# lukeduball/VoxelRaymarcher

Hardware: AMD Instinct MI355X
Metric: Mrays/sec at 1920x1080, 256^3 grid (VCS+original); achieved HBM GB/s (higher is better)
Workload: dtype f32; 1 GPU; C2: 256^3 synthetic, vcs+original, 1920x1080; grid=256, width=1920, height=1080, tiling=weak, store=VOXEL_CLUSTER_STORE, algorithm=ORIGINAL, scale=48, voxels=395883, parallelism=row-band tiles x1, layout=bands, frames_in_flight=2, hw_queues=4

## Files before the change

include/vr.h:

```cpp
#ifndef VR_H
#define VR_H

#include <stddef.h>
#include <stdint.h>

#ifdef __cplusplus
extern "C" {
#endif

#define VR_OK 0
#define VR_E_INVALID (-1)
#define VR_E_HIP (-2)
#define VR_E_NOMEM (-3)
#define VR_E_IO (-4)
#define VR_E_BUILD (-5)
#define VR_E_PARSE (-6)

typedef enum { VR_STORE_VCS = 0, VR_STORE_HASHTABLE = 1 } vr_store;

typedef enum { VR_ALGO_LONGESTAXIS = 0, VR_ALGO_ORIGINAL = 1 } vr_algo;

typedef struct {
    float origin[3];
    float lower_left[3];
    float horizontal[3];
    float vertical[3];
    float forward[3];
} vr_camera;

typedef struct {
    float light_dir[3];
    float light_color[3];
    float light_pos[3];
    int32_t use_point_light;
    int32_t use_shadows;
} vr_lighting;

typedef struct vr_scene vr_scene;

typedef struct {
    uint32_t diameter;
    int32_t min_coord;
    uint32_t region_count;
    uint32_t store;
    uint64_t voxel_count;
    uint64_t device_bytes;
    int32_t device;
} vr_scene_info;

typedef struct {
    uint32_t n;
    double p_region, p_cluster, p_voxel;
    uint64_t seed;
} vr_synth_params;

int vr_camera_make(const float eye[3], const float look_at[3], const float up[3],
                   float fov_deg, float aspect, vr_camera* out);

int vr_lighting_default(vr_lighting* out);

int vr_lighting_set_direction(vr_lighting* lit, const float dir[3]);

int vr_scene_create(int device, vr_store store, const int32_t* xyz, const uint32_t* rgb,
                    size_t n, vr_scene** out);

typedef enum { VR_BUILD_AUTO = 0, VR_BUILD_DEVICE = 1, VR_BUILD_HOST = 2 } vr_build;

int vr_scene_create_ex(int device, vr_store store, const int32_t* xyz, const uint32_t* rgb, size_t n,
                       int inputs_on_device, vr_build build, void* stream, vr_scene** out);

int vr_scene_digest(const vr_scene* s, uint64_t out[5]);

int vr_scene_load_vox(int device, vr_store store, const char* path, vr_scene** out);

int vr_scene_get_info(const vr_scene* s, vr_scene_info* out);
void vr_scene_destroy(vr_scene* s);

#define VR_VOXEL_REMOVE 0xFFFFFFFFu

int vr_scene_edit(vr_scene* s, const int32_t* xyz, const uint32_t* rgb, size_t n,
                  int inputs_on_device, void* stream);

int vr_scene_voxels(const vr_scene* s, int32_t* xyz, uint32_t* rgb, size_t capacity,
                    int outputs_on_device, void* stream, size_t* n_out);

#define VR_HIT_MISS    0u
#define VR_HIT_VOXEL   1u
#define VR_HIT_NEVER   2u
#define VR_HIT_OUTSIDE 3u

typedef struct {
    uint32_t status;
    uint32_t color;
    int32_t  voxel[3];
    int32_t  normal[3];
    int32_t  region[3];
    float    point[3];
    uint32_t reserved[2];
} vr_hit;

int vr_pick(const vr_scene* s, vr_algo algo, const vr_camera* cam,
            const float translation[3], uint32_t scale, uint32_t width, uint32_t height,
            const uint32_t* px, const uint32_t* py, size_t n, int inputs_on_device,
            vr_hit* hits, int outputs_on_device, void* stream);

typedef struct {
    float    origin[3];
    uint32_t reserved0;
    float    direction[3];
    uint32_t reserved1;
} vr_ray;

typedef enum {
    VR_TRACE_ORDER_AUTO = 0,
    VR_TRACE_ORDER_GIVEN = 1,
    VR_TRACE_ORDER_COHERENT = 2
} vr_trace_order;

int vr_trace(const vr_scene* s, vr_algo algo, const float translation[3], uint32_t scale,
             const vr_ray* rays, size_t n, int inputs_on_device,
             vr_hit* hits, int outputs_on_device, uint32_t order, void* stream);

int vr_camera_rays(int device, const vr_camera* cam, uint32_t width, uint32_t height,
                   const uint32_t* px, const uint32_t* py, size_t n, int inputs_on_device,
                   vr_ray* rays, int outputs_on_device, void* stream);

int vr_render(const vr_scene* s, vr_algo algo, const vr_camera* cam, const vr_lighting* lit,
              const float translation[3], uint32_t scale, uint32_t width, uint32_t height,
              uint32_t row_begin, uint32_t row_end, uint32_t* out_dev, void* stream);

int vr_render_bands(const vr_scene* s, vr_algo algo, const vr_camera* cam, const vr_lighting* lit,
                    const float translation[3], uint32_t scale, uint32_t width, uint32_t height,
                    uint32_t band_rows, uint32_t rank, uint32_t nranks, uint32_t* out_dev,
                    void* stream);
uint64_t vr_band_buffer_words(uint32_t width, uint32_t height, uint32_t band_rows, uint32_t nranks);

int vr_render_tiles(const vr_scene* s, vr_algo algo, const vr_camera* cam, const vr_lighting* lit,
                    const float translation[3], uint32_t scale, uint32_t width, uint32_t height,
                    uint32_t band_rows, uint32_t tile_cols, uint32_t rank, uint32_t nranks,
                    uint32_t* out_dev, void* stream);
uint64_t vr_tile_buffer_words(uint32_t width, uint32_t height, uint32_t band_rows, uint32_t tile_cols,
                              uint32_t nranks);
uint32_t vr_deal_stride_default(uint32_t nranks);
int vr_assemble_tiles(const void* parts_dev, void* frame_dev, uint32_t elem_bytes, uint32_t width,
                      uint32_t height, uint32_t band_rows, uint32_t tile_cols, uint32_t nranks,
                      uint32_t deal_stride, void* stream);

typedef enum {
    VR_KERNEL_AUTO = 0,
    VR_KERNEL_TILE = 1,
    VR_KERNEL_TILE_REWALK = 3
} vr_kernel;

typedef struct {
    uint32_t struct_size;
    uint32_t kernel;
    uint32_t row_begin, row_end;
    uint32_t band_rows;
    uint32_t rank, nranks;
    uint32_t defer_cap;
    uint64_t* bytes_dev;
    uint32_t schedule;
    uint32_t reserved;
    uint64_t* stats_dev;
    uint32_t occupancy;
    uint32_t tile_cols;
    uint32_t deal_stride;
    uint32_t reserved2;
} vr_render_opts;
#define VR_RENDER_OPTS_MIN_SIZE 48u

typedef enum {
    VR_OCCUPANCY_AUTO = 0,
    VR_OCCUPANCY_LONE = 1,
    VR_OCCUPANCY_IN_FLIGHT = 2
} vr_occupancy;

int vr_render_opts_init(vr_render_opts* opts);

typedef enum {
    VR_SCHEDULE_AUTO = 0,
    VR_SCHEDULE_GRID = 1,
    VR_SCHEDULE_HEAVIEST_FIRST = 2
} vr_schedule;
int vr_forget_orders(int device);
int vr_debug_skip_next_crawl(int device);
int vr_debug_capture_lane_order(int device);
int vr_debug_lane_order(int device, uint32_t info[8], uint32_t* pcost, uint64_t pcost_words, uint8_t* perm,
                        uint64_t perm_bytes);
int vr_debug_order_uses(int device, uint64_t out[8]);
int vr_render_ex(const vr_scene* s, vr_algo algo, const vr_camera* cam, const vr_lighting* lit,
                 const float translation[3], uint32_t scale, uint32_t width, uint32_t height,
                 const vr_render_opts* opts, uint32_t* out_dev, void* stream);

int vr_render_count(const vr_scene* s, vr_algo algo, const vr_camera* cam, const vr_lighting* lit,
                    const float translation[3], uint32_t scale, uint32_t width, uint32_t height,
                    uint32_t row_begin, uint32_t row_end, uint32_t* out_dev,
                    uint64_t* bytes_dev, void* stream);

int vr_pack_rgb8(const uint32_t* words_dev, uint8_t* rgb_dev, uint64_t n_pixels, void* stream);

int vr_png_write(const char* path, const uint8_t* image, uint32_t width, uint32_t height, int channels, int level);

int vr_png_encode(const uint8_t* image, uint32_t width, uint32_t height, int channels, int level, int threads,
                  uint8_t* out, size_t capacity, size_t* out_len);

int vr_synth_generate(const vr_synth_params* p, int32_t* xyz, uint32_t* rgb, size_t capacity,
                      size_t* n_out);

int vr_vox_read(const char* path, int32_t* xyz, uint32_t* rgb, size_t capacity, size_t* n_out);
int vr_vox_write(const char* path, const int32_t* xyz, const uint32_t* rgb, size_t n);

int vr_vxb_read(const char* path, int32_t* xyz, uint32_t* rgb, size_t capacity, size_t* n_out);
int vr_vxb_write(const char* path, const int32_t* xyz, const uint32_t* rgb, size_t n);
int vr_scene_file_read(const char* path, int32_t* xyz, uint32_t* rgb, size_t capacity, size_t* n_out);

const char* vr_last_error(void);
const char* vr_version(void);

#ifdef __cplusplus
}
#endif
#endif
```

voxelraymarcher_amd/__init__.py:

```python
from ._capi import LIB_PATH, VrError, lib
from .output import FrameWriter, ImageWriter, encode_png, write_png
from .renderer import (CONFIGS, HIT_DTYPE, VOXEL_REMOVE, Build, HitStatus, Camera, DeviceScene, Kernel, Occupancy, PreparedRender, RayMarchAlgorithm,
                       RenderConfig,
                       Schedule, StorageType, VoxelSceneCPU, VoxelSceneInfo, assemble_tiles_device, band_buffer_words,
                       create_scene, deal_stride_default, debug_capture_lane_order, debug_lane_order, debug_order_uses, debug_skip_next_crawl,
                       forget_orders, pack_rgb8, pick, parse_algorithm, parse_storage, RAY_DTYPE, TraceOrder, camera_rays, trace,
                       read_voxel_file, render_bands, render_count, render_ex, render_tiles, run_raymarching_kernel,
                       setup_constant_values, synth_scene, tile_buffer_words, write_binary_scene, write_voxel_file)

__all__ = ["LIB_PATH", "VrError", "lib", "FrameWriter", "ImageWriter", "encode_png", "write_png", "CONFIGS", "HIT_DTYPE", "HitStatus",
           "VOXEL_REMOVE", "Build", "pick", "RAY_DTYPE", "TraceOrder", "camera_rays", "trace",
           "Camera", "DeviceScene", "Kernel", "Occupancy", "PreparedRender", "RayMarchAlgorithm", "RenderConfig", "Schedule",
           "StorageType", "VoxelSceneCPU", "VoxelSceneInfo", "assemble_tiles_device", "band_buffer_words",
           "create_scene", "deal_stride_default", "debug_capture_lane_order", "debug_lane_order", "debug_order_uses",
           "debug_skip_next_crawl", "forget_orders", "pack_rgb8", "parse_algorithm", "parse_storage",
           "read_voxel_file", "render_bands", "render_count", "render_ex", "render_tiles", "run_raymarching_kernel",
           "setup_constant_values", "synth_scene", "tile_buffer_words", "write_binary_scene", "write_voxel_file"]
```

voxelraymarcher_amd/_capi.py:

```python
from __future__ import annotations

import ctypes
import os
from ctypes import (POINTER, c_char_p, c_double, c_float, c_int, c_int32, c_size_t, c_uint8, c_uint32,
                    c_uint64, c_void_p)

import torch

HERE = os.path.dirname(os.path.abspath(__file__))
LIB_PATH = os.environ.get("VR_LIBRARY") or os.path.join(HERE, "libvr.so")

VR_OK = 0
ERRORS = {-1: "VR_E_INVALID", -2: "VR_E_HIP", -3: "VR_E_NOMEM", -4: "VR_E_IO", -5: "VR_E_BUILD", -6: "VR_E_PARSE"}

VR_STORE_VCS, VR_STORE_HASHTABLE = 0, 1
VR_ALGO_LONGESTAXIS, VR_ALGO_ORIGINAL = 0, 1


class VrCamera(ctypes.Structure):
    _fields_ = [("origin", c_float * 3), ("lower_left", c_float * 3), ("horizontal", c_float * 3),
                ("vertical", c_float * 3), ("forward", c_float * 3)]


class VrLighting(ctypes.Structure):
    _fields_ = [("light_dir", c_float * 3), ("light_color", c_float * 3), ("light_pos", c_float * 3),
                ("use_point_light", c_int32), ("use_shadows", c_int32)]


class VrSceneInfo(ctypes.Structure):
    _fields_ = [("diameter", c_uint32), ("min_coord", c_int32), ("region_count", c_uint32), ("store", c_uint32),
                ("voxel_count", c_uint64), ("device_bytes", c_uint64), ("device", c_int32)]


class VrSynthParams(ctypes.Structure):
    _fields_ = [("n", c_uint32), ("p_region", c_double), ("p_cluster", c_double), ("p_voxel", c_double),
                ("seed", c_uint64)]


VR_KERNEL_AUTO, VR_KERNEL_TILE, VR_KERNEL_TILE_REWALK = 0, 1, 3
VR_SCHEDULE_AUTO, VR_SCHEDULE_GRID, VR_SCHEDULE_HEAVIEST_FIRST = 0, 1, 2
VR_OCCUPANCY_AUTO, VR_OCCUPANCY_LONE, VR_OCCUPANCY_IN_FLIGHT = 0, 1, 2


class VrRenderOpts(ctypes.Structure):
    _fields_ = [("struct_size", c_uint32), ("kernel", c_uint32), ("row_begin", c_uint32), ("row_end", c_uint32),
                ("band_rows", c_uint32), ("rank", c_uint32), ("nranks", c_uint32), ("defer_cap", c_uint32),
                ("bytes_dev", c_void_p), ("schedule", c_uint32), ("reserved", c_uint32), ("stats_dev", c_void_p),
                ("occupancy", c_uint32), ("tile_cols", c_uint32), ("deal_stride", c_uint32), ("reserved2", c_uint32)]


VR_RENDER_OPTS_MIN_SIZE = 48

VR_HIT_MISS, VR_HIT_VOXEL, VR_HIT_NEVER, VR_HIT_OUTSIDE = 0, 1, 2, 3


class VrHit(ctypes.Structure):
    _fields_ = [("status", c_uint32), ("color", c_uint32), ("voxel", c_int32 * 3), ("normal", c_int32 * 3),
                ("region", c_int32 * 3), ("point", c_float * 3), ("reserved", c_uint32 * 2)]


class VrRay(ctypes.Structure):
    _fields_ = [("origin", c_float * 3), ("reserved0", c_uint32), ("direction", c_float * 3), ("reserved1", c_uint32)]


VR_TRACE_ORDER_AUTO, VR_TRACE_ORDER_GIVEN, VR_TRACE_ORDER_COHERENT = 0, 1, 2


class VrError(RuntimeError):
    def __init__(self, code: int, where: str, msg: str):
        super().__init__(f"{where}: {ERRORS.get(code, code)}: {msg}")
        self.code = code


SIGNATURES = {
    "vr_camera_make": (c_int, [POINTER(c_float), POINTER(c_float), POINTER(c_float), c_float, c_float,
                               POINTER(VrCamera)]),
    "vr_lighting_default": (c_int, [POINTER(VrLighting)]),
    "vr_lighting_set_direction": (c_int, [POINTER(VrLighting), POINTER(c_float)]),
    "vr_png_write": (c_int, [c_char_p, c_void_p, c_uint32, c_uint32, c_int, c_int]),
    "vr_png_encode": (c_int, [c_void_p, c_uint32, c_uint32, c_int, c_int, c_int, c_void_p, c_size_t, POINTER(c_size_t)]),
    "vr_scene_create": (c_int, [c_int, c_int, POINTER(c_int32), POINTER(c_uint32), c_size_t, POINTER(c_void_p)]),
    "vr_scene_create_ex": (c_int, [c_int, c_int, c_void_p, c_void_p, c_size_t, c_int, c_int, c_void_p, POINTER(c_void_p)]),
    "vr_scene_digest": (c_int, [c_void_p, POINTER(c_uint64)]),
    "vr_scene_load_vox": (c_int, [c_int, c_int, c_char_p, POINTER(c_void_p)]),
    "vr_scene_get_info": (c_int, [c_void_p, POINTER(VrSceneInfo)]),
    "vr_scene_destroy": (None, [c_void_p]),
    "vr_scene_edit": (c_int, [c_void_p, c_void_p, c_void_p, c_size_t, c_int, c_void_p]),
    "vr_scene_voxels": (c_int, [c_void_p, c_void_p, c_void_p, c_size_t, c_int, c_void_p, POINTER(c_size_t)]),
    "vr_render": (c_int, [c_void_p, c_int, POINTER(VrCamera), POINTER(VrLighting), POINTER(c_float), c_uint32,
                          c_uint32, c_uint32, c_uint32, c_uint32, c_void_p, c_void_p]),
    "vr_render_bands": (c_int, [c_void_p, c_int, POINTER(VrCamera), POINTER(VrLighting), POINTER(c_float),
                                c_uint32, c_uint32, c_uint32, c_uint32, c_uint32, c_uint32, c_void_p, c_void_p]),
    "vr_band_buffer_words": (c_uint64, [c_uint32, c_uint32, c_uint32, c_uint32]),
    "vr_render_tiles": (c_int, [c_void_p, c_int, POINTER(VrCamera), POINTER(VrLighting), POINTER(c_float),
                                c_uint32, c_uint32, c_uint32, c_uint32, c_uint32, c_uint32, c_uint32, c_void_p,
                                c_void_p]),
    "vr_tile_buffer_words": (c_uint64, [c_uint32, c_uint32, c_uint32, c_uint32, c_uint32]),
    "vr_deal_stride_default": (c_uint32, [c_uint32]),
    "vr_forget_orders": (c_int, [c_int]),
    "vr_debug_skip_next_crawl": (c_int, [c_int]),
    "vr_debug_capture_lane_order": (c_int, [c_int]),
    "vr_debug_lane_order": (c_int, [c_int, POINTER(c_uint32), c_void_p, c_uint64, c_void_p, c_uint64]),
    "vr_debug_order_uses": (c_int, [c_int, POINTER(c_uint64)]),
    "vr_assemble_tiles": (c_int, [c_void_p, c_void_p, c_uint32, c_uint32, c_uint32, c_uint32, c_uint32, c_uint32,
                                  c_uint32, c_void_p]),
    "vr_render_ex": (c_int, [c_void_p, c_int, POINTER(VrCamera), POINTER(VrLighting), POINTER(c_float), c_uint32,
                             c_uint32, c_uint32, POINTER(VrRenderOpts), c_void_p, c_void_p]),
    "vr_render_opts_init": (c_int, [POINTER(VrRenderOpts)]),
    "vr_render_count": (c_int, [c_void_p, c_int, POINTER(VrCamera), POINTER(VrLighting), POINTER(c_float),
                                c_uint32, c_uint32, c_uint32, c_uint32, c_uint32, c_void_p, c_void_p, c_void_p]),
    "vr_pick": (c_int, [c_void_p, c_int, POINTER(VrCamera), POINTER(c_float), c_uint32, c_uint32, c_uint32, c_void_p,
                        c_void_p, c_size_t, c_int, c_void_p, c_int, c_void_p]),
    "vr_trace": (c_int, [c_void_p, c_int, POINTER(c_float), c_uint32, c_void_p, c_size_t, c_int, c_void_p, c_int,
                         c_uint32, c_void_p]),
    "vr_camera_rays": (c_int, [c_int, POINTER(VrCamera), c_uint32, c_uint32, c_void_p, c_void_p, c_size_t, c_int,
                               c_void_p, c_int, c_void_p]),
    "vr_pack_rgb8": (c_int, [c_void_p, c_void_p, c_uint64, c_void_p]),
    "vr_synth_generate": (c_int, [POINTER(VrSynthParams), POINTER(c_int32), POINTER(c_uint32), c_size_t,
                                  POINTER(c_size_t)]),
    "vr_vox_read": (c_int, [c_char_p, POINTER(c_int32), POINTER(c_uint32), c_size_t, POINTER(c_size_t)]),
    "vr_vox_write": (c_int, [c_char_p, POINTER(c_int32), POINTER(c_uint32), c_size_t]),
    "vr_vxb_read": (c_int, [c_char_p, POINTER(c_int32), POINTER(c_uint32), c_size_t, POINTER(c_size_t)]),
    "vr_vxb_write": (c_int, [c_char_p, POINTER(c_int32), POINTER(c_uint32), c_size_t]),
    "vr_scene_file_read": (c_int, [c_char_p, POINTER(c_int32), POINTER(c_uint32), c_size_t, POINTER(c_size_t)]),
    "vr_last_error": (c_char_p, []),
    "vr_version": (c_char_p, []),
}

_lib = None


def lib() -> ctypes.CDLL:
    global _lib
    if _lib is None:
        if not os.path.exists(LIB_PATH):
            raise ImportError(f"{LIB_PATH} not built: run __graft_entry__.build() "
                              "(make -C voxelraymarcher_amd/csrc)")
        handle = ctypes.CDLL(LIB_PATH, mode=ctypes.RTLD_GLOBAL)
        for name, (res, args) in SIGNATURES.items():
            fn = getattr(handle, name)
            fn.restype = res
            fn.argtypes = args
        _lib = handle
    return _lib


def check(rc: int, where: str) -> None:
    if rc != VR_OK:
        raise VrError(rc, where, lib().vr_last_error().decode(errors="replace"))


def f3(v) -> ctypes.Array:
    return (c_float * 3)(*[float(x) for x in v])


__all__ = ["lib", "check", "VrCamera", "VrLighting", "VrRenderOpts", "VR_RENDER_OPTS_MIN_SIZE", "VR_KERNEL_AUTO",
           "VR_KERNEL_TILE", "VR_KERNEL_TILE_REWALK", "VR_SCHEDULE_AUTO", "VR_SCHEDULE_GRID",
           "VR_SCHEDULE_HEAVIEST_FIRST", "VR_OCCUPANCY_AUTO", "VR_OCCUPANCY_LONE", "VR_OCCUPANCY_IN_FLIGHT",
           "VrSceneInfo", "VrSynthParams", "VrHit", "VR_HIT_MISS",
           "VR_HIT_VOXEL", "VR_HIT_NEVER", "VR_HIT_OUTSIDE", "VrRay", "VR_TRACE_ORDER_AUTO",
           "VR_TRACE_ORDER_GIVEN", "VR_TRACE_ORDER_COHERENT", "VrError", "SIGNATURES",
           "VR_STORE_VCS", "VR_STORE_HASHTABLE", "VR_ALGO_LONGESTAXIS", "VR_ALGO_ORIGINAL", "f3", "LIB_PATH",
           "c_uint8"]
```

voxelraymarcher_amd/csrc/vr_internal.h:

```cpp
#pragma once

#include <hip/hip_runtime.h>
#include <stddef.h>
#include <stdint.h>

#include <string>

namespace vr {

int set_error(int code, const std::string& msg);

constexpr uint32_t kEmpty = 1u << 30;
constexpr uint32_t kNone = 0xFFFFFFFFu;
constexpr int32_t kBlock = 64;
constexpr uint32_t kTileBudget = 4096u;
constexpr uint32_t kCrawlBudget = 1u << 30;
constexpr uint32_t kDeferMarker = 0xFFFFFFFFu;
constexpr uint32_t kVcsMaxRegions = 65536u;
constexpr uint32_t kHashFilterWords = 8192u;

struct KScene {
    const uint32_t* region_slot;
    const uint2* vcs_mask;
    const uint32_t* vcs_vals;
    const uint32_t* vcs_cbits;
    const uint4* ht_meta;
    const uint2* ht_slots;
    const uint32_t* ht_filter;
    uint32_t D;
    int32_t min_coord;
    uint32_t n_regions;
};

struct KView {
    float llc[3], hor[3], ver[3], org[3];
    float L[3], LC[3], LP[3];
    float Lr[3];
    uint32_t L_fast;
    float Lw[3];
    uint32_t L_order, L_cls, L_unit, L_eq;
    float translation[3];
    float scale_f;
    int32_t use_point_light, use_shadows;
    uint32_t W, H;
    uint32_t row0, band_rows, rank, nranks, local_rows, row_limit;
    uint32_t band_minv;
    uint32_t LW;
    uint32_t tile_cols;
    uint32_t tile_minv;
    uint32_t col_R, col_rank, col_stride;
    uint32_t* out;
    unsigned long long* bytes;
    unsigned long long* stats;
    uint32_t* defer;
    uint32_t defer_cap;
    uint32_t crawl_rewalk;
    uint32_t crawl_rpw;
    uint32_t* defer_stat;
    const uint32_t* order;
    uint32_t* cost;
    const uint8_t* perm;
    uint32_t* pcost;
    uint32_t* slot_stat;
    uint32_t launch_id;
};
static_assert(sizeof(KView) - offsetof(KView, out) == 104,
              "a KView field was added after `out`: review whether it belongs to the view identity");

constexpr uint32_t kDeferCap = 16384;
constexpr uint32_t kDeferRecWords = 20;
constexpr uint32_t kDeferWords = 4 + kDeferCap * kDeferRecWords;

hipError_t launch_march(int store, int algo, bool count, const KScene& s, const KView& v,
                        hipStream_t stream, uint32_t crawl_wgs, bool in_flight, bool crawl = true);
uint32_t crawl_grid(uint32_t records, uint32_t rpw);
constexpr uint32_t kPickMiss = 0, kPickVoxel = 1, kPickNever = 2, kPickOutside = 3;
hipError_t launch_pick(int store, int algo, const KScene& s, const KView& v, const uint32_t* px, const uint32_t* py,
                       uint32_t n, void* hits, hipStream_t stream);
hipError_t launch_trace(int store, int algo, const KScene& s, const KView& v, const void* rays, const uint32_t* idx,
                        uint32_t n, void* hits, hipStream_t stream);
hipError_t launch_camera_rays(const KView& v, const uint32_t* px, const uint32_t* py, uint32_t n, void* rays,
                              hipStream_t stream);
hipError_t trace_order(const KScene& s, const KView& v, const void* rays, uint32_t n, hipStream_t stream,
                       void** scratch, const uint32_t** idx);
hipError_t launch_cluster_bits(const uint2* vcs_mask, uint32_t n_regions, uint32_t* cbits, hipStream_t stream);
hipError_t launch_hash_filter(const uint4* ht_meta, const uint2* ht_slots, uint32_t n_regions, uint32_t* filter,
                              hipStream_t stream);
hipError_t launch_pack_rgb8(const uint32_t* words, uint8_t* rgb, uint64_t n, hipStream_t stream);
struct TileLayout {
    uint32_t W, H, band_rows, tile_cols, R, stride, LW;
    uint64_t rank_words;
};
hipError_t launch_assemble_tiles(const void* parts, void* frame, uint32_t elem_bytes, const TileLayout& t,
                                 hipStream_t stream);
void march_grid(const KView& v, uint32_t& columns, uint32_t& rows);
constexpr uint32_t kWavesPerTileGroup = 2;
hipError_t launch_order(const uint32_t* cost, uint32_t n, uint32_t columns, uint32_t* order, hipStream_t stream);
size_t perm_bytes(uint32_t gx, uint32_t gy);
struct LaneShape {
    uint32_t block_x, block_y, entry_bytes, seat;
};
LaneShape lane_shape();
hipError_t launch_perm(const uint32_t* pcost, uint32_t LW, uint32_t rows, uint32_t gx, uint32_t gy, uint8_t* perm,
                       uint32_t* cost, hipStream_t stream);

}
```

voxelraymarcher_amd/csrc/vr_launch.cpp:

```cpp
#include <algorithm>
#include <chrono>
#include <climits>
#include <cmath>
#include <cstddef>
#include <cstdio>
#include <cstdlib>
#include <cstring>
#include <initializer_list>
#include <mutex>
#include <string>
#include <vector>

#include "vr_host.h"
#pragma GCC visibility push(hidden)
#include "vr_launch_plan.h"
#pragma GCC visibility pop

namespace {

using vr::DeviceGuard;
using vr::fail;
using vr::hip_fail;

int make_view(const vr_scene* s, const vr_camera* cam, const vr_lighting* lit, const float translation[3],
              uint32_t scale, uint32_t width, uint32_t height, vr::KView& v) {
    if (!s) return fail(VR_E_INVALID, "scene is NULL");
    if (!cam || !lit) return fail(VR_E_INVALID, "camera/lighting NULL");
    if (width == 0 || height == 0 || width > 65536 || height > 65536) return fail(VR_E_INVALID, "bad image size");
    memset(&v, 0, sizeof v);
    for (int i = 0; i < 3; ++i) {
        v.llc[i] = cam->lower_left[i]; v.hor[i] = cam->horizontal[i]; v.ver[i] = cam->vertical[i];
        v.org[i] = cam->origin[i];
        v.L[i] = lit->light_dir[i]; v.LC[i] = lit->light_color[i]; v.LP[i] = lit->light_pos[i];
        v.translation[i] = translation ? translation[i] : 0.0f;
    }
    v.L_fast = 1u;
    for (int i = 0; i < 3; ++i) {
        const float a = std::fabs(v.L[i]);
        v.Lr[i] = 1.0f / v.L[i];
        if (!(a >= 0x1p-64f && a <= 0x1p+20f)) v.L_fast = 0u;
    }
    {
        const float ax = std::fabs(v.L[0]), ay = std::fabs(v.L[1]), az = std::fabs(v.L[2]);
        const uint32_t order =
            (ax > ay && ax > az) ? (ay > az ? 0u : 1u) : (ay > az ? (ax > az ? 2u : 3u) : (ax > ay ? 4u : 5u));
        const float k = 1.0f / (order < 2u ? ax : (order < 4u ? ay : az));
        uint32_t cls = 0;
        bool unit = order == 5u && ax == ay && ay == az;
        for (int i = 0; i < 3; ++i) {
            v.Lw[i] = k * v.L[i];
            cls |= (uint32_t)(v.Lw[i] > 0.0f) << (2 * i) | (uint32_t)(v.Lw[i] < 0.0f) << (2 * i + 1);
            unit = unit && std::fabs(v.Lw[i]) == 1.0f;
        }
        v.L_order = order;
        v.L_cls = cls;
        v.L_unit = unit ? 1u : 0u;
        v.L_eq = (v.L[0] == v.L[1] && v.L[1] == v.L[2]) ? 1u : 0u;
    }
    v.scale_f = (float)scale;
    v.use_point_light = lit->use_point_light ? 1 : 0;
    v.use_shadows = lit->use_shadows ? 1 : 0;
    v.W = width;
    v.H = height;
    v.LW = width;
    return VR_OK;
}

bool env_flag(const char* name, bool dflt) {
    const char* e = std::getenv(name);
    return e ? (dflt ? e[0] != '0' : e[0] == '1') : dflt;
}
uint32_t env_uint(const char* name, long lo, long hi, uint32_t dflt) {
    const char* e = std::getenv(name);
    const long v = e ? std::strtol(e, nullptr, 10) : lo - 1;
    return v >= lo && v <= hi ? (uint32_t)v : dflt;
}
uint32_t order_refresh() { static const uint32_t r = env_uint("VR_ORDER_REFRESH", 1, LONG_MAX, 0); return r; }
bool order_enabled() { static const bool on = env_flag("VR_ORDER", true); return on; }
bool lane_order_enabled() { static const bool on = env_flag("VR_LANE_ORDER", true); return on; }
bool crawl_skip_enabled() { static const bool on = env_flag("VR_CRAWL_SKIP", true); return on; }
const vr::PolicyKnobs& policy_knobs() {
    static const vr::PolicyKnobs k = {env_flag("VR_INFLIGHT_HEAVY", false), env_flag("VR_INFLIGHT_WAVES", true),
                                      env_uint("VR_CRAWL_RPW", 1, 64, 0), env_uint("VR_CRAWL_RPW_IN_FLIGHT", 1, 64, 32)};
    return k;
}

struct SlotRing {
    const size_t words = vr::kDeferWords;
    const uint32_t nslots = 16;
    struct Slot {
        vr::WorkOrder work;
        vr::LaneOrder lane;
        vr::CrawlSkip skip;
    };
    struct Dev {
        std::mutex mu;
        uint32_t* base = nullptr;
        std::vector<hipEvent_t> ev;
        std::vector<bool> used;
        uint32_t next = 0;
        uint32_t* stat_host = nullptr;
        uint32_t* stat_dev = nullptr;
        uint32_t launch_serial = 0;
        std::vector<Slot> slot;
        bool any = false;
        hipStream_t last_stream = nullptr;
        uint32_t last_idx = 0;
        uint64_t last_key = 0;
        bool force_skip = false;
        uint64_t uses[6] = {0, 0, 0, 0, 0, 0};
        bool capture_lane = false;
        struct LaneCapture {
            uint32_t LW = 0, rows = 0, gx = 0, gy = 0;
            std::vector<uint32_t> pcost;
            std::vector<uint8_t> perm;
        } lane_capture;
        bool alone(hipStream_t st) const {
            return !any || last_stream == st || hipEventQuery(ev[last_idx]) == hipSuccess;
        }
        bool follow(hipStream_t st, uint32_t idx, uint64_t key) {
            const bool repeat = last_key == key;
            any = true;
            last_stream = st;
            last_idx = idx;
            last_key = key;
            return repeat;
        }
    } dev[64];
} g_defer_ring;

int ring_init(SlotRing& r, SlotRing::Dev& D) {
    void* q = nullptr;
    const size_t bytes = (size_t)r.nslots * r.words * sizeof(uint32_t);
    std::vector<hipEvent_t> made;
    auto undo = [&](hipError_t e, const char* what) {
        for (hipEvent_t x : made) (void)hipEventDestroy(x);
        if (q) (void)hipFree(q);
        return hip_fail(e, what);
    };
    hipError_t e = hipMalloc(&q, bytes);
    if (e != hipSuccess) { q = nullptr; return undo(e, "hipMalloc(slot ring)"); }
    e = hipMemset(q, 0, bytes);
    if (e == hipSuccess) e = hipDeviceSynchronize();
    if (e != hipSuccess) return undo(e, "hipMemset(slot ring)");
    std::vector<hipEvent_t> ev(r.nslots);
    for (uint32_t i = 0; i < r.nslots; ++i) {
        e = hipEventCreateWithFlags(&ev[i], hipEventDisableTiming);
        if (e != hipSuccess) return undo(e, "hipEventCreate(slot ring)");
        made.push_back(ev[i]);
    }
    void* h = nullptr;
    void* hd = nullptr;
    const size_t stat_words = 2u + 2u * (size_t)r.nslots;
    e = hipHostMalloc(&h, sizeof(uint32_t) * stat_words, hipHostMallocMapped | hipHostMallocCoherent);
    if (e == hipSuccess) {
        for (size_t i = 0; i < stat_words; ++i) ((volatile uint32_t*)h)[i] = 0u;
        e = hipHostGetDevicePointer(&hd, h, 0);
        if (e != hipSuccess) (void)hipHostFree(h);
    }
    if (e != hipSuccess) return undo(e, "hipHostMalloc(crawl statistics)");
    D.ev = std::move(ev);
    D.used.assign(r.nslots, false);
    D.slot.assign(r.nslots, SlotRing::Slot{});
    D.stat_host = (uint32_t*)h;
    D.stat_dev = (uint32_t*)hd;
    D.base = (uint32_t*)q;
    return VR_OK;
}

struct SlotLease {
    SlotRing* ring = nullptr;
    std::unique_lock<std::mutex> lk;
    int dev = -1;
    uint32_t idx = 0;
    uint32_t* p = nullptr;
    int acquire(SlotRing& r, int d, hipStream_t stream) {
        if (d < 0 || d >= 64) return fail(VR_E_INVALID, "device index too large");
        SlotRing::Dev& D = r.dev[d];
        lk = std::unique_lock<std::mutex>(D.mu);
        if (!D.base) {
            int rc = ring_init(r, D);
            if (rc) return rc;
        }
        ring = &r;
        dev = d;
        idx = D.next;
        D.next = (D.next + 1u) % r.nslots;
        if (D.used[idx]) {
            hipError_t e = hipStreamWaitEvent(stream, D.ev[idx], 0);
            if (e != hipSuccess) return hip_fail(e, "hipStreamWaitEvent(slot ring)");
        }
        p = D.base + r.words * idx;
        return VR_OK;
    }
    SlotRing::Dev& D() const { return ring->dev[dev]; }
    int release(hipStream_t stream) {
        hipError_t e = hipEventRecord(D().ev[idx], stream);
        if (e != hipSuccess) return hip_fail(e, "hipEventRecord(slot ring)");
        D().used[idx] = true;
        lk.unlock();
        return VR_OK;
    }
};

uint64_t view_key(const vr_scene* s, vr_algo algo, const vr::KView& v) {
    const uint32_t a = (uint32_t)algo;
    uint64_t h = vr::fnv1a(vr::kFnvBasis, &s->serial, sizeof s->serial);
    h = vr::fnv1a(h, &s->revision, sizeof s->revision);
    h = vr::fnv1a(h, &a, sizeof a);
    return vr::fnv1a(h, &v, offsetof(vr::KView, out));
}

uint64_t crawl_key(uint64_t key, const vr::KView& v) {
    const uint32_t knobs[2] = {v.defer_cap, v.crawl_rewalk};
    return vr::fnv1a(key, knobs, sizeof knobs);
}

struct Regrow {
    void** p;
    size_t bytes;
};
hipError_t regrow(std::initializer_list<Regrow> bufs, hipStream_t st) {
    hipError_t e = hipSuccess;
    for (const Regrow& b : bufs) {
        const hipError_t e2 = *b.p ? hipFreeAsync(*b.p, st) : hipSuccess;
        if (e == hipSuccess) e = e2;
        *b.p = nullptr;
    }
    for (const Regrow& b : bufs)
        if (e == hipSuccess) e = hipMallocAsync(b.p, b.bytes, st);
    if (e != hipSuccess)
        for (const Regrow& b : bufs) {
            if (*b.p) (void)hipFreeAsync(*b.p, st);
            *b.p = nullptr;
        }
    return e;
}

hipError_t bind_work_order(vr::WorkOrder& W, uint32_t gx, uint32_t gy, uint64_t key, bool repeat, hipStream_t st,
                           vr::KView& v, bool& remake) {
    const uint32_t n = gx * gy;
    if (n > W.cap) {
        W.cap = 0;
        W.valid = false;
        const hipError_t e = regrow({{(void**)&W.cost, sizeof(uint32_t) * vr::kWavesPerTileGroup * (size_t)n},
                                     {(void**)&W.order, sizeof(uint32_t) * (size_t)n}}, st);
        if (e != hipSuccess) return e;
        W.cap = n;
    }
    const bool match = W.matches(gx, gy, key);
    v.order = match ? W.order : nullptr;
    remake = vr::remake_due(match, W.relaned, repeat, W.age, order_refresh());
    v.cost = remake ? W.cost : nullptr;
    return hipSuccess;
}

hipError_t bind_lane_order(vr::LaneOrder& L, uint32_t gx, uint32_t gy, uint64_t key, bool repeat, hipStream_t st,
                           vr::KView& v, bool& relane, const char*& what) {
    const size_t nperm = vr::perm_bytes(gx, gy);
    if (nperm > L.bcap) {
        L.bcap = 0;
        L.valid = false;
        what = "lane order buffer";
        const hipError_t e = regrow({{(void**)&L.perm, nperm}}, st);
        if (e != hipSuccess) return e;
        L.bcap = nperm;
    }
    const bool match = L.matches(gx, gy, key);
    v.perm = match ? L.perm : nullptr;
    relane = vr::remake_due(match, false, repeat, L.age, order_refresh());
    if (!relane) return hipSuccess;
    what = "lane order walk lengths";
    return hipMallocAsync((void**)&v.pcost, sizeof(uint32_t) * (size_t)v.LW * v.local_rows, st);
}

int refuse_capture(hipStream_t st) {
    hipStreamCaptureStatus cap = hipStreamCaptureStatusNone;
    const hipError_t e = hipStreamIsCapturing(st, &cap);
    if (e != hipSuccess) return hip_fail(e, "hipStreamIsCapturing");
    if (cap != hipStreamCaptureStatusNone)
        return fail(VR_E_INVALID, "vr_render* cannot be captured into a HIP graph (stream is capturing)");
    return VR_OK;
}

void order_check(const vr::WorkOrder& W, uint32_t slot, uint32_t gx, uint32_t gy) {
    if (!std::getenv("VR_ORDER_CHECK")) return;
    const uint32_t n = gx * gy;
    std::vector<uint32_t> h(n), c(2 * (size_t)n);
    (void)hipDeviceSynchronize();
    (void)hipMemcpy(h.data(), W.order, 4 * (size_t)n, hipMemcpyDeviceToHost);
    (void)hipMemcpy(c.data(), W.cost, 8 * (size_t)n, hipMemcpyDeviceToHost);
    std::vector<int> seen(n, 0);
    int bad = 0;
    for (uint32_t i = 0; i < n; ++i) {
        const uint32_t t = (h[i] >> 16) * gx + (h[i] & 0xFFFFu);
        if ((h[i] & 0xFFFFu) >= gx || t >= n || seen[t]++) ++bad;
    }
    fprintf(stderr, "[order] slot %u grid %ux%u n %u bad %d first %08x %08x cost0 %u %u\n", slot, gx, gy, n, bad, h[0],
            n > 1 ? h[1] : 0u, c[0], c[1]);
}

#ifdef VR_HOST_PROF
}
static uint64_t g_hp[4096][8];
static uint32_t g_hp_n = 0;
static inline uint64_t hp_now() { return (uint64_t)std::chrono::steady_clock::now().time_since_epoch().count(); }
extern "C" int vr_host_prof_fetch(uint64_t* out, int n) {
    const uint32_t k = g_hp_n < 4096u ? g_hp_n : 4096u;
    const uint32_t m = (uint32_t)n < k ? (uint32_t)n : k;
    for (uint32_t i = 0; i < m; ++i)
        for (int j = 0; j < 8; ++j) out[8 * i + j] = g_hp[(g_hp_n - m + i) % 4096u][j];
    return (int)m;
}
namespace {
#define VR_HP(i) hp_row[i] = hp_now()
#else
#define VR_HP(i) do { } while (0)
#endif

int launch(const vr_scene* s, vr_algo algo, uint32_t kernel, uint32_t schedule, uint32_t occupancy, vr::KView& v,
           void* stream) {
#ifdef VR_HOST_PROF
    uint64_t* hp_row = g_hp[g_hp_n++ % 4096u];
    for (int j = 0; j < 8; ++j) hp_row[j] = 0;
#endif
    VR_HP(0);
    if (algo != VR_ALGO_ORIGINAL && algo != VR_ALGO_LONGESTAXIS) return fail(VR_E_INVALID, "unknown algorithm");
    if (kernel != VR_KERNEL_AUTO && kernel != VR_KERNEL_TILE && kernel != VR_KERNEL_TILE_REWALK)
        return fail(VR_E_INVALID, "unknown kernel (2, the persistent kernel, was retired)");
    if (occupancy > VR_OCCUPANCY_IN_FLIGHT) return fail(VR_E_INVALID, "unknown occupancy");
    if (v.local_rows == 0 || v.LW == 0) return VR_OK;
    DeviceGuard dg(s->device);
    const hipStream_t st = (hipStream_t)stream;
    int rc = refuse_capture(st);
    if (rc) return rc;
    SlotLease lease;
    rc = lease.acquire(g_defer_ring, s->device, st);
    if (rc) return rc;
    VR_HP(1);
    auto bail = [&](hipError_t err, const char* what) {
        (void)lease.release(st);
        return hip_fail(err, what);
    };
    SlotRing::Dev& D = lease.D();
    SlotRing::Slot& S = D.slot[lease.idx];
    v.crawl_rewalk = kernel == VR_KERNEL_TILE_REWALK ? 1u : 0u;
    v.defer = lease.p;
    v.defer_cap = (v.defer_cap && v.defer_cap < vr::kDeferCap) ? v.defer_cap : vr::kDeferCap;
    v.defer_stat = D.stat_dev;
    v.slot_stat = D.stat_dev + 2 + 2 * (size_t)lease.idx;
    const uint32_t expect = *(volatile uint32_t*)D.stat_host;
    uint32_t gx = 0, gy = 0;
    vr::march_grid(v, gx, gy);
    const uint32_t n = gx * gy;
    const bool alone = D.alone(st);
    VR_HP(2);
    const vr::LaunchPolicy pol = vr::launch_policy(schedule, occupancy, alone, policy_knobs());
    v.crawl_rpw = pol.crawl_rpw;
    const uint64_t key = view_key(s, algo, v);
    const bool repeat = D.follow(st, lease.idx, key);
    VR_HP(3);
    bool remake = false, relane = false;
    hipError_t e = hipSuccess;
    if (pol.heavy && order_enabled() && n != 0) {
        e = bind_work_order(S.work, gx, gy, key, repeat, st, v, remake);
        if (e != hipSuccess) return bail(e, "work order buffers");
    }
    if (lane_order_enabled() && n != 0) {
        const char* what = "";
        e = bind_lane_order(S.lane, gx, gy, key, repeat, st, v, relane, what);
        if (e != hipSuccess) return bail(e, what);
    }
    VR_HP(4);
    v.launch_id = vr::next_launch_id(D.launch_serial);
    const uint64_t report = *reinterpret_cast<volatile uint64_t*>(D.stat_host + 2 + 2 * (size_t)lease.idx);
    const bool crawl = S.skip.step(crawl_key(key, v), report, v.launch_id, D.force_skip, crawl_skip_enabled());
    VR_HP(5);
    const vr::KScene ks = vr::kscene(s);
    const uint32_t cwgs = vr::crawl_grid(expect, v.crawl_rpw);
    D.uses[0] += 1u;
    D.uses[2] += v.perm != nullptr;
    D.uses[4] += v.order != nullptr;
    D.uses[5] += !crawl;
    VR_HP(6);
    e = vr::launch_march((int)s->store, (int)algo, v.bytes != nullptr, ks, v, st, cwgs, pol.hi, crawl);
    VR_HP(7);
    bool with_costs = false;
    if (e == hipSuccess && relane) {
        with_costs = order_enabled() && S.work.cost && S.work.cap >= n;
        e = vr::launch_perm(v.pcost, v.LW, v.local_rows, gx, gy, S.lane.perm, with_costs ? S.work.cost : nullptr, st);
        S.lane.learned(gx, gy, key, e == hipSuccess);
        D.uses[1] += e == hipSuccess;
        S.work.relaned = !with_costs;
        if (e == hipSuccess && D.capture_lane) {
            D.capture_lane = false;
            SlotRing::Dev::LaneCapture& C = D.lane_capture;
            C.LW = v.LW, C.rows = v.local_rows, C.gx = gx, C.gy = gy;
            C.pcost.resize((size_t)v.LW * v.local_rows);
            C.perm.resize(vr::perm_bytes(gx, gy));
            e = hipStreamSynchronize(st);
            if (e == hipSuccess) e = hipMemcpy(C.pcost.data(), v.pcost, sizeof(uint32_t) * C.pcost.size(), hipMemcpyDeviceToHost);
            if (e == hipSuccess) e = hipMemcpy(C.perm.data(), S.lane.perm, C.perm.size(), hipMemcpyDeviceToHost);
        }
    }
    if (e == hipSuccess && (remake || with_costs)) {
        e = vr::launch_order(S.work.cost, n, gx, S.work.order, st);
        order_check(S.work, lease.idx, gx, gy);
        S.work.learned(gx, gy, key, e == hipSuccess);
        D.uses[3] += e == hipSuccess;
    }
    if (v.pcost) {
        const hipError_t ef = hipFreeAsync(v.pcost, st);
        if (e == hipSuccess) e = ef;
    }
    rc = lease.release(st);
    if (e != hipSuccess) return hip_fail(e, "ray-march launch");
    return rc;
}

}

extern "C" {

int vr_render_ex(const vr_scene* s, vr_algo algo, const vr_camera* cam, const vr_lighting* lit,
                 const float translation[3], uint32_t scale, uint32_t width, uint32_t height,
                 const vr_render_opts* opts, uint32_t* out_dev, void* stream) {
    if (!opts) return fail(VR_E_INVALID, "opts is NULL");
    if (opts->struct_size < VR_RENDER_OPTS_MIN_SIZE)
        return fail(VR_E_INVALID, "vr_render_opts.struct_size is " + std::to_string(opts->struct_size) +
                                      ": set it to sizeof(vr_render_opts) (vr_render_opts_init); a struct built "
                                      "against the layout without struct_size is not accepted");
    vr_render_opts o{};
    std::memcpy(&o, opts, std::min<size_t>(opts->struct_size, sizeof o));
    if (o.reserved != 0u) return fail(VR_E_INVALID, "vr_render_opts.reserved must be 0");
    vr::KView v;
    int rc = make_view(s, cam, lit, translation, scale, width, height, v);
    if (rc) return rc;
    if (!out_dev) return fail(VR_E_INVALID, "out_dev is NULL");
    const uint32_t row_end = o.row_end == 0xFFFFFFFFu ? height : o.row_end;
    if (o.row_begin > row_end || row_end > height) return fail(VR_E_INVALID, "bad row range");
    if (!o.nranks || o.rank >= o.nranks) return fail(VR_E_INVALID, "bad band partition");
    if (o.reserved2 != 0u) return fail(VR_E_INVALID, "vr_render_opts.reserved2 must be 0");
    const uint32_t rows = row_end - o.row_begin;
    const uint32_t band = o.band_rows ? o.band_rows : std::max(1u, rows);
    v.row0 = o.row_begin;
    v.row_limit = row_end;
    v.band_rows = band;
    v.band_minv = band == 1u ? 0xFFFFFFFFu : (uint32_t)((1ull << 32) / band);
    if (o.tile_cols == 0u) {
        v.rank = o.rank;
        v.nranks = o.nranks;
        v.local_rows = (uint32_t)(vr_band_buffer_words(width, rows, band, o.nranks) / width);
    } else {
        if (o.tile_cols > width) return fail(VR_E_INVALID, "tile_cols larger than the frame width");
        v.rank = 0;
        v.nranks = 1;
        v.local_rows = (uint32_t)(((uint64_t)rows + band - 1) / band * band);
        const uint32_t nblk = (width + o.tile_cols - 1) / o.tile_cols;
        v.LW = (nblk + o.nranks - 1) / o.nranks * o.tile_cols;
        v.tile_cols = o.tile_cols;
        v.tile_minv = o.tile_cols == 1u ? 0xFFFFFFFFu : (uint32_t)((1ull << 32) / o.tile_cols);
        v.col_R = o.nranks;
        v.col_rank = o.rank;
        v.col_stride = (o.deal_stride ? o.deal_stride : vr_deal_stride_default(o.nranks)) % o.nranks;
        if (v.local_rows > 65535u || v.LW > 65535u) return fail(VR_E_INVALID, "tile buffer too large");
    }
    v.out = out_dev;
    v.bytes = (unsigned long long*)o.bytes_dev;
    v.stats = o.bytes_dev ? (unsigned long long*)o.stats_dev : nullptr;
    v.defer_cap = o.defer_cap;
    if (o.schedule > VR_SCHEDULE_HEAVIEST_FIRST) return fail(VR_E_INVALID, "unknown schedule");
    return launch(s, algo, o.kernel, o.schedule, o.occupancy, v, stream);
}

int vr_pick(const vr_scene* s, vr_algo algo, const vr_camera* cam, const float translation[3], uint32_t scale,
            uint32_t width, uint32_t height, const uint32_t* px, const uint32_t* py, size_t n, int inputs_on_device,
            vr_hit* hits, int outputs_on_device, void* stream) {
    static_assert(sizeof(vr_hit) == 64 && offsetof(vr_hit, voxel) == 8 && offsetof(vr_hit, normal) == 20 &&
                      offsetof(vr_hit, region) == 32 && offsetof(vr_hit, point) == 44 && offsetof(vr_hit, reserved) == 56,
                  "vr_hit: the record pick_kernel writes");
    static_assert(vr::kPickMiss == VR_HIT_MISS && vr::kPickVoxel == VR_HIT_VOXEL && vr::kPickNever == VR_HIT_NEVER &&
                      vr::kPickOutside == VR_HIT_OUTSIDE, "VR_HIT_*");
    if (!s) return fail(VR_E_INVALID, "vr_pick: scene is NULL");
    if (!cam || !translation) return fail(VR_E_INVALID, "vr_pick: camera/translation NULL");
    if (n && (!px || !py || !hits)) return fail(VR_E_INVALID, "vr_pick: px/py/hits NULL");
    if (width == 0 || height == 0 || width > 65536 || height > 65536) return fail(VR_E_INVALID, "vr_pick: bad image size");
    if (n >= (1ull << 31)) return fail(VR_E_INVALID, "vr_pick: too many queries");
    if (algo != VR_ALGO_ORIGINAL && algo != VR_ALGO_LONGESTAXIS) return fail(VR_E_INVALID, "vr_pick: unknown algorithm");
    if (n == 0) return VR_OK;
    vr_lighting lit;
    vr_lighting_default(&lit);
    vr::KView v;
    int rc = make_view(s, cam, &lit, translation, scale, width, height, v);
    if (rc) return rc;
    v.row_limit = height;
    v.band_rows = height;
    v.band_minv = height == 1u ? 0xFFFFFFFFu : (uint32_t)((1ull << 32) / height);
    v.nranks = 1;
    v.local_rows = height;
    DeviceGuard dg(s->device);
    const hipStream_t st = (hipStream_t)stream;
    hipStreamCaptureStatus cap = hipStreamCaptureStatusNone;
    hipError_t e = hipStreamIsCapturing(st, &cap);
    if (e != hipSuccess) return hip_fail(e, "hipStreamIsCapturing");
    if (cap != hipStreamCaptureStatusNone)
        return fail(VR_E_INVALID, "vr_pick cannot be captured into a HIP graph (stream is capturing)");
    const uint32_t *dpx = px, *dpy = py;
    void *tq = nullptr, *th = nullptr;
    auto release = [&]() {
        if (tq) (void)hipFree(tq);
        if (th) (void)hipFree(th);
    };
    if (!inputs_on_device) {
        e = hipMalloc(&tq, 2 * n * sizeof(uint32_t));
        if (e == hipSuccess) e = hipMemcpyAsync(tq, px, n * sizeof(uint32_t), hipMemcpyHostToDevice, st);
        if (e == hipSuccess)
            e = hipMemcpyAsync((uint32_t*)tq + n, py, n * sizeof(uint32_t), hipMemcpyHostToDevice, st);
        if (e != hipSuccess) { release(); return hip_fail(e, "vr_pick: query upload"); }
        dpx = (const uint32_t*)tq;
        dpy = dpx + n;
    }
    void* dh = hits;
    if (!outputs_on_device) {
        e = hipMalloc(&th, n * sizeof(vr_hit));
        if (e != hipSuccess) { release(); return hip_fail(e, "vr_pick: hit buffer"); }
        dh = th;
    } else if (((uintptr_t)hits & 15u) != 0u) {
        release();
        return fail(VR_E_INVALID, "vr_pick: device hits must be 16-byte aligned");
    }
    e = vr::launch_pick((int)s->store, (int)algo, vr::kscene(s), v, dpx, dpy, (uint32_t)n, dh, st);
    if (e == hipSuccess && !outputs_on_device)
        e = hipMemcpyAsync(hits, th, n * sizeof(vr_hit), hipMemcpyDeviceToHost, st);
    const hipError_t es = hipStreamSynchronize(st);
    if (e == hipSuccess) e = es;
    release();
    if (e != hipSuccess) return hip_fail(e, "vr_pick");
    return VR_OK;
}

int vr_trace(const vr_scene* s, vr_algo algo, const float translation[3], uint32_t scale, const vr_ray* rays, size_t n,
             int inputs_on_device, vr_hit* hits, int outputs_on_device, uint32_t order, void* stream) {
    static_assert(sizeof(vr_ray) == 32 && offsetof(vr_ray, reserved0) == 12 && offsetof(vr_ray, direction) == 16 &&
                      offsetof(vr_ray, reserved1) == 28, "vr_ray: the record trace_kernel loads");
    if (!s) return fail(VR_E_INVALID, "vr_trace: scene is NULL");
    if (!translation) return fail(VR_E_INVALID, "vr_trace: translation NULL");
    if (n && (!rays || !hits)) return fail(VR_E_INVALID, "vr_trace: rays/hits NULL");
    if (n >= (1ull << 31)) return fail(VR_E_INVALID, "vr_trace: too many rays");
    if (algo != VR_ALGO_ORIGINAL && algo != VR_ALGO_LONGESTAXIS) return fail(VR_E_INVALID, "vr_trace: unknown algorithm");
    if (order != VR_TRACE_ORDER_AUTO && order != VR_TRACE_ORDER_GIVEN && order != VR_TRACE_ORDER_COHERENT)
        return fail(VR_E_INVALID, "vr_trace: unknown order");
    if (n == 0) return VR_OK;
    if (inputs_on_device && ((uintptr_t)rays & 15u) != 0u)
        return fail(VR_E_INVALID, "vr_trace: device rays must be 16-byte aligned");
    if (outputs_on_device && ((uintptr_t)hits & 15u) != 0u)
        return fail(VR_E_INVALID, "vr_trace: device hits must be 16-byte aligned");
    vr::KView v;
    memset(&v, 0, sizeof v);
    for (int i = 0; i < 3; ++i) v.translation[i] = translation[i];
    v.scale_f = (float)scale;
    const bool coherent = order == VR_TRACE_ORDER_COHERENT;
    DeviceGuard dg(s->device);
    const hipStream_t st = (hipStream_t)stream;
    hipStreamCaptureStatus cap = hipStreamCaptureStatusNone;
    hipError_t e = hipStreamIsCapturing(st, &cap);
    if (e != hipSuccess) return hip_fail(e, "hipStreamIsCapturing");
    if (cap != hipStreamCaptureStatusNone)
        return fail(VR_E_INVALID, "vr_trace cannot be captured into a HIP graph (stream is capturing)");
    void *tr = nullptr, *th = nullptr, *to = nullptr;
    auto release = [&]() {
        if (tr) (void)hipFree(tr);
        if (th) (void)hipFree(th);
        if (to) (void)hipFree(to);
    };
    const void* dr = rays;
    if (!inputs_on_device) {
        e = hipMalloc(&tr, n * sizeof(vr_ray));
        if (e == hipSuccess) e = hipMemcpyAsync(tr, rays, n * sizeof(vr_ray), hipMemcpyHostToDevice, st);
        if (e != hipSuccess) { (void)hipStreamSynchronize(st); release(); return hip_fail(e, "vr_trace: ray upload"); }
        dr = tr;
    }
    void* dh = hits;
    if (!outputs_on_device) {
        e = hipMalloc(&th, n * sizeof(vr_hit));
        if (e != hipSuccess) { (void)hipStreamSynchronize(st); release(); return hip_fail(e, "vr_trace: hit buffer"); }
        dh = th;
    }
    const uint32_t* idx = nullptr;
    if (coherent) e = vr::trace_order(vr::kscene(s), v, dr, (uint32_t)n, st, &to, &idx);
    if (e == hipSuccess) e = vr::launch_trace((int)s->store, (int)algo, vr::kscene(s), v, dr, idx, (uint32_t)n, dh, st);
    if (e == hipSuccess && !outputs_on_device)
        e = hipMemcpyAsync(hits, th, n * sizeof(vr_hit), hipMemcpyDeviceToHost, st);
    const hipError_t es = hipStreamSynchronize(st);
    if (e == hipSuccess) e = es;
    release();
    if (e != hipSuccess) return hip_fail(e, "vr_trace");
    return VR_OK;
}

int vr_camera_rays(int device, const vr_camera* cam, uint32_t width, uint32_t height, const uint32_t* px,
                   const uint32_t* py, size_t n, int inputs_on_device, vr_ray* rays, int outputs_on_device, void* stream) {
    if (!cam) return fail(VR_E_INVALID, "vr_camera_rays: camera NULL");
    if (n && (!px || !py || !rays)) return fail(VR_E_INVALID, "vr_camera_rays: px/py/rays NULL");
    if (width == 0 || height == 0 || width > 65536 || height > 65536)
        return fail(VR_E_INVALID, "vr_camera_rays: bad image size");
    if (n >= (1ull << 31)) return fail(VR_E_INVALID, "vr_camera_rays: too many pixels");
    if (device < 0 || device > 63) return fail(VR_E_INVALID, "vr_camera_rays: bad device");
    if (n == 0) return VR_OK;
    if (outputs_on_device && ((uintptr_t)rays & 15u) != 0u)
        return fail(VR_E_INVALID, "vr_camera_rays: device rays must be 16-byte aligned");
    vr::KView v;
    memset(&v, 0, sizeof v);
    for (int i = 0; i < 3; ++i) {
        v.llc[i] = cam->lower_left[i]; v.hor[i] = cam->horizontal[i]; v.ver[i] = cam->vertical[i];
        v.org[i] = cam->origin[i];
    }
    v.W = width;
    v.H = height;
    v.LW = width;
    v.row_limit = height;
    v.band_rows = height;
    v.band_minv = height == 1u ? 0xFFFFFFFFu : (uint32_t)((1ull << 32) / height);
    v.nranks = 1;
    v.local_rows = height;
    int ndev = 0;
    if (hipGetDeviceCount(&ndev) != hipSuccess || device >= ndev) return fail(VR_E_INVALID, "vr_camera_rays: no such device");
    DeviceGuard dg(device);
    const hipStream_t st = (hipStream_t)stream;
    hipStreamCaptureStatus cap = hipStreamCaptureStatusNone;
    hipError_t e = hipStreamIsCapturing(st, &cap);
    if (e != hipSuccess) return hip_fail(e, "hipStreamIsCapturing");
    if (cap != hipStreamCaptureStatusNone)
        return fail(VR_E_INVALID, "vr_camera_rays cannot be captured into a HIP graph (stream is capturing)");
    const uint32_t *dpx = px, *dpy = py;
    void *tq = nullptr, *tr = nullptr;
    auto release = [&]() {
        if (tq) (void)hipFree(tq);
        if (tr) (void)hipFree(tr);
    };
    if (!inputs_on_device) {
        e = hipMalloc(&tq, 2 * n * sizeof(uint32_t));
        if (e == hipSuccess) e = hipMemcpyAsync(tq, px, n * sizeof(uint32_t), hipMemcpyHostToDevice, st);
        if (e == hipSuccess)
            e = hipMemcpyAsync((uint32_t*)tq + n, py, n * sizeof(uint32_t), hipMemcpyHostToDevice, st);
        if (e != hipSuccess) { (void)hipStreamSynchronize(st); release(); return hip_fail(e, "vr_camera_rays: pixel upload"); }
        dpx = (const uint32_t*)tq;
        dpy = dpx + n;
    }
    void* dr = rays;
    if (!outputs_on_device) {
        e = hipMalloc(&tr, n * sizeof(vr_ray));
        if (e != hipSuccess) { (void)hipStreamSynchronize(st); release(); return hip_fail(e, "vr_camera_rays: ray buffer"); }
        dr = tr;
    }
    e = vr::launch_camera_rays(v, dpx, dpy, (uint32_t)n, dr, st);
    if (e == hipSuccess && !outputs_on_device)
        e = hipMemcpyAsync(rays, tr, n * sizeof(vr_ray), hipMemcpyDeviceToHost, st);
    const hipError_t es = hipStreamSynchronize(st);
    if (e == hipSuccess) e = es;
    release();
    if (e != hipSuccess) return hip_fail(e, "vr_camera_rays");
    return VR_OK;
}

int vr_render_opts_init(vr_render_opts* opts) {
    if (!opts) return fail(VR_E_INVALID, "NULL argument");
    *opts = vr_render_opts{};
    opts->struct_size = (uint32_t)sizeof(vr_render_opts);
    opts->kernel = VR_KERNEL_AUTO;
    opts->row_begin = 0;
    opts->row_end = 0xFFFFFFFFu;
    opts->band_rows = 0;
    opts->rank = 0;
    opts->nranks = 1;
    opts->schedule = VR_SCHEDULE_AUTO;
    return VR_OK;
}

namespace {
vr_render_opts opts_rows(uint32_t row_begin, uint32_t row_end) {
    vr_render_opts o;
    vr_render_opts_init(&o);
    o.row_begin = row_begin;
    o.row_end = row_end;
    return o;
}
}

int vr_render(const vr_scene* s, vr_algo algo, const vr_camera* cam, const vr_lighting* lit, const float translation[3],
              uint32_t scale, uint32_t width, uint32_t height, uint32_t row_begin, uint32_t row_end, uint32_t* out_dev,
              void* stream) {
    const vr_render_opts o = opts_rows(row_begin, row_end);
    return vr_render_ex(s, algo, cam, lit, translation, scale, width, height, &o, out_dev, stream);
}

uint64_t vr_band_buffer_words(uint32_t width, uint32_t height, uint32_t band_rows, uint32_t nranks) {
    if (!band_rows || !nranks) return 0;
    uint64_t nb = (height + (uint64_t)band_rows - 1) / band_rows;
    uint64_t per = (nb + nranks - 1) / nranks;
    return per * band_rows * (uint64_t)width;
}

uint32_t vr_deal_stride_default(uint32_t nranks) {
    return (nranks % 3u == 0u) ? 1u : 3u;
}

int vr_forget_orders(int device) {
    if (device < 0 || device >= 64) return fail(VR_E_INVALID, "device index out of range");
    SlotRing::Dev& D = g_defer_ring.dev[device];
    std::lock_guard<std::mutex> lk(D.mu);
    for (SlotRing::Slot& S : D.slot) {
        S.work.forget();
        S.lane.forget();
        S.skip.forget();
    }
    D.last_key = 0;
    return VR_OK;
}

int vr_debug_skip_next_crawl(int device) {
    if (device < 0 || device >= 64) return fail(VR_E_INVALID, "device index out of range");
    SlotRing::Dev& D = g_defer_ring.dev[device];
    std::lock_guard<std::mutex> lk(D.mu);
    D.force_skip = true;
    return VR_OK;
}

int vr_debug_order_uses(int device, uint64_t out[8]) {
    if (device < 0 || device >= 64) return fail(VR_E_INVALID, "device index out of range");
    if (!out) return fail(VR_E_INVALID, "out is NULL");
    SlotRing::Dev& D = g_defer_ring.dev[device];
    const vr::LaneShape sh = vr::lane_shape();
    std::lock_guard<std::mutex> lk(D.mu);
    for (int i = 0; i < 6; ++i) out[i] = D.uses[i];
    out[6] = g_defer_ring.nslots;
    out[7] = (uint64_t)sh.block_x << 16 | sh.block_y;
    return VR_OK;
}

int vr_debug_capture_lane_order(int device) {
    if (device < 0 || device >= 64) return fail(VR_E_INVALID, "device index out of range");
    SlotRing::Dev& D = g_defer_ring.dev[device];
    std::lock_guard<std::mutex> lk(D.mu);
    D.capture_lane = true;
    D.lane_capture = {};
    return VR_OK;
}

int vr_debug_lane_order(int device, uint32_t info[8], uint32_t* pcost, uint64_t pcost_words, uint8_t* perm,
                        uint64_t perm_bytes) {
    if (device < 0 || device >= 64) return fail(VR_E_INVALID, "device index out of range");
    if (!info) return fail(VR_E_INVALID, "info is NULL");
    SlotRing::Dev& D = g_defer_ring.dev[device];
    std::lock_guard<std::mutex> lk(D.mu);
    const SlotRing::Dev::LaneCapture& C = D.lane_capture;
    if (C.perm.empty()) return fail(VR_E_INVALID, "no lane order captured (vr_debug_capture_lane_order, then a repeated view)");
    const vr::LaneShape sh = vr::lane_shape();
    const uint32_t words[8] = {C.LW, C.rows, C.gx, C.gy, sh.block_x, sh.block_y, sh.entry_bytes, sh.seat};
    std::memcpy(info, words, sizeof words);
    if (pcost) {
        if (pcost_words != C.pcost.size()) return fail(VR_E_INVALID, "pcost_words is not info[0] * info[1]");
        std::memcpy(pcost, C.pcost.data(), sizeof(uint32_t) * C.pcost.size());
    }
    if (perm) {
        if (perm_bytes != C.perm.size()) return fail(VR_E_INVALID, "perm_bytes is not the captured order's size");
        std::memcpy(perm, C.perm.data(), C.perm.size());
    }
    return VR_OK;
}

uint64_t vr_tile_buffer_words(uint32_t width, uint32_t height, uint32_t band_rows, uint32_t tile_cols, uint32_t nranks) {
    if (!nranks || !tile_cols || !width || !height) return 0;
    const uint64_t band = band_rows ? band_rows : height;
    const uint64_t rows = (height + band - 1) / band * band;
    const uint64_t nblk = ((uint64_t)width + tile_cols - 1) / tile_cols;
    return rows * ((nblk + nranks - 1) / nranks * tile_cols);
}

int vr_render_tiles(const vr_scene* s, vr_algo algo, const vr_camera* cam, const vr_lighting* lit,
                    const float translation[3], uint32_t scale, uint32_t width, uint32_t height, uint32_t band_rows,
                    uint32_t tile_cols, uint32_t rank, uint32_t nranks, uint32_t* out_dev, void* stream) {
    if (!band_rows || !tile_cols) return fail(VR_E_INVALID, "band_rows and tile_cols must be > 0");
    vr_render_opts o = opts_rows(0, height);
    o.band_rows = band_rows;
    o.tile_cols = tile_cols;
    o.rank = rank;
    o.nranks = nranks;
    return vr_render_ex(s, algo, cam, lit, translation, scale, width, height, &o, out_dev, stream);
}

int vr_assemble_tiles(const void* parts_dev, void* frame_dev, uint32_t elem_bytes, uint32_t width, uint32_t height,
                      uint32_t band_rows, uint32_t tile_cols, uint32_t nranks, uint32_t deal_stride, void* stream) {
    if (!parts_dev || !frame_dev) return fail(VR_E_INVALID, "NULL device buffer");
    if (elem_bytes < 1u || elem_bytes > 4u) return fail(VR_E_INVALID, "elem_bytes must be 1..4");
    if (!width || !height || !band_rows || !tile_cols || !nranks || tile_cols > width)
        return fail(VR_E_INVALID, "bad tile layout");
    vr::TileLayout t{};
    t.W = width;
    t.H = height;
    t.band_rows = band_rows;
    t.tile_cols = tile_cols;
    t.R = nranks;
    t.stride = (deal_stride ? deal_stride : vr_deal_stride_default(nranks)) % nranks;
    t.LW = (uint32_t)(vr_tile_buffer_words(width, band_rows, band_rows, tile_cols, nranks) / band_rows);
    t.rank_words = vr_tile_buffer_words(width, height, band_rows, tile_cols, nranks);
    hipError_t e = vr::launch_assemble_tiles(parts_dev, frame_dev, elem_bytes, t, (hipStream_t)stream);
    if (e != hipSuccess) return hip_fail(e, "assemble_tiles launch");
    return VR_OK;
}

int vr_render_bands(const vr_scene* s, vr_algo algo, const vr_camera* cam, const vr_lighting* lit,
                    const float translation[3], uint32_t scale, uint32_t width, uint32_t height, uint32_t band_rows,
                    uint32_t rank, uint32_t nranks, uint32_t* out_dev, void* stream) {
    if (!band_rows) return fail(VR_E_INVALID, "band_rows must be > 0");
    vr_render_opts o = opts_rows(0, height);
    o.band_rows = band_rows;
    o.rank = rank;
    o.nranks = nranks;
    return vr_render_ex(s, algo, cam, lit, translation, scale, width, height, &o, out_dev, stream);
}

int vr_render_count(const vr_scene* s, vr_algo algo, const vr_camera* cam, const vr_lighting* lit,
                    const float translation[3], uint32_t scale, uint32_t width, uint32_t height, uint32_t row_begin,
                    uint32_t row_end, uint32_t* out_dev, uint64_t* bytes_dev, void* stream) {
    if (!bytes_dev) return fail(VR_E_INVALID, "bytes_dev is NULL");
    vr_render_opts o = opts_rows(row_begin, row_end);
    o.bytes_dev = bytes_dev;
    return vr_render_ex(s, algo, cam, lit, translation, scale, width, height, &o, out_dev, stream);
}

int vr_pack_rgb8(const uint32_t* words_dev, uint8_t* rgb_dev, uint64_t n_pixels, void* stream) {
    if (n_pixels && (!words_dev || !rgb_dev)) return fail(VR_E_INVALID, "NULL device buffer");
    hipError_t e = vr::launch_pack_rgb8(words_dev, rgb_dev, n_pixels, (hipStream_t)stream);
    if (e != hipSuccess) return hip_fail(e, "pack_rgb8 launch");
    return VR_OK;
}

}
```

voxelraymarcher_amd/csrc/vr_launch_plan.h:

```cpp
#pragma once

#include <stddef.h>
#include <stdint.h>

#include "vr.h"

namespace vr {

struct PolicyKnobs {
    bool inflight_heavy;
    bool in_flight_occupancy;
    uint32_t rpw_override;
    uint32_t rpw_in_flight;
};
struct LaunchPolicy {
    bool heavy;
    bool hi;
    uint32_t crawl_rpw;
};
inline LaunchPolicy launch_policy(uint32_t schedule, uint32_t occupancy, bool alone, const PolicyKnobs& k) {
    LaunchPolicy p;
    p.heavy = schedule == VR_SCHEDULE_HEAVIEST_FIRST || (schedule == VR_SCHEDULE_AUTO && (alone || k.inflight_heavy));
    p.hi = occupancy == VR_OCCUPANCY_IN_FLIGHT || (occupancy == VR_OCCUPANCY_AUTO && !alone && k.in_flight_occupancy);
    p.crawl_rpw = k.rpw_override ? k.rpw_override : (alone ? 2u : k.rpw_in_flight);
    return p;
}

inline bool refresh_due(uint32_t& age, uint32_t refresh) { return refresh != 0 && ++age >= refresh; }
inline bool remake_due(bool match, bool stale, bool repeat, uint32_t& age, uint32_t refresh) {
    return match ? (stale || refresh_due(age, refresh)) : repeat;
}

struct Learned {
    uint32_t gx = 0, gy = 0, age = 0;
    uint64_t key = 0;
    bool valid = false;
    bool matches(uint32_t x, uint32_t y, uint64_t k) const { return valid && gx == x && gy == y && key == k; }
    void learned(uint32_t x, uint32_t y, uint64_t k, bool ok) { valid = ok; gx = x; gy = y; key = k; age = 0; }
    void forget() { valid = false; }
};
struct WorkOrder : Learned {
    uint32_t* cost = nullptr;
    uint32_t* order = nullptr;
    uint32_t cap = 0;
    bool relaned = false;
    void learned(uint32_t x, uint32_t y, uint64_t k, bool ok) { Learned::learned(x, y, k, ok); relaned = false; }
    void forget() { valid = relaned = false; }
};
struct LaneOrder : Learned {
    uint8_t* perm = nullptr;
    size_t bcap = 0;
};

inline uint32_t next_launch_id(uint32_t& serial) { return ++serial ? serial : ++serial; }

struct CrawlSkip {
    uint32_t cid = 0;
    uint64_t ckey = 0;
    bool czero = false;
    bool step(uint64_t key, uint64_t report, uint32_t lid, bool& force, bool enabled) {
        const uint32_t rid = (uint32_t)report, count = (uint32_t)(report >> 32);
        if (ckey != key) {
            czero = false;
        } else if (czero) {
            if (count != 0u) czero = false;
        } else if (cid != 0u) {
            czero = rid == cid && count == 0u;
        }
        if (force) {
            force = false;
            czero = true;
            ckey = key;
        }
        const bool crawl = !(czero && enabled);
        if (crawl) {
            cid = lid;
            ckey = key;
        }
        return crawl;
    }
    void forget() { cid = 0; czero = false; }
};

}
```

voxelraymarcher_amd/csrc/vr_march.hip:

```cpp
#include "vr_device.h"
#include "vr_crawl.h"

#include <algorithm>
#include <type_traits>

#ifdef VR_CRAWL_PROF
__device__ unsigned int g_vr_crawl_prof[16384 * 8];
#endif
#ifdef VR_DIAG
__device__ unsigned long long g_vr_diag[64];
#define VR_DIAG_COUNT(k)                                                              \
    do {                                                                             \
        if (__lane_id() == (uint32_t)__builtin_ctzll(__builtin_amdgcn_read_exec())) \
            atomicAdd(&g_vr_diag[(k)], 1ull);                                        \
    } while (0)
#define VR_DIAG_COUNT_IF(c, k)                                  \
    do {                                                       \
        if (__builtin_amdgcn_ballot_w64(c) != 0) VR_DIAG_COUNT(k); \
    } while (0)
#define VR_DIAG_PAT(shadow, p) VR_DIAG_COUNT(((shadow) ? 51 : 43) + (p))
#else
#define VR_DIAG_COUNT(k) do { } while (0)
#define VR_DIAG_COUNT_IF(c, k) do { } while (0)
#define VR_DIAG_PAT(shadow, p) do { } while (0)
#endif

namespace vr {
namespace {

template <int S> struct Sgn { static constexpr int value = S; };
template <int S>
__device__ __forceinline__ float plane_v(float o, float g, float ge) {
    if constexpr (S > 0) return ceilf(o) + kEps;
    else if constexpr (S < 0) return floorf(o) - kEps;
    else return next_plane_fma(o, g, ge);
}
template <int S>
__device__ __forceinline__ int32_t plane_c8(int32_t c8) {
    if constexpr (S > 0) return 8;
    else if constexpr (S < 0) return 0;
    else return c8;
}

#ifndef VR_TILES_X
#define VR_TILES_X 2
#endif
#ifndef VR_TILES_Y
#define VR_TILES_Y 1
#endif
constexpr uint32_t kTilesX = VR_TILES_X, kTilesY = VR_TILES_Y;
#ifndef VR_UNIFORM_SKIP
#define VR_UNIFORM_SKIP 1
#endif
#ifndef VR_LONG_TAIL_GENERIC
#define VR_LONG_TAIL_GENERIC false
#endif
#ifndef VR_LONG_TAIL_EQ
#define VR_LONG_TAIL_EQ 0
#endif

constexpr uint32_t kDeferredIters = 0xFFFFFFFFu;

__device__ __forceinline__ void deferral_report(const KView& v) {
    if (v.slot_stat) *reinterpret_cast<uint2*>(v.slot_stat) = uint2{v.launch_id, 1u};
}

__device__ __forceinline__ void tile_group(const KView& v, uint32_t& bx, uint32_t& by) {
    bx = blockIdx.x;
    by = blockIdx.y;
    if (v.order) {
        const uint32_t t = v.order[blockIdx.y * gridDim.x + blockIdx.x];
        bx = t & 0xFFFFu;
        by = t >> 16;
    }
}

#ifdef VR_LANE_BLOCK
#define VR_LANE_BLOCK_DEFAULT_X VR_LANE_BLOCK
#define VR_LANE_BLOCK_DEFAULT_Y VR_LANE_BLOCK
#else
#define VR_LANE_BLOCK_DEFAULT_X 16
#define VR_LANE_BLOCK_DEFAULT_Y 32
#endif
#ifndef VR_LANE_BLOCK_X
#define VR_LANE_BLOCK_X VR_LANE_BLOCK_DEFAULT_X
#endif
#ifndef VR_LANE_BLOCK_Y
#define VR_LANE_BLOCK_Y VR_LANE_BLOCK_DEFAULT_Y
#endif
constexpr uint32_t kLaneBlockX = VR_LANE_BLOCK_X, kLaneBlockY = VR_LANE_BLOCK_Y;
static_assert((kLaneBlockX == 16 || kLaneBlockX == 32) && (kLaneBlockY == 16 || kLaneBlockY == 32),
              "lane block: 16 or 32 pixels a side");
constexpr uint32_t kLanePixels = kLaneBlockX * kLaneBlockY;
constexpr uint32_t kLbX = kLaneBlockX / (8u * kTilesX), kLbY = kLaneBlockY / (8u * kTilesY);
using PermT = std::conditional<kLanePixels == 256, uint8_t, uint16_t>::type;
#ifndef VR_LANE_SEAT
#define VR_LANE_SEAT 0
#endif
constexpr uint32_t kLaneSeat = VR_LANE_SEAT;
static_assert(kLaneSeat <= 1u, "lane seat: 0 (cost order) or 1 (Morton order)");
constexpr bool kLaneOrder = kTilesX == 2 && kTilesY == 1;
__device__ __forceinline__ void lane_pixel(const KView& v, uint32_t& x, uint32_t& l) {
    const uint32_t lane = threadIdx.x & 63u, wave = threadIdx.x >> 6;
    uint32_t bx, by;
    tile_group(v, bx, by);
    const uint32_t BX = bx / kLbX, BY = by / kLbY;
    if (kLaneOrder && v.perm && (BX + 1u) * kLbX <= gridDim.x && (BY + 1u) * kLbY <= gridDim.y) {
        const uint32_t q = ((by % kLbY) * kLbX + bx % kLbX) * kTilesX + wave;
        const uint32_t blk = BY * ((gridDim.x + kLbX - 1u) / kLbX) + BX;
        const uint32_t p = reinterpret_cast<const PermT*>(v.perm)[(size_t)blk * kLanePixels + q * 64u + lane];
        x = BX * kLaneBlockX + p % kLaneBlockX;
        l = BY * kLaneBlockY + p / kLaneBlockX;
    } else {
        x = (bx * kTilesX + wave % kTilesX) * 8u + (lane & 7u);
        l = (by * kTilesY + wave / kTilesX) * 8u + (lane >> 3);
    }
}

__device__ __forceinline__ uint32_t* tile_pixels() {
    __shared__ uint32_t p[64u * kTilesX * kTilesY];
    return p;
}

__device__ __forceinline__ uint32_t* tile_prim() {
    __shared__ uint32_t p[64u * kTilesX * kTilesY];
    return p;
}

template <int STORE, bool CRAWL>
struct ExactWalk { static constexpr bool value = CRAWL; };
template <bool PICK> struct PickCell {};
template <> struct PickCell<true> { i3 pv{0, 0, 0}; };
template <int STORE, bool COUNT, bool CRAWL, bool PICK = false>
struct Walker : Ctx<STORE, COUNT, ExactWalk<STORE, CRAWL>::value ? kCrawlBudget : kTileBudget>, PickCell<PICK> {
    using C = Ctx<STORE, COUNT, ExactWalk<STORE, CRAWL>::value ? kCrawlBudget : kTileBudget>;
    static constexpr bool kExact = ExactWalk<STORE, CRAWL>::value;
    static constexpr uint32_t kBudget = C::kBudget;
    using C::s; using C::v; using C::aborted; using C::tick; using C::exists; using C::lookup;
    using C::lighting; using C::normal_from_t; using C::in_region; using C::grid_in_region;
    using C::advance_region; using C::in_scene; using C::region_at; using C::skip_null; using C::bytes;
    __device__ Walker(const KScene& s_, const KView& v_) : C(s_, v_) {}
    static constexpr bool kFastSetup = STORE == STORE_HASH;
#ifndef VR_LONG_REMAT
#define VR_LONG_REMAT 1
#endif
    static constexpr bool kRematDir = VR_LONG_REMAT && STORE == STORE_VCS && !CRAWL;
    uint32_t ctx = 0, lit_saved = 0;
    uint32_t* lbm = nullptr;
    uint32_t bm_reg = kNone;

    template <bool SHADOW, bool EQ = false>
    __device__ __forceinline__ bool grid_original(f3& o, f3 d, uint32_t reg, i3 cr, Hit& h,
                                                  const uint32_t* rs = nullptr, const Rcp* rc = nullptr) {
        return grid_original_rt(o, d, reg, cr, h, SHADOW, SHADOW && EQ, rs, rc);
    }
    __device__ __forceinline__ bool grid_original_rt(f3& o, f3 d, uint32_t reg, i3 cr, Hit& h, const bool SHADOW,
                                                     const bool EQ, const uint32_t* rs = nullptr,
                                                     const Rcp* rc = nullptr, const bool generic = false) {
        const bool resume = CRAWL && rs != nullptr;
        VR_DIAG_COUNT(SHADOW ? 9 : 8);
        const bool px = d.x > 0.0f, py = d.y > 0.0f, pz = d.z > 0.0f;
        const bool zx = SHADOW && d.x == 0.0f, zy = SHADOW && d.y == 0.0f, zz = SHADOW && d.z == 0.0f;
        float tX, tY, tZ;
        if (resume) {
            tX = __uint_as_float(rs[11]); tY = __uint_as_float(rs[12]); tZ = __uint_as_float(rs[13]);
        } else if (!CRAWL) {
            const bool use_rc = rc && (kFastSetup || SHADOW);
            const Rcp r0x = use_rc ? rc[0] : rcp_setup(d.x), r0y = use_rc ? rc[1] : rcp_setup(d.y),
                      r0z = use_rc ? rc[2] : rcp_setup(d.z);
            const float sx = px ? 1.0f : -1.0f, sy = py ? 1.0f : -1.0f, sz = pz ? 1.0f : -1.0f;
            const float ax = next_plane_fma(o.x, sx, sx * kEps) - o.x, ay = next_plane_fma(o.y, sy, sy * kEps) - o.y,
                        az = next_plane_fma(o.z, sz, sz * kEps) - o.z;
            const bool fast = r0x.ok && r0y.ok && r0z.ok && !zx && !zy && !zz &&
                              fminf(fabsf(ax), fminf(fabsf(ay), fabsf(az))) >= 0x1p-90f;
            tX = div_fast(ax, r0x); tY = div_fast(ay, r0y); tZ = div_fast(az, r0z);
            if (__builtin_expect(__builtin_amdgcn_ballot_w64(!fast) != 0, 0)) {
                VR_DIAG_COUNT(32);
                tX = fast ? tX : (zx ? kInf : ax / d.x);
                tY = fast ? tY : (zy ? kInf : ay / d.y);
                tZ = fast ? tZ : (zz ? kInf : az / d.z);
            }
            o = add(o, scl(fminf(tX, fminf(tY, tZ)) + kEps, d));
        } else {
            const float nX = px ? ceilf(o.x) + kEps : floorf(o.x) - kEps;
            const float nY = py ? ceilf(o.y) + kEps : floorf(o.y) - kEps;
            const float nZ = pz ? ceilf(o.z) + kEps : floorf(o.z) - kEps;
            tX = zx ? kInf : (nX - o.x) / d.x;
            tY = zy ? kInf : (nY - o.y) / d.y;
            tZ = zz ? kInf : (nZ - o.z) / d.z;
            o = add(o, scl(fminf(tX, fminf(tY, tZ)) + kEps, d));
        }
        uint32_t col = kEmpty;
        if constexpr (STORE == STORE_VCS) {
            const uint2* mreg = s.vcs_mask + (size_t)reg * 8192u;
            const uint32_t moff = reg << 16;
            const uint32_t* bits = nullptr;
            if constexpr (CRAWL) {
                if (lbm) {
                    if (reg != bm_reg) {
                        const uint4* src = reinterpret_cast<const uint4*>(s.vcs_cbits + (size_t)reg * 16u);
                        const uint4 b0 = src[0], b1 = src[1], b2 = src[2], b3 = src[3];
                        uint4* dst = reinterpret_cast<uint4*>(lbm);
                        dst[0] = b0; dst[1] = b1; dst[2] = b2; dst[3] = b3;
                        bm_reg = reg;
                    }
                    bits = lbm;
                }
            }
            o = add(o, f3{0.0f, 0.0f, 0.0f});
            if (!this->in_region_bits_nz(o)) return false;
            if (aborted || this->iters >= kBudget) { aborted = true; return false; }
            bool found = false, inside = true, crawl = false;
            uint32_t crawl_after = 0;
            bool crawl_off = false;
            uint32_t vi = 0;
            int32_t qx = 0, qy = 0, qz = 0;
            Blk blk{0u, kNone};
            uint32_t bit = 0;
            bool resume_now = resume;
            for (;;) {
                f3 dl = d;
                if (CRAWL) asm("" : "+v"(dl.x), "+v"(dl.y), "+v"(dl.z));
                Rcp rx, ry, rz;
                if (rc && !CRAWL && (kFastSetup || SHADOW)) {
                    rx = EQ ? Rcp{fabsf(dl.x), fabsf(rc[0].r), rc[0].ok} : rc[0];
                    ry = rc[1];
                    rz = rc[2];
                } else {
                    rx = rcp_setup(EQ ? fabsf(dl.x) : dl.x); ry = rcp_setup(dl.y); rz = rcp_setup(dl.z);
                }
                const float gx = px ? 1.0f : -1.0f, gy = py ? 1.0f : -1.0f, gz = pz ? 1.0f : -1.0f;
                const float ex = gx * kEps, ey = gy * kEps, ez = gz * kEps;
                const int32_t cx8 = px ? 8 : 0, cy8 = py ? 8 : 0, cz8 = pz ? 8 : 0;
                const bool walk_ok = rx.ok && ry.ok && rz.ok && !zx && !zy && !zz;
                const float nlim = walk_ok ? 0x1p-90f : kInf;
                if (resume_now) {
                    resume_now = false;
                    blk = Blk{0u, kNone};
                    bit = 0;
                    qx = (int32_t)rs[15]; qy = (int32_t)rs[16]; qz = (int32_t)rs[17];
                } else {
                    auto walk = [&](auto SXc, auto SYc, auto SZc) {
                        constexpr int SX = decltype(SXc)::value, SY = decltype(SYc)::value, SZ = decltype(SZc)::value;
                        constexpr bool kPos = SX == 2 && SY == 2 && SZ == 2;
                        uint32_t ic = this->iters + (0x42800000u - kBudget);
                        const bool okw = __builtin_amdgcn_ballot_w64(!walk_ok) == 0;
                        VR_DIAG_COUNT((SHADOW ? 4 : 0) + (SX == 0 ? 1 : 0));
                        for (;;) {
                            VR_DIAG_COUNT((SHADOW ? 6 : 2) + (SX == 0 ? 1 : 0));
                            const int32_t vx = f2i(o.x), vy = f2i(o.y), vz = f2i(o.z);
                            this->count(4);
                            const uint32_t wi = this->word_index((uint32_t)vx, (uint32_t)vy, (uint32_t)vz);
                            if constexpr (CRAWL) {
                                const bool pres = !bits || ((bits[wi >> 9] >> ((wi >> 4) & 31u)) & 1u);
                                if (COUNT && !pres) ++this->nl;
                                blk = Blk{0u, kNone};
                                if (pres)
                                    blk = *reinterpret_cast<const uint2*>(reinterpret_cast<const char*>(s.vcs_mask) +
                                                                          (moff | (wi << 3)));
                            } else {
                                blk = *reinterpret_cast<const uint2*>(reinterpret_cast<const char*>(s.vcs_mask) +
                                                                      (moff | (wi << 3)));
                            }
                            __builtin_amdgcn_sched_barrier(0);
#if VR_UNIFORM_SKIP
                            float vX = plane_v<SX>(o.x, gx, ex), vY = plane_v<SY>(o.y, gy, ey), vZ = plane_v<SZ>(o.z, gz, ez);
                            asm("" : "+v"(vX), "+v"(vY), "+v"(vZ), "+v"(blk.x), "+v"(blk.y));
                            const bool skip = absent(blk);
                            float nX = vX, nY = vY, nZ = vZ;
                            const bool any_skip = __builtin_amdgcn_ballot_w64(skip) != 0;
                            if (any_skip) {
                                float cX = (float)((vx & 0x38) + plane_c8<SX>(cx8)), cY = (float)((vy & 0x38) + plane_c8<SY>(cy8)),
                                      cZ = (float)((vz & 0x38) + plane_c8<SZ>(cz8));
                                nX = skip ? cX : vX; nY = skip ? cY : vY; nZ = skip ? cZ : vZ;
                                asm volatile("" : "+v"(nX), "+v"(nY), "+v"(nZ));
                            }
#else
                            float vX = plane_v<SX>(o.x, gx, ex), vY = plane_v<SY>(o.y, gy, ey), vZ = plane_v<SZ>(o.z, gz, ez);
                            float cX = (float)((vx & 0x38) + plane_c8<SX>(cx8)), cY = (float)((vy & 0x38) + plane_c8<SY>(cy8)),
                                  cZ = (float)((vz & 0x38) + plane_c8<SZ>(cz8));
                            asm("" : "+v"(vX), "+v"(vY), "+v"(vZ), "+v"(cX), "+v"(cY), "+v"(cZ), "+v"(blk.x), "+v"(blk.y));
                            const bool skip = absent(blk);
                            const bool any_skip = __builtin_amdgcn_ballot_w64(skip) != 0;
#endif
                            const bool chk = !kPos && (!okw || any_skip);
#ifdef VR_DIAG
                            {
                                const uint64_t bs = __builtin_amdgcn_ballot_w64(skip);
                                if (bs == 0) VR_DIAG_COUNT(SHADOW ? 24 : 22);
                                else if (bs == __builtin_amdgcn_read_exec()) VR_DIAG_COUNT(SHADOW ? 25 : 23);
                            }
#endif
                            bit = this->word_bit5((uint32_t)vy, (uint32_t)vz);
                            const uint32_t fm = (uint32_t)__builtin_amdgcn_sbfe((int32_t)blk.x, bit, 1u);
                            found = fm != 0u;
                            vi = blk.y + __popc(blk.x & ((1u << (bit & 31u)) - 1u));
                            if (COUNT && !skip) this->count_bsearch(mreg + (wi & ~15u), vi, found);
#if !VR_UNIFORM_SKIP
                            const float nX = skip ? cX : vX;
                            const float nY = skip ? cY : vY;
                            const float nZ = skip ? cZ : vZ;
#endif
                            const float ax = nX - o.x, ay = nY - o.y, az = nZ - o.z;
                            float sMin;
                            crawl = false;
                            if (EQ) {
                                const float am = fminf(fabsf(ax), fminf(fabsf(ay), fabsf(az)));
                                sMin = div_fast(am, rx);
                                if (chk) {
                                    const bool bad = !(am >= nlim);
                                    if (__builtin_expect(__builtin_amdgcn_ballot_w64(bad) != 0, 0)) {
                                        VR_DIAG_COUNT(33);
                                        sMin = bad ? am / fabsf(d.x) : sMin;
                                        crawl = bad & walk_ok & skip & (sMin == 0.0f) &
                                                (CRAWL ? ic + 1u - (0x42800000u - kBudget) >= crawl_after : !crawl_off);
                                        if (CRAWL && crawl) { qx = vx; qy = vy; qz = vz; }
                                    }
                                }
                            } else {
                                float sX = div_fast(ax, rx), sY = div_fast(ay, ry), sZ = div_fast(az, rz);
                                if (chk) {
                                    const bool bad = !(fminf(fabsf(ax), fminf(fabsf(ay), fabsf(az))) >= nlim);
                                    if (__builtin_expect(__builtin_amdgcn_ballot_w64(bad) != 0, 0)) {
                                        VR_DIAG_COUNT(34);
                                        sX = bad ? (zx ? kInf : ax / d.x) : sX;
                                        sY = bad ? (zy ? kInf : ay / d.y) : sY;
                                        sZ = bad ? (zz ? kInf : az / d.z) : sZ;
                                        crawl = bad & walk_ok & skip & (fminf(sX, fminf(sY, sZ)) == 0.0f) &
                                                (CRAWL ? ic + 1u - (0x42800000u - kBudget) >= crawl_after : !crawl_off);
                                        if (CRAWL && crawl) { qx = vx; qy = vy; qz = vz; }
                                    }
                                }
                                sMin = fminf(sX, fminf(sY, sZ));
                                const bool vox = !skip && !found;
                                tX = vox ? sX : tX; tY = vox ? sY : tY; tZ = vox ? sZ : tZ;
                            }
                            const float ts = bit_select(fm, -kEps, sMin) + kEps;
                            o = EQ ? add(o, f3{ts * d.x, ts * d.x, ts * d.x}) : add(o, scl(ts, d));
                            asm("v_add_u32 %0, 1, %0" : "+v"(ic));
                            const uint32_t ev = max(max(max(max(__float_as_uint(o.x), __float_as_uint(o.y)), __float_as_uint(o.z)),
                                                        ic), fm);
                            if (ev >= 0x42800000u || crawl) break;
                        }
                        this->iters = ic - (0x42800000u - kBudget);
                    };
                    const uint32_t sg = (px ? 1u : 0u) | (py ? 2u : 0u) | (pz ? 4u : 0u);
                    using N = Sgn<-1>;
                    using P = Sgn<1>;
                    if (CRAWL || generic) {
                        walk(Sgn<0>{}, Sgn<0>{}, Sgn<0>{});
                    } else {
                        bool todo = true;
#ifdef VR_DIAG
                        uint32_t pass = 0;
#endif
                        while (todo) {
                            const uint32_t pat = __builtin_amdgcn_readfirstlane(sg);
#ifdef VR_DIAG
                            if (++pass == 2u) VR_DIAG_COUNT(41);
#endif
                            if (sg == pat) {
                                todo = false;
                                switch (pat) {
                                case 0: VR_DIAG_PAT(SHADOW, 0); walk(N{}, N{}, N{}); break;
                                case 7:
                                    VR_DIAG_PAT(SHADOW, 7);
                                    if (__builtin_amdgcn_ballot_w64(!walk_ok) == 0) {
                                        walk(Sgn<2>{}, Sgn<2>{}, Sgn<2>{});
                                    } else {
                                        VR_DIAG_COUNT(42);
                                        walk(P{}, P{}, P{});
                                    }
                                    break;
                                case 1: VR_DIAG_PAT(SHADOW, 1); if (!EQ) walk(P{}, N{}, N{}); break;
                                case 2: VR_DIAG_PAT(SHADOW, 2); if (!EQ) walk(N{}, P{}, N{}); break;
                                case 3: VR_DIAG_PAT(SHADOW, 3); if (!EQ) walk(P{}, P{}, N{}); break;
                                case 4: VR_DIAG_PAT(SHADOW, 4); if (!EQ) walk(N{}, N{}, P{}); break;
                                case 5: VR_DIAG_PAT(SHADOW, 5); if (!EQ) walk(P{}, N{}, P{}); break;
                                default: VR_DIAG_PAT(SHADOW, 6); if (!EQ) walk(N{}, P{}, P{}); break;
                                }
                            }
                        }
                    }
                }
                asm("" : "+v"(blk.x), "+v"(blk.y), "+v"(bit), "+v"(o.x), "+v"(o.y), "+v"(o.z), "+v"(this->iters));
                found = !absent(blk) & (__builtin_amdgcn_ubfe(blk.x, bit, 1u) != 0u);
                inside = found || this->in_region_bits_nz(o);
                crawl = !found && inside && this->iters < kBudget;
                if (!crawl || !inside || this->iters >= kBudget) break;
                if constexpr (!CRAWL) {
                    const bool kx = !px && truncf(o.x * 0.125f) == o.x * 0.125f && o.x + kEps * d.x == o.x;
                    const bool ky = !py && truncf(o.y * 0.125f) == o.y * 0.125f && o.y + kEps * d.y == o.y;
                    const bool kz = !pz && truncf(o.z * 0.125f) == o.z * 0.125f && o.z + kEps * d.z == o.z;
                    if ((kx || ky || kz) && v.defer) {
                        const uint32_t idx = atomicAdd(v.defer, 1u);
                        deferral_report(v);
                        if (idx < v.defer_cap) {
                            uint32_t* r = v.defer + 4 + (size_t)idx * kDeferRecWords;
                            r[0] = tile_pixels()[threadIdx.x];
                            r[1] = (SHADOW ? 1u : 0u) | this->ctx;
                            r[2] = __float_as_uint(o.x); r[3] = __float_as_uint(o.y); r[4] = __float_as_uint(o.z);
                            r[5] = (uint32_t)cr.x; r[6] = (uint32_t)cr.y; r[7] = (uint32_t)cr.z;
                            r[8] = v.launch_id;
                            r[9] = this->iters;
                            r[10] = this->bytes;
                            r[11] = SHADOW ? 0u : __float_as_uint(tX); r[12] = SHADOW ? 0u : __float_as_uint(tY);
                            r[13] = SHADOW ? 0u : __float_as_uint(tZ); r[14] = 0u;
                            r[1] |= v.crawl_rewalk ? 4u : 0u;
                            r[18] = this->lit_saved;
                            this->iters = kDeferredIters;
                            aborted = true;
                            return false;
                        }
                    }
                    if (kx || ky || kz) crawl_off = true;
// ... 557 lines not shown
            if (__builtin_expect(__builtin_amdgcn_ballot_w64(!fast) != 0, 0)) {
                VR_DIAG_COUNT(39);
                tX = fast ? tX : ax / d.x;
                tY = fast ? tY : ay / d.y;
                tZ = fast ? tZ : az / d.z;
            }
            if (tX <= 0.0f) tX = kInf;
            if (tY <= 0.0f) tY = kInf;
            if (tZ <= 0.0f) tZ = kInf;
            float tMin = fminf(tX, fminf(tY, tZ));
            if (tMin == kInf) return false;
            so = add(so, scl(tMin + kEps, d));
            cr = i3{f2i(floorf(so.x / 64.0f)), f2i(floorf(so.y / 64.0f)), f2i(floorf(so.z / 64.0f))};
            if (kExact && this->cycle_step(cyc, cr, so)) { aborted = true; return false; }
        }
        f3 o = sub(so, mk((float)(cr.x * kBlock), (float)(cr.y * kBlock), (float)(cr.z * kBlock)));
        return primary_regions<ALGO>(o, d, cr, h, nullptr, rc);
    }
    template <int ALGO>
    __device__ __forceinline__ bool primary_regions(f3 o, f3 d, i3 cr, Hit& h, const uint32_t* rs,
                                                    const Rcp* rc = nullptr) {
        if (CRAWL && rs != nullptr) {
            const bool hit = grid_original_rt(o, d, this->region_at_nocount(cr), cr, h, false, false, rs);
            if (aborted) return false;
            if (hit) return true;
            advance_region(cr, o);
        }
        auto cyc = this->cycle_start(cr, o);
        while (in_scene(cr)) {
            if (kRematDir && ALGO == ALGO_LONGEST) asm volatile("" : "+v"(d.x), "+v"(d.y), "+v"(d.z));
            if (!tick()) return false;
            VR_DIAG_COUNT(10);
            uint32_t reg = region_at(cr);
            auto cyc1 = this->cycle_start(cr, o);
            while (reg == kNone) {
                if (!tick()) return false;
                VR_DIAG_COUNT(11);
                if (!this->template skip_null<false>(cr, o, d, reg)) return false;
                if (kExact && this->cycle_step(cyc1, cr, o)) { aborted = true; return false; }
            }
            bool hit = ALGO == ALGO_ORIGINAL ? grid_original<false>(o, d, reg, cr, h, nullptr, rc)
                                             : (STORE == STORE_VCS ? grid_longest_vcs<false>(o, d, reg, cr, h)
                                                                   : grid_longest<false>(o, d, reg, cr, h));
            if (aborted) return false;
            if (hit) return true;
            advance_region(cr, o);
            if (kExact && this->cycle_step(cyc, cr, o)) { aborted = true; return false; }
        }
        return false;
    }

    template <bool LONGEST, bool EQ = false>
    __device__ __forceinline__ bool shadow(f3 o, i3 cr, const uint32_t* rs = nullptr) {
        f3 d = ld3(v.L);
        const bool lf = v.L_fast != 0u;
        const Rcp rc[3] = {Rcp{d.x, v.Lr[0], lf}, Rcp{d.y, v.Lr[1], lf}, Rcp{d.z, v.Lr[2], lf}};
        Hit dummy;
        if (CRAWL && rs != nullptr) {
            const bool hit = grid_original_rt(o, d, this->region_at_nocount(cr), cr, dummy, true, EQ, rs);
            if (aborted) return false;
            if (hit) return true;
            advance_region(cr, o);
        }
        auto cyc = this->cycle_start(cr, o);
        while (in_scene(cr)) {
            if (kRematDir && LONGEST) asm volatile("" : "+s"(d.x), "+s"(d.y), "+s"(d.z));
            if (!tick()) return false;
            VR_DIAG_COUNT(12);
            uint32_t reg = region_at(cr);
            auto cyc1 = this->cycle_start(cr, o);
            while (reg == kNone) {
                if (!tick()) return false;
                VR_DIAG_COUNT(13);
                if (!this->template skip_null<!LONGEST>(cr, o, d, reg)) return false;
                if (kExact && this->cycle_step(cyc1, cr, o)) { aborted = true; return false; }
            }
            bool hit = LONGEST ? (STORE == STORE_VCS ? grid_longest_vcs<true>(o, d, reg, cr, dummy)
                                                     : grid_longest<true>(o, d, reg, cr, dummy))
                               : grid_original<true, EQ>(o, d, reg, cr, dummy, nullptr, rc);
            if (aborted) return false;
            if (hit) return true;
            advance_region(cr, o);
            if (kExact && this->cycle_step(cyc, cr, o)) { aborted = true; return false; }
        }
        return false;
    }
};

template <bool FAST>
__device__ __forceinline__ bool pixel_ray(const KView& v, uint32_t x, uint32_t l, f3& ro, f3& rd) {
    const uint32_t q0 = __umulhi(l, v.band_minv), r0 = l - q0 * v.band_rows;
    const bool up = r0 >= v.band_rows;
    const uint32_t band = q0 + (up ? 1u : 0u), in_band = up ? r0 - v.band_rows : r0;
    const uint32_t y = v.row0 + (band * v.nranks + v.rank) * v.band_rows + in_band;
    if (y >= v.row_limit) return false;
    if (v.tile_cols) {
        const uint32_t j0 = __umulhi(x, v.tile_minv), r1 = x - j0 * v.tile_cols;
        const bool up1 = r1 >= v.tile_cols;
        const uint32_t j = j0 + (up1 ? 1u : 0u), in_blk = up1 ? r1 - v.tile_cols : r1;
        const uint32_t off = (v.col_rank + v.col_R - (v.col_stride * (band % v.col_R)) % v.col_R) % v.col_R;
        x = (j * v.col_R + off) * v.tile_cols + in_blk;
        if (x >= v.W) return false;
    }
    if (!FAST) {
        float u = ((float)x + 0.5f) / (float)v.W;
        float vv = ((float)(v.H - y) + 0.5f) / (float)v.H;
        ro = add(add(ld3(v.llc), scl(u, ld3(v.hor))), scl(vv, ld3(v.ver)));
        rd = unit(sub(ro, ld3(v.org)));
        return true;
    }
    const Rcp rW = rcp_setup((float)v.W), rH = rcp_setup((float)v.H);
    float u = div_fast((float)x + 0.5f, rW);
    float vv = div_fast((float)(v.H - y) + 0.5f, rH);
    ro = add(add(ld3(v.llc), scl(u, ld3(v.hor))), scl(vv, ld3(v.ver)));
    const f3 c = sub(ro, ld3(v.org));
    const float len = sqrtf(c.x * c.x + c.y * c.y + c.z * c.z);
    const Rcp rl = rcp_setup(len);
    auto okn = [&](float n) { return __float_as_uint(n) == 0u || div_fast_ok(n, rl); };
    rd = f3{div_fast(c.x, rl), div_fast(c.y, rl), div_fast(c.z, rl)};
    VR_DIAG_COUNT_IF(!(okn(c.x) && okn(c.y) && okn(c.z)), 40);
    if (!(okn(c.x) && okn(c.y) && okn(c.z))) rd = f3{c.x / len, c.y / len, c.z / len};
    return true;
}

template <int STORE, bool COUNT, bool CRAWL>
__device__ __forceinline__ uint32_t light_and_shadow(Walker<STORE, COUNT, CRAWL>& w, const KView& v, const Hit& h) {
    bool sh = false;
    const f3 rwp = add(ld3(v.translation), mk((float)(h.region.x * kBlock), (float)(h.region.y * kBlock),
                                              (float)(h.region.z * kBlock)));
    const uint32_t lit = w.lighting(h.col, h.nc, rwp, h.so);
    if (v.use_shadows) {
        VR_DIAG_COUNT(16);
        w.lit_saved = lit;
        const bool eq = v.L[0] == v.L[1] && v.L[1] == v.L[2];
        if (h.longest) {
            w.ctx = 2u;
            sh = w.template shadow<true>(h.so, h.region);
        } else {
            sh = eq ? w.template shadow<false, true>(h.so, h.region) : w.template shadow<false>(h.so, h.region);
        }
    }
    return lit * (uint32_t)!sh;
}

__device__ __forceinline__ uint32_t defer_rewalk(const KView& v) {
    const uint32_t idx = atomicAdd(v.defer, 1u);
    deferral_report(v);
    if (idx < v.defer_cap) {
        uint32_t* r = v.defer + 4 + (size_t)idx * kDeferRecWords;
        r[0] = tile_pixels()[threadIdx.x];
        r[1] = 4u;
        r[8] = v.launch_id;
        return 0u;
    }
    atomicAdd(v.defer + 2, 1u);
    return kDeferMarker;
}

struct CrawlLds {
    uint32_t* lbm = nullptr;
};
template <class W>
__device__ __forceinline__ void attach(W& w, const CrawlLds* cl) {
    if (!cl) return;
    w.lbm = cl->lbm;
}

template <int STORE, int ALGO, bool COUNT, bool CRAWL>
__device__ __forceinline__ uint32_t shade(const KScene& s, const KView& v, uint32_t x, uint32_t l,
                                          uint32_t& bytes, uint32_t* iters = nullptr, uint2* ff = nullptr,
                                          uint32_t* dg = nullptr, const CrawlLds* cl = nullptr) {
    uint32_t col = 0;
    bytes = 0;
    if (ff) *ff = uint2{0u, 0u};
    f3 ro, rd;
    if (pixel_ray<true>(v, x, l, ro, rd)) {
        Walker<STORE, COUNT, CRAWL> w(s, v);
        attach(w, cl);
        Hit h;
        const bool hit = w.template primary<ALGO>(ro, rd, h);
        if (!CRAWL && v.pcost) tile_prim()[threadIdx.x] = w.iters;
        if (hit) col = light_and_shadow(w, v, h);
        if (iters) *iters = w.iters;
        bytes = w.bytes + 4u;
        if (ff) *ff = uint2{w.ff, w.nl};
#ifdef VR_CRAWL_PROF
        if (dg) { dg[0] = w.iters - w.ff; dg[1] = w.d_runs; dg[2] = w.d_trips; }
#endif
        if (w.aborted) {
            col = 0;
            if (ff) *ff = uint2{0u, 0u};
            if (Walker<STORE, COUNT, CRAWL>::kExact) {
                bytes = 4u;
            } else {
                bytes = 0u;
                if (w.iters != kDeferredIters) col = defer_rewalk(v);
            }
        }
    }
    return col;
}

template <int STORE, int ALGO, bool COUNT>
__device__ __forceinline__ uint32_t shade_resume(const KScene& s, const KView& v,
                                                 const uint32_t* r, uint32_t& bytes, uint2& ff,
                                                 uint32_t* dg = nullptr, const CrawlLds* cl = nullptr) {
    const uint32_t x = r[0] & 0xFFFFu, l = r[0] >> 16;
    Walker<STORE, COUNT, true> w(s, v);
    attach(w, cl);
    w.iters = r[9];
    w.bytes = r[10];
    const f3 o{__uint_as_float(r[2]), __uint_as_float(r[3]), __uint_as_float(r[4])};
    const i3 cr{(int32_t)r[5], (int32_t)r[6], (int32_t)r[7]};
    uint32_t col = 0;
    if (!(r[1] & 1u)) {
        f3 ro, rd;
        pixel_ray<true>(v, x, l, ro, rd);
        Hit h;
        if (w.template primary_regions<ALGO>(o, rd, cr, h, r)) col = light_and_shadow(w, v, h);
    } else {
        const bool eq = v.L[0] == v.L[1] && v.L[1] == v.L[2];
        bool sh;
        if (r[1] & 2u) sh = eq ? w.template shadow<true, true>(o, cr, r) : w.template shadow<true>(o, cr, r);
        else sh = eq ? w.template shadow<false, true>(o, cr, r) : w.template shadow<false>(o, cr, r);
        col = r[18] * (uint32_t)!sh;
    }
    bytes = w.bytes + 4u;
    ff = uint2{w.ff, w.nl};
#ifdef VR_CRAWL_PROF
    if (dg) { dg[0] = w.iters - r[9] - w.ff; dg[1] = w.d_runs; dg[2] = w.d_trips; }
#endif
    if (w.aborted) {
        col = 0;
        bytes = 4u;
        ff = uint2{0u, 0u};
    }
    return col;
}

__device__ __forceinline__ void add_bytes(const KView& v, uint32_t lane, unsigned long long b) {
    for (int off = 32; off > 0; off >>= 1) b += __shfl_down(b, off, 64);
    if (lane == 0 && b) atomicAdd(v.bytes, b);
}
__device__ __forceinline__ void add_ff(const KView& v, uint32_t lane, unsigned long long n, unsigned long long m) {
    for (int off = 32; off > 0; off >>= 1) {
        n += __shfl_down(n, off, 64);
        m += __shfl_down(m, off, 64);
    }
    if (lane == 0 && (n | m) && v.stats) {
        atomicAdd(v.stats, n);
        atomicAdd(v.stats + 1, 4ull * (n + m));
    }
}

#ifndef VR_ORIG_WAVES
#define VR_ORIG_WAVES 7
#endif
#ifndef VR_LONG_WAVES
#define VR_LONG_WAVES 6
#endif
#ifndef VR_ORIG_WAVES_HI
#define VR_ORIG_WAVES_HI 7
#endif
#ifndef VR_LONG_WAVES_HI
#define VR_LONG_WAVES_HI 6
#endif
constexpr bool kLongHiVariant = VR_LONG_WAVES_HI != VR_LONG_WAVES;
constexpr bool kOrigHiVariant = VR_ORIG_WAVES_HI != VR_ORIG_WAVES;
template <int ALGO, bool HI> struct TileWaves {
    static constexpr int value = ALGO == ALGO_ORIGINAL ? (HI ? VR_ORIG_WAVES_HI : VR_ORIG_WAVES)
                                                       : (HI ? VR_LONG_WAVES_HI : VR_LONG_WAVES);
};
static_assert(kTilesX * kTilesY == kWavesPerTileGroup, "cost layout (vr_internal.h)");
template <int STORE, int ALGO, bool COUNT, bool HI = false>
__global__ __launch_bounds__(64 * kTilesX * kTilesY, (TileWaves<ALGO, HI>::value)) void march_kernel(KScene s, KView v) {
    const uint32_t lane = threadIdx.x & 63u, wave = threadIdx.x >> 6;
    uint32_t x, l;
    lane_pixel(v, x, l);
    tile_pixels()[threadIdx.x] = (l << 16) | x;
    if (v.pcost) tile_prim()[threadIdx.x] = 0u;
    uint32_t bytes = 0, iters = 0;
    if (x < v.LW && l < v.local_rows) {
        const uint32_t c = shade<STORE, ALGO, COUNT, false>(s, v, x, l, bytes, &iters);
        asm volatile("" ::: "memory");
        const uint32_t p = tile_pixels()[threadIdx.x];
        const size_t at = (size_t)(p >> 16) * v.LW + (p & 0xFFFFu);
        v.out[at] = c;
        if (v.pcost) {
            const uint32_t p0 = tile_prim()[threadIdx.x];
            v.pcost[at] = min(p0, 0xFFFFu) << 16 | min(iters - p0, 0xFFFFu);
        }
    }
    if (COUNT) add_bytes(v, lane, bytes);
    if (v.cost) {
        for (int off = 32; off > 0; off >>= 1) iters = max(iters, (uint32_t)__shfl_xor((int)iters, off, 64));
        if (lane == 0) {
            uint32_t bx, by;
            tile_group(v, bx, by);
            v.cost[(by * gridDim.x + bx) * kWavesPerTileGroup + wave] = iters;
        }
    }
}

constexpr uint32_t kLaneShift = kLanePixels == 256 ? 8u : kLanePixels == 512 ? 9u : 10u;
template <bool DESCENDING>
__device__ __forceinline__ uint32_t wave_sort(uint32_t key, uint32_t lane) {
    for (uint32_t size = 2; size <= 64u; size <<= 1) {
        for (uint32_t stride = size >> 1; stride > 0; stride >>= 1) {
            const uint32_t other = (uint32_t)__shfl_xor((int)key, (int)stride, 64);
            const bool keep_max = (((lane & stride) == 0u) == ((lane & size) == 0u)) == DESCENDING;
            key = keep_max ? max(key, other) : min(key, other);
        }
    }
    return key;
}
__device__ __forceinline__ uint32_t lane_morton(uint32_t px, uint32_t py) {
    auto spread4 = [](uint32_t v) {
        v = (v | v << 2) & 0x33u;
        return (v | v << 1) & 0x55u;
    };
    return spread4(px & 15u) | spread4(py & 15u) << 1 | (px >> 4) << 8 | (py >> 4) << 9;
}
__global__ __launch_bounds__(kLanePixels) void perm_kernel(const uint32_t* __restrict__ pcost, uint32_t LW,
                                                           uint32_t rows, uint32_t gx, uint32_t gy,
                                                           uint8_t* __restrict__ perm, uint32_t* __restrict__ cost) {
    constexpr uint32_t kWaves = kLanePixels / 64u, kTiles = (kLaneBlockX / 8u) * (kLaneBlockY / 8u);
    __shared__ uint32_t sorted[kLanePixels];
    __shared__ __attribute__((aligned(16))) PermT slots[kLanePixels];
    __shared__ uint32_t wmax[2u * kWaves];
    __shared__ uint32_t ps[kLanePixels];
    static_assert(kTiles == kWaves, "one 8x8 tile per wave slot");
    const uint32_t t = threadIdx.x, lane = t & 63u, wave = t >> 6;
    const uint32_t nbx = (gx + kLbX - 1u) / kLbX, BX = blockIdx.x % nbx, BY = blockIdx.x / nbx;
    const uint32_t px = t % kLaneBlockX, py = t / kLaneBlockX;
    const uint32_t x = BX * kLaneBlockX + px, l = BY * kLaneBlockY + py;
    uint32_t p = 0, s = 0;
    if (x < LW && l < rows) {
        const uint32_t w = pcost[(size_t)l * LW + x];
        p = w >> 16;
        s = w & 0xFFFFu;
    }
    const uint32_t c = min(max(p, s) + ((p + s) >> 3), (1u << (32u - kLaneShift)) - 1u);
    if (cost) {
        if (t < 2u * kWaves) wmax[t] = 0u;
        ps[t] = p << 16 | s;
    }
    if ((BX + 1u) * kLbX > gx || (BY + 1u) * kLbY > gy) {
        if (cost) {
            __syncthreads();
            const uint32_t ti = (py >> 3) * (kLaneBlockX / 8u) + (px >> 3);
            atomicMax(&wmax[ti], p);
            atomicMax(&wmax[kWaves + ti], s);
            __syncthreads();
            if (t < kTiles) {
                const uint32_t tx = t % (kLaneBlockX / 8u), ty = t / (kLaneBlockX / 8u);
                const uint32_t col = BX * kLbX + tx / kTilesX, row = BY * kLbY + ty;
                if (col < gx && row < gy)
                    cost[(row * gx + col) * kWavesPerTileGroup + tx % kTilesX] = wmax[t] + wmax[kWaves + t];
            }
        }
        return;
    }
    const uint32_t key = wave_sort<true>((c << kLaneShift) | t, lane);
    sorted[t] = key;
    __syncthreads();
    uint32_t rank = lane;
#pragma unroll
    for (uint32_t o = 1; o < kWaves; ++o) {
        const uint32_t* sw = sorted + (((wave + o) % kWaves) << 6);
        uint32_t lo = 0;
#pragma unroll
        for (uint32_t step = 32; step > 0; step >>= 1)
            if (sw[lo + step - 1u] > key) lo += step;
        rank += lo + (sw[63] > key ? 1u : 0u);
    }
    const uint32_t pix = key & (kLanePixels - 1u);
    slots[rank] = (PermT)pix;
    if (cost) {
        const uint32_t w = ps[pix];
        atomicMax(&wmax[rank >> 6], w >> 16);
        atomicMax(&wmax[kWaves + (rank >> 6)], w & 0xFFFFu);
    }
    __syncthreads();
    if (cost && t < kWaves) {
        const uint32_t g = t / kTilesX;
        const uint32_t col = BX * kLbX + g % kLbX, row = BY * kLbY + g / kLbX;
        cost[(row * gx + col) * kWavesPerTileGroup + t % kTilesX] = wmax[t] + wmax[kWaves + t];
    }
    if (kLaneSeat == 1u) {
        const uint32_t q = slots[t];
        const uint32_t k = wave_sort<false>(lane_morton(q % kLaneBlockX, q / kLaneBlockX) << kLaneShift | q, lane);
        slots[t] = (PermT)(k & (kLanePixels - 1u));
        __syncthreads();
    }
    constexpr uint32_t kWords = kLanePixels * sizeof(PermT) / 4u;
    uint32_t* out = reinterpret_cast<uint32_t*>(perm + (size_t)blockIdx.x * kLanePixels * sizeof(PermT));
    if (t < kWords) out[t] = reinterpret_cast<const uint32_t*>(slots)[t];
}

constexpr uint32_t kOrderClasses = 128;
__global__ __launch_bounds__(1024) void order_kernel(const uint32_t* __restrict__ cost, uint32_t n, uint32_t columns,
                                                     uint32_t* __restrict__ order) {
    __shared__ uint32_t cnt[kOrderClasses];
    if (threadIdx.x < kOrderClasses) cnt[threadIdx.x] = 0u;
    __syncthreads();
    auto cls = [&](uint32_t i) {
        uint32_t c = 0;
#pragma unroll
        for (uint32_t w = 0; w < kWavesPerTileGroup; ++w) c = max(c, cost[i * kWavesPerTileGroup + w]);
        return kOrderClasses - 1u - min(kOrderClasses - 1u, c >> 2);
    };
    for (uint32_t i = threadIdx.x; i < n; i += blockDim.x) atomicAdd(&cnt[cls(i)], 1u);
    __syncthreads();
    if (threadIdx.x == 0) {
        uint32_t run = 0;
        for (uint32_t k = 0; k < kOrderClasses; ++k) {
            const uint32_t c = cnt[k];
            cnt[k] = run;
            run += c;
        }
    }
    __syncthreads();
    for (uint32_t i = threadIdx.x; i < n; i += blockDim.x) order[atomicAdd(&cnt[cls(i)], 1u)] = (i / columns) << 16 | (i % columns);
}

#ifndef VR_CRAWL_RPW
#define VR_CRAWL_RPW 4
#endif
constexpr uint32_t kCrawlRpw = VR_CRAWL_RPW;
#ifndef VR_CRAWL_MAX_RPW
#define VR_CRAWL_MAX_RPW 32
#endif
constexpr uint32_t kCrawlMaxRpw = VR_CRAWL_MAX_RPW;
constexpr uint32_t kCrawlWaves = 2;
constexpr uint32_t kCrawlLdsWords = 4u + kCrawlWaves * kCrawlMaxRpw * 16u;
template <int STORE, int ALGO, bool COUNT>
__global__ __launch_bounds__(64 * kCrawlWaves) void crawl_kernel(KScene s, KView v) {
    __shared__ __attribute__((aligned(16))) uint32_t dyn[kCrawlLdsWords];
    if (threadIdx.x == 0) {
        dyn[0] = v.defer[0];
        dyn[1] = v.defer[2];
    }
    __syncthreads();
    const uint32_t total = dyn[0], overflow = dyn[1];
    if (blockIdx.x == 0 && threadIdx.x == 0) {
        if (v.defer_stat) *v.defer_stat = total + overflow;
        if (v.slot_stat) *reinterpret_cast<uint2*>(v.slot_stat) = uint2{v.launch_id, total + overflow};
    }
    if (total == 0u && overflow == 0u) return;
    const uint32_t n = min(total, v.defer_cap);
    CrawlLds cl;
    unsigned long long bytes = 0, ffs = 0, nls = 0;
    const uint32_t rpw = v.crawl_rpw ? v.crawl_rpw : kCrawlRpw;
    const uint32_t wave = (blockIdx.x * blockDim.x + threadIdx.x) >> 6, wlane = threadIdx.x & 63u;
    const uint32_t nwaves = (gridDim.x * blockDim.x) >> 6;
    if (STORE == STORE_VCS && s.vcs_cbits && rpw <= kCrawlMaxRpw && wlane < rpw)
        cl.lbm = dyn + 4 + ((threadIdx.x >> 6) * kCrawlMaxRpw + wlane) * 16u;
    for (uint32_t i = wave * rpw + wlane; wlane < rpw && i < n; i += nwaves * rpw) {
        uint32_t* r = v.defer + 4 + (size_t)i * kDeferRecWords;
        if (r[8] != v.launch_id) continue;
        uint32_t b;
        const uint32_t x = r[0] & 0xFFFFu, l = r[0] >> 16;
        bool amb = (r[1] & 4u) != 0u;
        if (!amb) {
            f3 d = ld3(v.L);
            if (!(r[1] & 1u)) {
                f3 ro;
                pixel_ray<true>(v, x, l, ro, d);
            }
            const f3 o{__uint_as_float(r[2]), __uint_as_float(r[3]), __uint_as_float(r[4])};
#pragma unroll 1
            for (uint32_t a = 0; a < 3u; ++a) {
                int32_t qa;
                amb |= !crawl_voxel(comp(o, a), kEps * comp(d, a), qa);
                r[15 + a] = (uint32_t)qa;
            }
        }
        uint2 f{0u, 0u};
#ifdef VR_CRAWL_PROF
        uint32_t dg[3] = {0, 0, 0};
        const long long c0 = clock64(), t0 = wall_clock64();
        v.out[(size_t)l * v.LW + x] = amb ? shade<STORE, ALGO, COUNT, true>(s, v, x, l, b, nullptr, &f, dg, &cl)
                                         : shade_resume<STORE, ALGO, COUNT>(s, v, r, b, f, dg, &cl);
        const long long c1 = clock64(), t1 = wall_clock64();
        if (i < 16384u) {
            g_vr_crawl_prof[8 * i + 0] = (uint32_t)min(c1 - c0, 0xFFFFFFFFll);
            g_vr_crawl_prof[8 * i + 1] = dg[0] | (amb ? 0x80000000u : 0u);
            g_vr_crawl_prof[8 * i + 2] = dg[1];
            g_vr_crawl_prof[8 * i + 3] = dg[2];
            g_vr_crawl_prof[8 * i + 4] = (uint32_t)t0;
            g_vr_crawl_prof[8 * i + 5] = (uint32_t)t1;
        }
#else
        v.out[(size_t)l * v.LW + x] = amb ? shade<STORE, ALGO, COUNT, true>(s, v, x, l, b, nullptr, &f, nullptr, &cl)
                                         : shade_resume<STORE, ALGO, COUNT>(s, v, r, b, f, nullptr, &cl);
#endif
        bytes += b;
        ffs += f.x;
        nls += f.y;
    }
    if (overflow != 0u) {
        const size_t npx = (size_t)v.local_rows * v.LW;
        for (size_t i = (size_t)blockIdx.x * blockDim.x + threadIdx.x; i < npx; i += (size_t)gridDim.x * blockDim.x) {
            if (v.out[i] != kDeferMarker) continue;
            uint32_t b;
            uint2 f{0u, 0u};
            const CrawlLds clo;
            v.out[i] = shade<STORE, ALGO, COUNT, true>(s, v, (uint32_t)(i % v.LW), (uint32_t)(i / v.LW), b, nullptr, &f,
                                                       nullptr, &clo);
            bytes += b;
            ffs += f.x;
            nls += f.y;
        }
    }
    if (COUNT) {
        add_bytes(v, threadIdx.x & 63u, bytes);
        add_ff(v, threadIdx.x & 63u, ffs, nls);
    }
    __syncthreads();
    if (threadIdx.x == 0 && atomicAdd(&v.defer[1], 1u) == gridDim.x - 1u) {
        v.defer[0] = 0;
        v.defer[1] = 0;
        v.defer[2] = 0;
    }
}

constexpr uint32_t kPickThreads = 256;
template <int STORE, int ALGO>
__global__ __launch_bounds__(kPickThreads) void pick_kernel(KScene s, KView v, const uint32_t* __restrict__ px,
                                                           const uint32_t* __restrict__ py, uint32_t n,
                                                           uint4* __restrict__ hits) {
    const uint32_t i = blockIdx.x * kPickThreads + threadIdx.x;
    if (i >= n) return;
    const uint32_t x = px[i], y = py[i];
    uint4 r0{kPickOutside, 0u, 0u, 0u}, r1{0u, 0u, 0u, 0u}, r2{0u, 0u, 0u, 0u}, r3{0u, 0u, 0u, 0u};
    f3 ro, rd;
    if (x < v.W && y < v.H && pixel_ray<true>(v, x, y, ro, rd)) {
        Walker<STORE, false, true, true> w(s, v);
        Hit h;
        const bool hit = w.template primary<ALGO>(ro, rd, h);
        r0.x = w.aborted ? kPickNever : (hit ? kPickVoxel : kPickMiss);
        if (hit && !w.aborted) {
            const uint32_t key = ((uint32_t)w.pv.x << 20) | ((uint32_t)w.pv.y << 10) | (uint32_t)w.pv.z;
            const f3 nrm = w.normal_of(h.nc);
            r0.y = h.col;
            r0.z = (uint32_t)(h.region.x * kBlock) + (key >> 20);
            r0.w = (uint32_t)(h.region.y * kBlock) + ((key >> 10) & 1023u);
            r1.x = (uint32_t)(h.region.z * kBlock) + (key & 1023u);
            r1.y = (uint32_t)(int32_t)nrm.x;
            r1.z = (uint32_t)(int32_t)nrm.y;
            r1.w = (uint32_t)(int32_t)nrm.z;
            r2 = uint4{(uint32_t)h.region.x, (uint32_t)h.region.y, (uint32_t)h.region.z, __float_as_uint(h.so.x)};
            r3 = uint4{__float_as_uint(h.so.y), __float_as_uint(h.so.z), 0u, 0u};
        }
    }
    uint4* rec = hits + (size_t)i * 4u;
    rec[0] = r0;
    rec[1] = r1;
    rec[2] = r2;
    rec[3] = r3;
}

template <int STORE, int ALGO>
__global__ __launch_bounds__(kPickThreads) void trace_kernel(KScene s, KView v, const float4* __restrict__ rays,
                                                            const uint32_t* __restrict__ idx, uint32_t n,
                                                            uint4* __restrict__ hits) {
    const uint32_t i = blockIdx.x * kPickThreads + threadIdx.x;
    if (i >= n) return;
    const uint32_t r = idx ? idx[i] : i;
    const float4 a = rays[(size_t)r * 2u], b = rays[(size_t)r * 2u + 1u];
    uint4 r0{kPickMiss, 0u, 0u, 0u}, r1{0u, 0u, 0u, 0u}, r2{0u, 0u, 0u, 0u}, r3{0u, 0u, 0u, 0u};
    {
        Walker<STORE, false, true, true> w(s, v);
        Hit h;
        const bool hit = w.template primary<ALGO>(f3{a.x, a.y, a.z}, unit(f3{b.x, b.y, b.z}), h);
        r0.x = w.aborted ? kPickNever : (hit ? kPickVoxel : kPickMiss);
        if (hit && !w.aborted) {
            const uint32_t key = ((uint32_t)w.pv.x << 20) | ((uint32_t)w.pv.y << 10) | (uint32_t)w.pv.z;
            const f3 nrm = w.normal_of(h.nc);
            r0.y = h.col;
            r0.z = (uint32_t)(h.region.x * kBlock) + (key >> 20);
            r0.w = (uint32_t)(h.region.y * kBlock) + ((key >> 10) & 1023u);
            r1.x = (uint32_t)(h.region.z * kBlock) + (key & 1023u);
            r1.y = (uint32_t)(int32_t)nrm.x;
            r1.z = (uint32_t)(int32_t)nrm.y;
            r1.w = (uint32_t)(int32_t)nrm.z;
            r2 = uint4{(uint32_t)h.region.x, (uint32_t)h.region.y, (uint32_t)h.region.z, __float_as_uint(h.so.x)};
            r3 = uint4{__float_as_uint(h.so.y), __float_as_uint(h.so.z), 0u, 0u};
        }
    }
    uint4* rec = hits + (size_t)r * 4u;
    rec[0] = r0;
    rec[1] = r1;
    rec[2] = r2;
    rec[3] = r3;
}

__global__ __launch_bounds__(kPickThreads) void camera_rays_kernel(KView v, const uint32_t* __restrict__ px,
                                                                  const uint32_t* __restrict__ py, uint32_t n,
                                                                  uint4* __restrict__ rays) {
    const uint32_t i = blockIdx.x * kPickThreads + threadIdx.x;
    if (i >= n) return;
    const uint32_t x = px[i], y = py[i];
    constexpr uint32_t kNaN = 0x7FC00000u;
    uint4 o{kNaN, kNaN, kNaN, 0u}, d{kNaN, kNaN, kNaN, 0u};
    f3 ro, rd;
    if (x < v.W && y < v.H && pixel_ray<true>(v, x, y, ro, rd)) {
        const f3 c = sub(ro, ld3(v.org));
        o = uint4{__float_as_uint(ro.x), __float_as_uint(ro.y), __float_as_uint(ro.z), 0u};
        d = uint4{__float_as_uint(c.x), __float_as_uint(c.y), __float_as_uint(c.z), 0u};
    }
    rays[(size_t)i * 2u] = o;
    rays[(size_t)i * 2u + 1u] = d;
}

__global__ void cluster_bits_kernel(const uint2* __restrict__ mask, uint32_t n_regions, uint32_t* __restrict__ cbits) {
    const uint32_t t = blockIdx.x * blockDim.x + threadIdx.x;
    if (t >= n_regions * 16u) return;
    const uint2* m = mask + (size_t)(t >> 4) * 8192u + (size_t)(t & 15u) * 32u * 16u;
    uint32_t b = 0;
    for (uint32_t k = 0; k < 32u; ++k) b |= (m[k * 16u].y != kNone ? 1u : 0u) << k;
    cbits[t] = b;
}

__global__ void hash_filter_kernel(const uint4* __restrict__ meta, const uint2* __restrict__ slots,
                                   uint32_t* __restrict__ filter) {
    using F = Ctx<STORE_VCS, false, kTileBudget>;
    const uint4 m = meta[blockIdx.x];
    uint32_t* f = filter + (size_t)blockIdx.x * kHashFilterWords;
    for (uint32_t i = threadIdx.x; i < 2u * m.y; i += blockDim.x) {
        const uint32_t k = slots[m.x + i].x;
        if (k == kEmpty) continue;
        const uint32_t x = (k >> 20) & 63u, y = (k >> 10) & 63u, z = k & 63u;
        atomicOr(&f[F::word_index(x, y, z)], 1u << (F::word_bit5(y, z) & 31u));
    }
}

__global__ void pack_rgb8_kernel(const uint32_t* __restrict__ w, uint8_t* __restrict__ rgb, uint64_t n) {
    uint64_t i = (uint64_t)blockIdx.x * blockDim.x + threadIdx.x;
    if (i >= n) return;
    uint32_t c = w[i];
    rgb[3 * i + 0] = (uint8_t)(c >> 16);
    rgb[3 * i + 1] = (uint8_t)((c >> 8) & 0xFFu);
    rgb[3 * i + 2] = (uint8_t)(c & 0xFFu);
}

template <int E>
__global__ void assemble_tiles_kernel(const uint8_t* __restrict__ parts, uint8_t* __restrict__ frame, TileLayout t) {
    const uint64_t i = (uint64_t)blockIdx.x * blockDim.x + threadIdx.x;
    if (i >= (uint64_t)t.W * t.H) return;
    const uint32_t y = (uint32_t)(i / t.W), x = (uint32_t)(i - (uint64_t)y * t.W);
    const uint32_t b = y / t.band_rows, j = x / t.tile_cols, in_blk = x - j * t.tile_cols;
    const uint32_t rank = (j + t.stride * (b % t.R)) % t.R;
    const uint64_t lx = (uint64_t)(j / t.R) * t.tile_cols + in_blk;
    const uint64_t src = (uint64_t)rank * t.rank_words + (uint64_t)y * t.LW + lx;
#pragma unroll
    for (int k = 0; k < E; ++k) frame[i * E + k] = parts[src * E + k];
}

}

uint32_t crawl_grid(uint32_t records, uint32_t rpw) {
    const uint32_t waves_per_wg = kCrawlWaves;
    rpw = rpw ? rpw : kCrawlRpw;
    const uint64_t waves = ((uint64_t)records * 5u / 4u + rpw - 1u) / rpw;
    const uint64_t wgs = (waves + waves_per_wg - 1u) / waves_per_wg;
    return (uint32_t)std::min<uint64_t>(std::max<uint64_t>(wgs, 64u), 4096u);
}

#ifdef VR_NO_CRAWL_PASS
constexpr bool kNoCrawlPass = true;
#else
constexpr bool kNoCrawlPass = false;
#endif

void march_grid(const KView& v, uint32_t& columns, uint32_t& rows) {
    columns = (v.LW + 8u * kTilesX - 1u) / (8u * kTilesX);
    rows = (v.local_rows + 8u * kTilesY - 1u) / (8u * kTilesY);
}

size_t perm_bytes(uint32_t gx, uint32_t gy) {
    return (size_t)((gx + kLbX - 1u) / kLbX) * ((gy + kLbY - 1u) / kLbY) * kLanePixels * sizeof(PermT);
}

LaneShape lane_shape() {
    return {kLaneBlockX, kLaneBlockY, (uint32_t)sizeof(PermT), kLaneSeat};
}

hipError_t launch_perm(const uint32_t* pcost, uint32_t LW, uint32_t rows, uint32_t gx, uint32_t gy, uint8_t* perm,
                       uint32_t* cost, hipStream_t stream) {
    const uint32_t nb = ((gx + kLbX - 1u) / kLbX) * ((gy + kLbY - 1u) / kLbY);
    if (nb == 0) return hipSuccess;
    hipLaunchKernelGGL(perm_kernel, dim3(nb), dim3(kLanePixels), 0, stream, pcost, LW, rows, gx, gy, perm, cost);
    return hipGetLastError();
}

hipError_t launch_order(const uint32_t* cost, uint32_t n, uint32_t columns, uint32_t* order, hipStream_t stream) {
    if (n == 0) return hipSuccess;
    hipLaunchKernelGGL(order_kernel, dim3(1), dim3(1024), 0, stream, cost, n, columns, order);
    return hipGetLastError();
}

hipError_t launch_march(int store, int algo, bool count, const KScene& s, const KView& v, hipStream_t stream,
                        uint32_t crawl_wgs, bool in_flight, bool crawl) {
    uint32_t gx, gy;
    march_grid(v, gx, gy);
    dim3 grid(gx, gy);
    dim3 block(64u * kTilesX * kTilesY);
    if (grid.x == 0 || grid.y == 0) return hipSuccess;
    const dim3 cgrid(crawl_wgs ? crawl_wgs : 64u);
    const dim3 cblock(64u * kCrawlWaves);
#define VR_LAUNCH(ST, AL, CT) VR_LAUNCH_HI(ST, AL, CT, false)
#define VR_LAUNCH_HI(ST, AL, CT, HI)                                                              \
    do {                                                                                           \
        hipLaunchKernelGGL((march_kernel<ST, AL, CT, HI>), grid, block, 0, stream, s, v);          \
        if (v.defer && crawl && !kNoCrawlPass)                                                     \
            hipLaunchKernelGGL((crawl_kernel<ST, AL, CT>), cgrid, cblock, 0, stream, s, v);        \
    } while (0)
#ifdef VR_ISA_ONLY
#ifndef VR_ISA_STORE
#define VR_ISA_STORE STORE_VCS
#endif
    (void)algo; (void)count; (void)store;
    if (in_flight) VR_LAUNCH_HI(VR_ISA_STORE, VR_ISA_ONLY, false, true);
    else VR_LAUNCH(VR_ISA_STORE, VR_ISA_ONLY, false);
#else
    const bool hi = in_flight && !count;
    if (store == STORE_VCS) {
        if (algo == ALGO_ORIGINAL) { if (count) VR_LAUNCH(STORE_VCS, ALGO_ORIGINAL, true); else VR_LAUNCH(STORE_VCS, ALGO_ORIGINAL, false); }
        else if (hi && kLongHiVariant) VR_LAUNCH_HI(STORE_VCS, ALGO_LONGEST, false, true);
        else { if (count) VR_LAUNCH(STORE_VCS, ALGO_LONGEST, true); else VR_LAUNCH(STORE_VCS, ALGO_LONGEST, false); }
    } else {
        if (algo == ALGO_ORIGINAL) {
            if (hi && kOrigHiVariant) VR_LAUNCH_HI(STORE_HASH, ALGO_ORIGINAL, false, true);
            else if (count) VR_LAUNCH(STORE_HASH, ALGO_ORIGINAL, true);
            else VR_LAUNCH(STORE_HASH, ALGO_ORIGINAL, false);
        }
        else { if (count) VR_LAUNCH(STORE_HASH, ALGO_LONGEST, true); else VR_LAUNCH(STORE_HASH, ALGO_LONGEST, false); }
    }
#endif
#undef VR_LAUNCH
#undef VR_LAUNCH_HI
    return hipGetLastError();
}

hipError_t launch_pick(int store, int algo, const KScene& s, const KView& v, const uint32_t* px, const uint32_t* py,
                       uint32_t n, void* hits, hipStream_t stream) {
    if (n == 0) return hipSuccess;
    const dim3 grid((n + kPickThreads - 1u) / kPickThreads), block(kPickThreads);
    uint4* out = static_cast<uint4*>(hits);
#define VR_PICK(ST, AL) hipLaunchKernelGGL((pick_kernel<ST, AL>), grid, block, 0, stream, s, v, px, py, n, out)
    if (store == STORE_VCS) {
        if (algo == ALGO_ORIGINAL) VR_PICK(STORE_VCS, ALGO_ORIGINAL); else VR_PICK(STORE_VCS, ALGO_LONGEST);
    } else {
        if (algo == ALGO_ORIGINAL) VR_PICK(STORE_HASH, ALGO_ORIGINAL); else VR_PICK(STORE_HASH, ALGO_LONGEST);
    }
#undef VR_PICK
    return hipGetLastError();
}

hipError_t launch_trace(int store, int algo, const KScene& s, const KView& v, const void* rays, const uint32_t* idx,
                        uint32_t n, void* hits, hipStream_t stream) {
    if (n == 0) return hipSuccess;
    const dim3 grid((n + kPickThreads - 1u) / kPickThreads), block(kPickThreads);
    const float4* in = static_cast<const float4*>(rays);
    uint4* out = static_cast<uint4*>(hits);
#define VR_TRACE(ST, AL) hipLaunchKernelGGL((trace_kernel<ST, AL>), grid, block, 0, stream, s, v, in, idx, n, out)
    if (store == STORE_VCS) {
        if (algo == ALGO_ORIGINAL) VR_TRACE(STORE_VCS, ALGO_ORIGINAL); else VR_TRACE(STORE_VCS, ALGO_LONGEST);
    } else {
        if (algo == ALGO_ORIGINAL) VR_TRACE(STORE_HASH, ALGO_ORIGINAL); else VR_TRACE(STORE_HASH, ALGO_LONGEST);
    }
#undef VR_TRACE
    return hipGetLastError();
}

hipError_t launch_camera_rays(const KView& v, const uint32_t* px, const uint32_t* py, uint32_t n, void* rays,
                              hipStream_t stream) {
    if (n == 0) return hipSuccess;
    hipLaunchKernelGGL(camera_rays_kernel, dim3((n + kPickThreads - 1u) / kPickThreads), dim3(kPickThreads), 0, stream, v,
                       px, py, n, static_cast<uint4*>(rays));
    return hipGetLastError();
}

hipError_t launch_cluster_bits(const uint2* vcs_mask, uint32_t n_regions, uint32_t* cbits, hipStream_t stream) {
    if (n_regions == 0) return hipSuccess;
    const uint32_t threads = n_regions * 16u;
    hipLaunchKernelGGL(cluster_bits_kernel, dim3((threads + 255u) / 256u), dim3(256), 0, stream, vcs_mask, n_regions,
                       cbits);
    return hipGetLastError();
}

hipError_t launch_assemble_tiles(const void* parts, void* frame, uint32_t elem_bytes, const TileLayout& t,
                                 hipStream_t stream) {
    const uint64_t n = (uint64_t)t.W * t.H;
    if (n == 0) return hipSuccess;
    const dim3 grid((unsigned)((n + 255) / 256)), block(256);
    const uint8_t* p = static_cast<const uint8_t*>(parts);
    uint8_t* f = static_cast<uint8_t*>(frame);
    switch (elem_bytes) {
    case 1: hipLaunchKernelGGL(assemble_tiles_kernel<1>, grid, block, 0, stream, p, f, t); break;
    case 2: hipLaunchKernelGGL(assemble_tiles_kernel<2>, grid, block, 0, stream, p, f, t); break;
    case 3: hipLaunchKernelGGL(assemble_tiles_kernel<3>, grid, block, 0, stream, p, f, t); break;
    default: hipLaunchKernelGGL(assemble_tiles_kernel<4>, grid, block, 0, stream, p, f, t); break;
    }
    return hipGetLastError();
}

hipError_t launch_hash_filter(const uint4* ht_meta, const uint2* ht_slots, uint32_t n_regions, uint32_t* filter,
                              hipStream_t stream) {
    if (n_regions == 0) return hipSuccess;
    hipLaunchKernelGGL(hash_filter_kernel, dim3(n_regions), dim3(256), 0, stream, ht_meta, ht_slots, filter);
    return hipGetLastError();
}

hipError_t launch_pack_rgb8(const uint32_t* words, uint8_t* rgb, uint64_t n, hipStream_t stream) {
    if (n == 0) return hipSuccess;
    hipLaunchKernelGGL(pack_rgb8_kernel, dim3((unsigned)((n + 255) / 256)), dim3(256), 0, stream, words, rgb, n);
    return hipGetLastError();
}

}

#ifdef VR_CRAWL_PROF
extern "C" int vr_crawl_prof_fetch(unsigned int* out, unsigned int n) {
    if (hipDeviceSynchronize() != hipSuccess) return -1;
    if (hipMemcpyFromSymbol(out, HIP_SYMBOL(g_vr_crawl_prof), sizeof(unsigned int) * 8 * (n < 16384u ? n : 16384u)) !=
        hipSuccess)
        return -1;
    return 0;
}
#endif
#ifdef VR_DIAG
extern "C" int vr_diag_fetch(uint64_t* out, int reset) {
    static_assert(sizeof(uint64_t) == sizeof(unsigned long long), "counter width");
    if (hipDeviceSynchronize() != hipSuccess) return -1;
    if (hipMemcpyFromSymbol(out, HIP_SYMBOL(g_vr_diag), sizeof(unsigned long long) * 64) != hipSuccess) return -1;
    if (reset) {
        unsigned long long z[64] = {0};
        if (hipMemcpyToSymbol(HIP_SYMBOL(g_vr_diag), z, sizeof z) != hipSuccess) return -1;
    }
    return 0;
}
#endif
```

voxelraymarcher_amd/renderer.py:

```python
from __future__ import annotations

import ctypes
import enum
from ctypes import c_int32, c_size_t, c_uint32, c_void_p
from dataclasses import dataclass, field

import numpy as np
import torch

from . import _capi
from ._capi import check, f3, lib


class StorageType(enum.IntEnum):
    VOXEL_CLUSTER_STORE = _capi.VR_STORE_VCS
    HASH_TABLE = _capi.VR_STORE_HASHTABLE


class RayMarchAlgorithm(enum.IntEnum):
    LONGEST_AXIS = _capi.VR_ALGO_LONGESTAXIS
    ORIGINAL = _capi.VR_ALGO_ORIGINAL


def parse_storage(name: str) -> StorageType:
# ... 245 lines not shown

class Kernel(enum.IntEnum):
    AUTO = _capi.VR_KERNEL_AUTO
    TILE = _capi.VR_KERNEL_TILE
    TILE_REWALK = _capi.VR_KERNEL_TILE_REWALK


class Schedule(enum.IntEnum):
    AUTO = _capi.VR_SCHEDULE_AUTO
    GRID = _capi.VR_SCHEDULE_GRID
    HEAVIEST_FIRST = _capi.VR_SCHEDULE_HEAVIEST_FIRST


class Occupancy(enum.IntEnum):
    AUTO = _capi.VR_OCCUPANCY_AUTO
    LONE = _capi.VR_OCCUPANCY_LONE
    IN_FLIGHT = _capi.VR_OCCUPANCY_IN_FLIGHT


def render_ex(scene: DeviceScene, algorithm: RayMarchAlgorithm, camera: Camera, lighting: _capi.VrLighting,
              info: VoxelSceneInfo, width: int, height: int, out: torch.Tensor, row_begin: int = 0,
              row_end: int | None = None, band_rows: int = 0, rank: int = 0, nranks: int = 1,
              counter: torch.Tensor | None = None, kernel: Kernel = Kernel.AUTO, stream=None,
              defer_cap: int = 0, schedule: Schedule = Schedule.AUTO,
              stats: torch.Tensor | None = None, occupancy: Occupancy = Occupancy.AUTO,
              tile_cols: int = 0, deal_stride: int = 0) -> torch.Tensor:
    row_end = height if row_end is None else row_end
    rows = row_end - row_begin
    if tile_cols:
        words = tile_buffer_words(width, rows, band_rows or max(1, rows), tile_cols, nranks)
    else:
        words = band_buffer_words(width, rows, band_rows or max(1, rows), nranks)
    _require_u32(out, words)
    for name, t in (("counter", counter), ("stats", stats)):
        if t is not None and (not t.is_cuda or t.dtype != torch.int64):
            raise TypeError(f"{name} must be a CUDA int64 tensor")
    if stats is not None and (counter is None or stats.numel() < 2 or not stats.is_contiguous()):
        raise ValueError("stats needs a counter and 2 contiguous int64 elements")
    opts = _capi.VrRenderOpts()
    check(lib().vr_render_opts_init(ctypes.byref(opts)), "vr_render_opts_init")
    opts.kernel, opts.row_begin, opts.row_end = int(kernel), int(row_begin), int(row_end)
    opts.band_rows, opts.rank, opts.nranks = int(band_rows), int(rank), int(nranks)
    opts.bytes_dev = c_void_p(counter.data_ptr()) if counter is not None else None
    opts.defer_cap, opts.schedule = int(defer_cap), int(schedule)
    opts.stats_dev = c_void_p(stats.data_ptr()) if stats is not None else None
    opts.occupancy, opts.tile_cols, opts.deal_stride = int(occupancy), int(tile_cols), int(deal_stride)
    check(lib().vr_render_ex(scene.handle, int(algorithm), ctypes.byref(camera.raw), ctypes.byref(lighting),
                             f3(info.translation), int(info.scale), int(width), int(height), ctypes.byref(opts),
                             c_void_p(out.data_ptr()), _stream_ptr(stream)), "vr_render_ex")
    return out


class PreparedRender:
    vr_stream_arg = True

    def __init__(self, scene: DeviceScene, algorithm: RayMarchAlgorithm, camera: Camera,
                 lighting: _capi.VrLighting, info: VoxelSceneInfo, width: int, height: int, row_begin: int = 0,
                 row_end: int | None = None, band_rows: int = 0, rank: int = 0, nranks: int = 1,
                 kernel: Kernel = Kernel.AUTO, schedule: Schedule = Schedule.AUTO,
                 occupancy: Occupancy = Occupancy.AUTO, tile_cols: int = 0, deal_stride: int = 0):
        row_end = height if row_end is None else row_end
        rows = row_end - row_begin
        if tile_cols:
            self.words = tile_buffer_words(width, rows, band_rows or max(1, rows), tile_cols, nranks)
        else:
            self.words = band_buffer_words(width, rows, band_rows or max(1, rows), nranks)
        opts = _capi.VrRenderOpts()
        check(lib().vr_render_opts_init(ctypes.byref(opts)), "vr_render_opts_init")
        opts.kernel, opts.row_begin, opts.row_end = int(kernel), int(row_begin), int(row_end)
        opts.band_rows, opts.rank, opts.nranks = int(band_rows), int(rank), int(nranks)
        opts.schedule, opts.occupancy = int(schedule), int(occupancy)
        opts.tile_cols, opts.deal_stride = int(tile_cols), int(deal_stride)
        self._keep = (scene, camera, lighting, opts, f3(info.translation))
        self._fn = lib().vr_render_ex
        self._args = (scene.handle, int(algorithm), ctypes.byref(camera.raw), ctypes.byref(lighting),
                      self._keep[4], int(info.scale), int(width), int(height), ctypes.byref(opts))
        self._checked = set()

    def __call__(self, out: torch.Tensor, stream=None) -> torch.Tensor:
        key = (out.data_ptr(), out.numel(), out.dtype, out.is_contiguous())
        if key not in self._checked:
            _require_u32(out, self.words)
            if len(self._checked) >= 64:
                self._checked.clear()
            self._checked.add(key)
        sh = (stream if stream is not None else torch.cuda.current_stream()).cuda_stream
        rc = self._fn(*self._args, c_void_p(key[0]), c_void_p(sh))
        if rc:
            check(rc, "vr_render_ex")
        return out


def run_raymarching_kernel(scene: DeviceScene, algorithm: RayMarchAlgorithm, camera: Camera,
                           lighting: _capi.VrLighting, info: VoxelSceneInfo, width: int, height: int,
                           out: torch.Tensor | None = None, row_begin: int = 0, row_end: int | None = None,
                           stream=None, kernel: Kernel = Kernel.AUTO) -> torch.Tensor:
    row_end = height if row_end is None else row_end
    words = (row_end - row_begin) * width
    if out is None:
        out = torch.empty(words, dtype=torch.int32, device=f"cuda:{scene.info()['device']}")
    if kernel == Kernel.AUTO:
        _require_u32(out, words)
        check(lib().vr_render(scene.handle, int(algorithm), ctypes.byref(camera.raw), ctypes.byref(lighting),
                              f3(info.translation), int(info.scale), int(width), int(height), int(row_begin),
                              int(row_end), c_void_p(out.data_ptr()), _stream_ptr(stream)), "vr_render")
        return out
    return render_ex(scene, algorithm, camera, lighting, info, width, height, out, row_begin, row_end,
                     kernel=kernel, stream=stream)


def render_count(scene: DeviceScene, algorithm: RayMarchAlgorithm, camera: Camera, lighting: _capi.VrLighting,
                 info: VoxelSceneInfo, width: int, height: int, out: torch.Tensor, counter: torch.Tensor,
                 row_begin: int = 0, row_end: int | None = None, stream=None,
                 kernel: Kernel = Kernel.AUTO) -> None:
    render_ex(scene, algorithm, camera, lighting, info, width, height, out, row_begin, row_end,
              counter=counter, kernel=kernel, stream=stream)


class HitStatus(enum.IntEnum):
    MISS = _capi.VR_HIT_MISS
    VOXEL = _capi.VR_HIT_VOXEL
    NEVER = _capi.VR_HIT_NEVER
    OUTSIDE = _capi.VR_HIT_OUTSIDE


HIT_DTYPE = np.dtype([("status", "<u4"), ("color", "<u4"), ("voxel", "<i4", (3,)), ("normal", "<i4", (3,)),
                      ("region", "<i4", (3,)), ("point", "<f4", (3,)), ("reserved", "<u4", (2,))])
assert HIT_DTYPE.itemsize == ctypes.sizeof(_capi.VrHit) == 64


def pick(scene: DeviceScene, algorithm: RayMarchAlgorithm, camera: Camera, info: VoxelSceneInfo, width: int,
         height: int, px, py, stream=None):
    sp = _stream_ptr(stream)
    args = (scene.handle, int(algorithm), ctypes.byref(camera.raw), f3(info.translation), int(info.scale), int(width),
            int(height))
    if hasattr(px, "is_cuda") and px.is_cuda:
        if not (hasattr(py, "is_cuda") and py.is_cuda) or px.device != py.device:
            raise TypeError("px and py must both be CUDA tensors on one device")
        for t in (px, py):
            if t.dtype not in (torch.int32, torch.uint32):
                raise TypeError("px/py must be int32 or uint32 tensors")
        px, py = px.contiguous().reshape(-1), py.contiguous().reshape(-1)
        if px.shape[0] != py.shape[0]:
            raise ValueError("px and py lengths differ")
        n = px.shape[0]
        hits = torch.empty((n, 16), dtype=torch.int32, device=px.device)
        if n:
            check(lib().vr_pick(*args, c_void_p(px.data_ptr()), c_void_p(py.data_ptr()), n, 1,
                                c_void_p(hits.data_ptr()), 1, sp), "vr_pick")
        return hits
    px = np.ascontiguousarray(px, dtype=np.uint32).reshape(-1)
    py = np.ascontiguousarray(py, dtype=np.uint32).reshape(-1)
    if px.shape[0] != py.shape[0]:
        raise ValueError("px and py lengths differ")
    n = px.shape[0]
    hits = np.zeros(n, dtype=HIT_DTYPE)
    if n:
        check(lib().vr_pick(*args, px.ctypes.data_as(c_void_p), py.ctypes.data_as(c_void_p), n, 0,
                            hits.ctypes.data_as(c_void_p), 0, sp), "vr_pick")
    return hits


class TraceOrder(enum.IntEnum):
    AUTO = _capi.VR_TRACE_ORDER_AUTO
    GIVEN = _capi.VR_TRACE_ORDER_GIVEN
    COHERENT = _capi.VR_TRACE_ORDER_COHERENT


RAY_DTYPE = np.dtype([("origin", "<f4", (3,)), ("reserved0", "<u4"), ("direction", "<f4", (3,)), ("reserved1", "<u4")])
assert RAY_DTYPE.itemsize == ctypes.sizeof(_capi.VrRay) == 32


def _rays_numpy(rays) -> np.ndarray:
    if isinstance(rays, np.ndarray) and rays.dtype == RAY_DTYPE:
        return np.ascontiguousarray(rays).reshape(-1)
    a = np.asarray(rays, dtype=np.float32)
    if a.size == 0:
        return np.zeros(0, dtype=RAY_DTYPE)
    if a.ndim != 2 or a.shape[1] != 6:
        raise ValueError("rays must be a RAY_DTYPE array or an (n, 6) array: origin, direction")
    out = np.zeros(a.shape[0], dtype=RAY_DTYPE)
    out["origin"], out["direction"] = a[:, :3], a[:, 3:]
    return out


def trace(scene: DeviceScene, algorithm: RayMarchAlgorithm, info: VoxelSceneInfo, rays,
          order: TraceOrder = TraceOrder.AUTO, stream=None):
    sp = _stream_ptr(stream)
    args = (scene.handle, int(algorithm), f3(info.translation), int(info.scale))
    if hasattr(rays, "is_cuda") and rays.is_cuda:
        if rays.dtype != torch.float32 or rays.dim() != 2 or rays.shape[1] not in (6, 8):
            raise TypeError("rays must be a float32 CUDA tensor of shape (n, 8) or (n, 6)")
        if rays.shape[1] == 6:
            full = torch.zeros((rays.shape[0], 8), dtype=torch.float32, device=rays.device)
            full[:, 0:3], full[:, 4:7] = rays[:, 0:3], rays[:, 3:6]
            rays = full
        rays = rays.contiguous()
        n = rays.shape[0]
        hits = torch.empty((n, 16), dtype=torch.int32, device=rays.device)
        if n:
            check(lib().vr_trace(*args, c_void_p(rays.data_ptr()), n, 1, c_void_p(hits.data_ptr()), 1, int(order), sp),
                  "vr_trace")
        return hits
    rays = _rays_numpy(rays)
    n = rays.shape[0]
    hits = np.zeros(n, dtype=HIT_DTYPE)
    if n:
        check(lib().vr_trace(*args, rays.ctypes.data_as(c_void_p), n, 0, hits.ctypes.data_as(c_void_p), 0, int(order),
                             sp), "vr_trace")
    return hits


def camera_rays(camera: Camera, width: int, height: int, px, py, device: int = 0, stream=None):
    sp = _stream_ptr(stream)
    args = (int(device), ctypes.byref(camera.raw), int(width), int(height))
    if hasattr(px, "is_cuda") and px.is_cuda:
        if not (hasattr(py, "is_cuda") and py.is_cuda) or px.device != py.device:
            raise TypeError("px and py must both be CUDA tensors on one device")
        for t in (px, py):
            if t.dtype not in (torch.int32, torch.uint32):
                raise TypeError("px/py must be int32 or uint32 tensors")
        px, py = px.contiguous().reshape(-1), py.contiguous().reshape(-1)
        if px.shape[0] != py.shape[0]:
            raise ValueError("px and py lengths differ")
        n = px.shape[0]
        rays = torch.empty((n, 8), dtype=torch.float32, device=px.device)
        if n:
            check(lib().vr_camera_rays(*args, c_void_p(px.data_ptr()), c_void_p(py.data_ptr()), n, 1,
                                       c_void_p(rays.data_ptr()), 1, sp), "vr_camera_rays")
        return rays
    px = np.ascontiguousarray(px, dtype=np.uint32).reshape(-1)
    py = np.ascontiguousarray(py, dtype=np.uint32).reshape(-1)
    if px.shape[0] != py.shape[0]:
        raise ValueError("px and py lengths differ")
    n = px.shape[0]
    rays = np.zeros(n, dtype=RAY_DTYPE)
    if n:
        check(lib().vr_camera_rays(*args, px.ctypes.data_as(c_void_p), py.ctypes.data_as(c_void_p), n, 0,
                                   rays.ctypes.data_as(c_void_p), 0, sp), "vr_camera_rays")
    return rays


def band_buffer_words(width: int, height: int, band_rows: int, nranks: int) -> int:
    return int(lib().vr_band_buffer_words(width, height, band_rows, nranks))


def render_bands(scene: DeviceScene, algorithm: RayMarchAlgorithm, camera: Camera, lighting: _capi.VrLighting,
                 info: VoxelSceneInfo, width: int, height: int, band_rows: int, rank: int, nranks: int,
                 out: torch.Tensor, stream=None) -> torch.Tensor:
    _require_u32(out, band_buffer_words(width, height, band_rows, nranks))
    check(lib().vr_render_bands(scene.handle, int(algorithm), ctypes.byref(camera.raw), ctypes.byref(lighting),
                                f3(info.translation), int(info.scale), int(width), int(height), int(band_rows),
                                int(rank), int(nranks), c_void_p(out.data_ptr()), _stream_ptr(stream)),
          "vr_render_bands")
    return out


def tile_buffer_words(width: int, height: int, band_rows: int, tile_cols: int, nranks: int) -> int:
    return int(lib().vr_tile_buffer_words(width, height, band_rows, tile_cols, nranks))


def deal_stride_default(nranks: int) -> int:
    return int(lib().vr_deal_stride_default(nranks))


def forget_orders(device: int = 0) -> None:
    check(lib().vr_forget_orders(int(device)), "vr_forget_orders")


def debug_skip_next_crawl(device: int = 0) -> None:
    check(lib().vr_debug_skip_next_crawl(int(device)), "vr_debug_skip_next_crawl")


def debug_capture_lane_order(device: int = 0) -> None:
    check(lib().vr_debug_capture_lane_order(int(device)), "vr_debug_capture_lane_order")


def debug_lane_order(device: int = 0):
    import numpy as np
    raw = (ctypes.c_uint32 * 8)()
    check(lib().vr_debug_lane_order(int(device), raw, None, 0, None, 0), "vr_debug_lane_order")
    info = dict(zip(("LW", "rows", "gx", "gy", "block_x", "block_y", "entry_bytes", "seat"), (int(x) for x in raw)))
    n = info["block_x"] * info["block_y"]
    blocks = -(-info["LW"] // info["block_x"]) * (-(-info["rows"] // info["block_y"]))
    pcost = np.empty((info["rows"], info["LW"]), dtype=np.uint32)
    perm = np.empty((blocks, n), dtype=np.uint8 if info["entry_bytes"] == 1 else np.uint16)
    check(lib().vr_debug_lane_order(int(device), raw, c_void_p(pcost.ctypes.data), pcost.size,
                                    c_void_p(perm.ctypes.data), perm.nbytes), "vr_debug_lane_order")
    return info, pcost, perm


ORDER_USES = ("launches", "lane_orders_made", "lane_order_uses", "work_orders_made", "work_order_uses",
              "crawl_skips", "slots", "lane_block")


def debug_order_uses(device: int = 0) -> dict:
    raw = (ctypes.c_uint64 * 8)()
    check(lib().vr_debug_order_uses(int(device), raw), "vr_debug_order_uses")
    d = dict(zip(ORDER_USES, (int(x) for x in raw)))
    d["lane_block"] = (d["lane_block"] >> 16, d["lane_block"] & 0xFFFF)
    return d


def render_tiles(scene: DeviceScene, algorithm: RayMarchAlgorithm, camera: Camera, lighting: _capi.VrLighting,
                 info: VoxelSceneInfo, width: int, height: int, band_rows: int, tile_cols: int, rank: int,
                 nranks: int, out: torch.Tensor, stream=None) -> torch.Tensor:
    _require_u32(out, tile_buffer_words(width, height, band_rows, tile_cols, nranks))
    check(lib().vr_render_tiles(scene.handle, int(algorithm), ctypes.byref(camera.raw), ctypes.byref(lighting),
                                f3(info.translation), int(info.scale), int(width), int(height), int(band_rows),
                                int(tile_cols), int(rank), int(nranks), c_void_p(out.data_ptr()),
                                _stream_ptr(stream)), "vr_render_tiles")
    return out


def assemble_tiles_device(parts: torch.Tensor, frame: torch.Tensor, elem_bytes: int, width: int, height: int,
                          band_rows: int, tile_cols: int, nranks: int, deal_stride: int = 0,
                          stream=None) -> torch.Tensor:
    need = tile_buffer_words(width, height, band_rows, tile_cols, nranks) * nranks * elem_bytes
    for name, t, n in (("parts", parts, need), ("frame", frame, width * height * elem_bytes)):
        if not t.is_cuda or not t.is_contiguous() or t.numel() * t.element_size() < n:
            raise ValueError(f"{name} must be a contiguous CUDA tensor of >= {n} bytes")
    check(lib().vr_assemble_tiles(c_void_p(parts.data_ptr()), c_void_p(frame.data_ptr()), int(elem_bytes),
                                  int(width), int(height), int(band_rows), int(tile_cols), int(nranks),
                                  int(deal_stride), _stream_ptr(stream)), "vr_assemble_tiles")
    return frame


def pack_rgb8(words: torch.Tensor, stream=None, out: torch.Tensor | None = None) -> torch.Tensor:
    rgb = torch.empty(words.numel() * 3, dtype=torch.uint8, device=words.device) if out is None else out
    if rgb.dtype != torch.uint8 or rgb.numel() != words.numel() * 3 or not rgb.is_contiguous():
        raise ValueError("out must be a contiguous uint8 tensor of 3 x words.numel() bytes")
    check(lib().vr_pack_rgb8(c_void_p(words.data_ptr()), c_void_p(rgb.data_ptr()), words.numel(),
                             _stream_ptr(stream)), "vr_pack_rgb8")
    return rgb


@dataclass
class RenderConfig:
    name: str
    grid: int
    p_region: float
    p_cluster: float
    p_voxel: float
    seed: int
    width: int
    height: int
    store: StorageType
    algorithm: RayMarchAlgorithm
    gpus: int = 1
    notes: str = ""
    scale: int = field(init=False)

    def __post_init__(self):
        self.scale = 3 * self.grid // 16

    def voxels(self):
        return synth_scene(self.grid, self.p_region, self.p_cluster, self.p_voxel, self.seed)


CONFIGS = {
    "C1": RenderConfig("C1", 64, 1.0, 0.5, 0.10, 0x1, 256, 256, StorageType.HASH_TABLE, RayMarchAlgorithm.ORIGINAL,
                       notes="scene.vox 64^3, hashtable+original (host-CPU plumbing config)"),
    "C2": RenderConfig("C2", 256, 1.0, 0.30, 0.08, 0x256, 1920, 1080, StorageType.VOXEL_CLUSTER_STORE,
                       RayMarchAlgorithm.ORIGINAL, notes="256^3 synthetic, vcs+original"),
    "C3": RenderConfig("C3", 256, 1.0, 0.30, 0.08, 0x256, 1920, 1080, StorageType.VOXEL_CLUSTER_STORE,
                       RayMarchAlgorithm.LONGEST_AXIS, notes="256^3 synthetic, vcs+longestaxis"),
    "C4": RenderConfig("C4", 512, 1.0, 1.0, 0.15, 0x512, 1920, 1080, StorageType.HASH_TABLE,
                       RayMarchAlgorithm.ORIGINAL, notes="512^3 dense, hashtable+original"),
    "C5": RenderConfig("C5", 1024, 0.35, 0.05, 0.25, 0x1024, 3840, 2160, StorageType.VOXEL_CLUSTER_STORE,
                       RayMarchAlgorithm.ORIGINAL, gpus=8, notes="1024^3 sparse, vcs+original, 8-GPU tiles"),
}
```

Before: 21940 Mrays/s.

## Make lane-order block shape selectable per occupancy mode and store

Templates the per-block lane permutation kernel over its block shape (16x16, 16x32, 16x64, 32x32) and keeps two permutation buffers, one for a lone launch and one for in-flight launches. The lone shape defaults to 16x16 and the in-flight shape to 16x32 for VCS (16x64 for hash table). Partial edge blocks are now sorted and permuted rather than skipped. The aim is to fit the cost-sorted ray grouping to the concurrency regime. In exchange it may build two permutations on a relane and adds more indexing logic.

```diff
diff --git a/include/vr.h b/include/vr.h
--- a/include/vr.h
+++ b/include/vr.h
@@ -189,6 +189,7 @@
 int vr_debug_lane_order(int device, uint32_t info[8], uint32_t* pcost, uint64_t pcost_words, uint8_t* perm,
                         uint64_t perm_bytes);
 int vr_debug_order_uses(int device, uint64_t out[8]);
+int vr_debug_lane_shape(int device, uint32_t lone, uint32_t in_flight);
 int vr_render_ex(const vr_scene* s, vr_algo algo, const vr_camera* cam, const vr_lighting* lit,
                  const float translation[3], uint32_t scale, uint32_t width, uint32_t height,
                  const vr_render_opts* opts, uint32_t* out_dev, void* stream);
diff --git a/voxelraymarcher_amd/__init__.py b/voxelraymarcher_amd/__init__.py
--- a/voxelraymarcher_amd/__init__.py
+++ b/voxelraymarcher_amd/__init__.py
@@ -3,7 +3,7 @@
 from .renderer import (CONFIGS, HIT_DTYPE, VOXEL_REMOVE, Build, HitStatus, Camera, DeviceScene, Kernel, Occupancy, PreparedRender, RayMarchAlgorithm,
                        RenderConfig,
                        Schedule, StorageType, VoxelSceneCPU, VoxelSceneInfo, assemble_tiles_device, band_buffer_words,
-                       create_scene, deal_stride_default, debug_capture_lane_order, debug_lane_order, debug_order_uses, debug_skip_next_crawl,
+                       create_scene, deal_stride_default, debug_capture_lane_order, debug_lane_order, debug_lane_shape, debug_order_uses, debug_skip_next_crawl,
                        forget_orders, pack_rgb8, pick, parse_algorithm, parse_storage, RAY_DTYPE, TraceOrder, camera_rays, trace,
                        read_voxel_file, render_bands, render_count, render_ex, render_tiles, run_raymarching_kernel,
                        setup_constant_values, synth_scene, tile_buffer_words, write_binary_scene, write_voxel_file)
@@ -12,7 +12,7 @@
            "VOXEL_REMOVE", "Build", "pick", "RAY_DTYPE", "TraceOrder", "camera_rays", "trace",
            "Camera", "DeviceScene", "Kernel", "Occupancy", "PreparedRender", "RayMarchAlgorithm", "RenderConfig", "Schedule",
            "StorageType", "VoxelSceneCPU", "VoxelSceneInfo", "assemble_tiles_device", "band_buffer_words",
-           "create_scene", "deal_stride_default", "debug_capture_lane_order", "debug_lane_order", "debug_order_uses",
+           "create_scene", "deal_stride_default", "debug_capture_lane_order", "debug_lane_order", "debug_lane_shape", "debug_order_uses",
            "debug_skip_next_crawl", "forget_orders", "pack_rgb8", "parse_algorithm", "parse_storage",
            "read_voxel_file", "render_bands", "render_count", "render_ex", "render_tiles", "run_raymarching_kernel",
            "setup_constant_values", "synth_scene", "tile_buffer_words", "write_binary_scene", "write_voxel_file"]
diff --git a/voxelraymarcher_amd/_capi.py b/voxelraymarcher_amd/_capi.py
--- a/voxelraymarcher_amd/_capi.py
+++ b/voxelraymarcher_amd/_capi.py
@@ -102,6 +102,7 @@
     "vr_debug_capture_lane_order": (c_int, [c_int]),
     "vr_debug_lane_order": (c_int, [c_int, POINTER(c_uint32), c_void_p, c_uint64, c_void_p, c_uint64]),
     "vr_debug_order_uses": (c_int, [c_int, POINTER(c_uint64)]),
+    "vr_debug_lane_shape": (c_int, [c_int, c_uint32, c_uint32]),
     "vr_assemble_tiles": (c_int, [c_void_p, c_void_p, c_uint32, c_uint32, c_uint32, c_uint32, c_uint32, c_uint32,
                                   c_uint32, c_void_p]),
     "vr_render_ex": (c_int, [c_void_p, c_int, POINTER(VrCamera), POINTER(VrLighting), POINTER(c_float), c_uint32,
diff --git a/voxelraymarcher_amd/csrc/vr_internal.h b/voxelraymarcher_amd/csrc/vr_internal.h
--- a/voxelraymarcher_amd/csrc/vr_internal.h
+++ b/voxelraymarcher_amd/csrc/vr_internal.h
@@ -63,6 +63,7 @@
     uint32_t* pcost;
     uint32_t* slot_stat;
     uint32_t launch_id;
+    uint16_t lane_lx, lane_ly;
 };
 static_assert(sizeof(KView) - offsetof(KView, out) == 104,
               "a KView field was added after `out`: review whether it belongs to the view identity");
@@ -96,12 +97,12 @@
 void march_grid(const KView& v, uint32_t& columns, uint32_t& rows);
 constexpr uint32_t kWavesPerTileGroup = 2;
 hipError_t launch_order(const uint32_t* cost, uint32_t n, uint32_t columns, uint32_t* order, hipStream_t stream);
-size_t perm_bytes(uint32_t gx, uint32_t gy);
-struct LaneShape {
-    uint32_t block_x, block_y, entry_bytes, seat;
+size_t perm_bytes(uint32_t shape, uint32_t gx, uint32_t gy);
+struct LaneLayout {
+    uint32_t entry_bytes, seat;
 };
-LaneShape lane_shape();
-hipError_t launch_perm(const uint32_t* pcost, uint32_t LW, uint32_t rows, uint32_t gx, uint32_t gy, uint8_t* perm,
-                       uint32_t* cost, hipStream_t stream);
+LaneLayout lane_layout();
+hipError_t launch_perm(uint32_t shape, const uint32_t* pcost, uint32_t LW, uint32_t rows, uint32_t gx, uint32_t gy,
+                       uint8_t* perm, uint32_t* cost, hipStream_t stream);
 
 }
diff --git a/voxelraymarcher_amd/csrc/vr_launch.cpp b/voxelraymarcher_amd/csrc/vr_launch.cpp
--- a/voxelraymarcher_amd/csrc/vr_launch.cpp
+++ b/voxelraymarcher_amd/csrc/vr_launch.cpp
@@ -79,9 +79,17 @@
 bool order_enabled() { static const bool on = env_flag("VR_ORDER", true); return on; }
 bool lane_order_enabled() { static const bool on = env_flag("VR_LANE_ORDER", true); return on; }
 bool crawl_skip_enabled() { static const bool on = env_flag("VR_CRAWL_SKIP", true); return on; }
+uint32_t env_lane(const char* name) {
+    const char* e = std::getenv(name);
+    unsigned w = 0, h = 0;
+    if (!e || std::sscanf(e, "%ux%u", &w, &h) != 2 || w > 0xFFFFu || h > 0xFFFFu) return 0;
+    const uint32_t s = vr::lane_shape(w, h);
+    return vr::lane_shape_ok(s) ? s : 0;
+}
 const vr::PolicyKnobs& policy_knobs() {
     static const vr::PolicyKnobs k = {env_flag("VR_INFLIGHT_HEAVY", false), env_flag("VR_INFLIGHT_WAVES", true),
-                                      env_uint("VR_CRAWL_RPW", 1, 64, 0), env_uint("VR_CRAWL_RPW_IN_FLIGHT", 1, 64, 32)};
+                                      env_uint("VR_CRAWL_RPW", 1, 64, 0), env_uint("VR_CRAWL_RPW_IN_FLIGHT", 1, 64, 32),
+                                      env_lane("VR_LONE_LANE"), env_lane("VR_INFLIGHT_LANE")};
     return k;
 }
 
@@ -107,11 +115,13 @@
         hipStream_t last_stream = nullptr;
         uint32_t last_idx = 0;
         uint64_t last_key = 0;
+        bool prev_alone = true;
         bool force_skip = false;
+        uint32_t force_lane[2] = {0, 0};
         uint64_t uses[6] = {0, 0, 0, 0, 0, 0};
         bool capture_lane = false;
         struct LaneCapture {
-            uint32_t LW = 0, rows = 0, gx = 0, gy = 0;
+            uint32_t LW = 0, rows = 0, gx = 0, gy = 0, shape = 0;
             std::vector<uint32_t> pcost;
             std::vector<uint8_t> perm;
         } lane_capture;
@@ -255,19 +265,26 @@
     return hipSuccess;
 }
 
-hipError_t bind_lane_order(vr::LaneOrder& L, uint32_t gx, uint32_t gy, uint64_t key, bool repeat, hipStream_t st,
-                           vr::KView& v, bool& relane, const char*& what) {
-    const size_t nperm = vr::perm_bytes(gx, gy);
-    if (nperm > L.bcap) {
-        L.bcap = 0;
+hipError_t bind_lane_order(vr::LaneOrder& L, const uint32_t shapes[2], bool in_flight, uint32_t gx, uint32_t gy,
+                           uint64_t key, bool repeat, hipStream_t st, vr::KView& v, bool& relane, const char*& what) {
+    for (uint32_t i = 0; i < 2u; ++i) {
+        if (i == 1u && shapes[1] == shapes[0]) break;
+        const size_t nperm = vr::perm_bytes(shapes[i], gx, gy);
+        if (nperm <= L.bcap[i]) continue;
+        L.bcap[i] = 0;
         L.valid = false;
         what = "lane order buffer";
-        const hipError_t e = regrow({{(void**)&L.perm, nperm}}, st);
+        const hipError_t e = regrow({{(void**)&L.perm[i], nperm}}, st);
         if (e != hipSuccess) return e;
-        L.bcap = nperm;
-    }
-    const bool match = L.matches(gx, gy, key);
-    v.perm = match ? L.perm : nullptr;
+        L.bcap[i] = nperm;
+    }
+    const bool match = L.matches(gx, gy, key, shapes);
+    if (match) {
+        const uint32_t shape = shapes[in_flight ? 1 : 0];
+        v.perm = L.perm[L.index(in_flight)];
+        v.lane_lx = (uint16_t)vr::lane_lx(shape);
+        v.lane_ly = (uint16_t)vr::lane_ly(shape);
+    }
     relane = vr::remake_due(match, false, repeat, L.age, order_refresh());
     if (!relane) return hipSuccess;
     what = "lane order walk lengths";
@@ -355,7 +372,11 @@
     const uint32_t n = gx * gy;
     const bool alone = D.alone(st);
     VR_HP(2);
-    const vr::LaunchPolicy pol = vr::launch_policy(schedule, occupancy, alone, policy_knobs());
+    vr::PolicyKnobs knobs = policy_knobs();
+    if (D.force_lane[0]) knobs.lane_lone = D.force_lane[0];
+    if (D.force_lane[1]) knobs.lane_in_flight = D.force_lane[1];
+    const vr::LaunchPolicy pol = vr::launch_policy(schedule, occupancy, alone, knobs, (uint32_t)s->store, D.prev_alone);
+    D.prev_alone = alone;
     v.crawl_rpw = pol.crawl_rpw;
     const uint64_t key = view_key(s, algo, v);
     const bool repeat = D.follow(st, lease.idx, key);
@@ -368,7 +389,7 @@
     }
     if (lane_order_enabled() && n != 0) {
         const char* what = "";
-        e = bind_lane_order(S.lane, gx, gy, key, repeat, st, v, relane, what);
+        e = bind_lane_order(S.lane, pol.lane, pol.lane_in_flight, gx, gy, key, repeat, st, v, relane, what);
         if (e != hipSuccess) return bail(e, what);
     }
     VR_HP(4);
@@ -387,20 +408,25 @@
     VR_HP(7);
     bool with_costs = false;
     if (e == hipSuccess && relane) {
+        vr::LaneOrder& L = S.lane;
         with_costs = order_enabled() && S.work.cost && S.work.cap >= n;
-        e = vr::launch_perm(v.pcost, v.LW, v.local_rows, gx, gy, S.lane.perm, with_costs ? S.work.cost : nullptr, st);
-        S.lane.learned(gx, gy, key, e == hipSuccess);
+        e = vr::launch_perm(pol.lane[0], v.pcost, v.LW, v.local_rows, gx, gy, L.perm[0], with_costs ? S.work.cost : nullptr, st);
+        if (e == hipSuccess && pol.lane[1] != pol.lane[0])
+            e = vr::launch_perm(pol.lane[1], v.pcost, v.LW, v.local_rows, gx, gy, L.perm[1], nullptr, st);
+        L.shape[0] = pol.lane[0], L.shape[1] = pol.lane[1];
+        L.learned(gx, gy, key, e == hipSuccess);
         D.uses[1] += e == hipSuccess;
         S.work.relaned = !with_costs;
         if (e == hipSuccess && D.capture_lane) {
             D.capture_lane = false;
             SlotRing::Dev::LaneCapture& C = D.lane_capture;
-            C.LW = v.LW, C.rows = v.local_rows, C.gx = gx, C.gy = gy;
+            const uint32_t which = L.index(pol.lane_in_flight);
+            C.LW = v.LW, C.rows = v.local_rows, C.gx = gx, C.gy = gy, C.shape = L.shape[which];
             C.pcost.resize((size_t)v.LW * v.local_rows);
-            C.perm.resize(vr::perm_bytes(gx, gy));
+            C.perm.resize(vr::perm_bytes(C.shape, gx, gy));
             e = hipStreamSynchronize(st);
             if (e == hipSuccess) e = hipMemcpy(C.pcost.data(), v.pcost, sizeof(uint32_t) * C.pcost.size(), hipMemcpyDeviceToHost);
-            if (e == hipSuccess) e = hipMemcpy(C.perm.data(), S.lane.perm, C.perm.size(), hipMemcpyDeviceToHost);
+            if (e == hipSuccess) e = hipMemcpy(C.perm.data(), L.perm[which], C.perm.size(), hipMemcpyDeviceToHost);
         }
     }
     if (e == hipSuccess && (remake || with_costs)) {
@@ -730,11 +756,21 @@
     if (device < 0 || device >= 64) return fail(VR_E_INVALID, "device index out of range");
     if (!out) return fail(VR_E_INVALID, "out is NULL");
     SlotRing::Dev& D = g_defer_ring.dev[device];
-    const vr::LaneShape sh = vr::lane_shape();
     std::lock_guard<std::mutex> lk(D.mu);
     for (int i = 0; i < 6; ++i) out[i] = D.uses[i];
     out[6] = g_defer_ring.nslots;
-    out[7] = (uint64_t)sh.block_x << 16 | sh.block_y;
+    out[7] = vr::kLaneDefault;
+    return VR_OK;
+}
+
+int vr_debug_lane_shape(int device, uint32_t lone, uint32_t in_flight) {
+    if (device < 0 || device >= 64) return fail(VR_E_INVALID, "device index out of range");
+    if ((lone && !vr::lane_shape_ok(lone)) || (in_flight && !vr::lane_shape_ok(in_flight)))
+        return fail(VR_E_INVALID, "lane shape: 0, or width << 16 | height of 16x16, 16x32, 16x64 or 32x32");
+    SlotRing::Dev& D = g_defer_ring.dev[device];
+    std::lock_guard<std::mutex> lk(D.mu);
+    D.force_lane[0] = lone;
+    D.force_lane[1] = in_flight;
     return VR_OK;
 }
 
@@ -755,8 +791,8 @@
     std::lock_guard<std::mutex> lk(D.mu);
     const SlotRing::Dev::LaneCapture& C = D.lane_capture;
     if (C.perm.empty()) return fail(VR_E_INVALID, "no lane order captured (vr_debug_capture_lane_order, then a repeated view)");
-    const vr::LaneShape sh = vr::lane_shape();
-    const uint32_t words[8] = {C.LW, C.rows, C.gx, C.gy, sh.block_x, sh.block_y, sh.entry_bytes, sh.seat};
+    const vr::LaneLayout lay = vr::lane_layout();
+    const uint32_t words[8] = {C.LW, C.rows, C.gx, C.gy, C.shape >> 16, C.shape & 0xFFFFu, lay.entry_bytes, lay.seat};
     std::memcpy(info, words, sizeof words);
     if (pcost) {
         if (pcost_words != C.pcost.size()) return fail(VR_E_INVALID, "pcost_words is not info[0] * info[1]");
diff --git a/voxelraymarcher_amd/csrc/vr_launch_plan.h b/voxelraymarcher_amd/csrc/vr_launch_plan.h
--- a/voxelraymarcher_amd/csrc/vr_launch_plan.h
+++ b/voxelraymarcher_amd/csrc/vr_launch_plan.h
@@ -5,24 +5,49 @@
 
 #include "vr.h"
 
+#if defined(__HIPCC__)
+#define VR_PLAN_FN __host__ __device__ inline
+#else
+#define VR_PLAN_FN inline
+#endif
+
 namespace vr {
+
+constexpr uint32_t lane_shape(uint32_t w, uint32_t h) { return w << 16 | h; }
+constexpr uint32_t kLane16x16 = lane_shape(16, 16), kLane16x32 = lane_shape(16, 32), kLane16x64 = lane_shape(16, 64),
+                   kLane32x32 = lane_shape(32, 32);
+constexpr uint32_t kLaneDefault = kLane16x32;
+constexpr uint32_t kLaneLone = kLane16x16;
+constexpr uint32_t lane_in_flight_shape(uint32_t store) { return store == VR_STORE_HASHTABLE ? kLane16x64 : kLane16x32; }
+inline bool lane_shape_ok(uint32_t s) { return s == kLane16x16 || s == kLane16x32 || s == kLane16x64 || s == kLane32x32; }
+inline uint32_t lane_lx(uint32_t s) { return (s >> 16) == 32u ? 1u : 0u; }
+inline uint32_t lane_ly(uint32_t s) { return (s & 0xFFFFu) == 64u ? 3u : (s & 0xFFFFu) == 32u ? 2u : 1u; }
+inline uint32_t lane_pixels(uint32_t s) { return (s >> 16) * (s & 0xFFFFu); }
 
 struct PolicyKnobs {
     bool inflight_heavy;
     bool in_flight_occupancy;
     uint32_t rpw_override;
     uint32_t rpw_in_flight;
+    uint32_t lane_lone = 0;
+    uint32_t lane_in_flight = 0;
 };
 struct LaunchPolicy {
     bool heavy;
     bool hi;
     uint32_t crawl_rpw;
+    bool lane_in_flight;
+    uint32_t lane[2];
 };
-inline LaunchPolicy launch_policy(uint32_t schedule, uint32_t occupancy, bool alone, const PolicyKnobs& k) {
+inline LaunchPolicy launch_policy(uint32_t schedule, uint32_t occupancy, bool alone, const PolicyKnobs& k,
+                                  uint32_t store = VR_STORE_VCS, bool prev_alone = true) {
     LaunchPolicy p;
     p.heavy = schedule == VR_SCHEDULE_HEAVIEST_FIRST || (schedule == VR_SCHEDULE_AUTO && (alone || k.inflight_heavy));
     p.hi = occupancy == VR_OCCUPANCY_IN_FLIGHT || (occupancy == VR_OCCUPANCY_AUTO && !alone && k.in_flight_occupancy);
     p.crawl_rpw = k.rpw_override ? k.rpw_override : (alone ? 2u : k.rpw_in_flight);
+    p.lane_in_flight = occupancy == VR_OCCUPANCY_IN_FLIGHT || (occupancy == VR_OCCUPANCY_AUTO && !(alone && prev_alone));
+    p.lane[0] = lane_shape_ok(k.lane_lone) ? k.lane_lone : kLaneLone;
+    p.lane[1] = lane_shape_ok(k.lane_in_flight) ? k.lane_in_flight : lane_in_flight_shape(store);
     return p;
 }
 
@@ -48,9 +73,27 @@
     void forget() { valid = relaned = false; }
 };
 struct LaneOrder : Learned {
-    uint8_t* perm = nullptr;
-    size_t bcap = 0;
+    uint32_t shape[2] = {0, 0};
+    uint8_t* perm[2] = {nullptr, nullptr};
+    size_t bcap[2] = {0, 0};
+    bool matches(uint32_t x, uint32_t y, uint64_t k) const { return Learned::matches(x, y, k); }
+    bool matches(uint32_t x, uint32_t y, uint64_t k, const uint32_t want[2]) const {
+        return Learned::matches(x, y, k) && shape[0] == want[0] && shape[1] == want[1];
+    }
+    uint32_t index(bool in_flight) const { return in_flight && shape[1] != shape[0] ? 1u : 0u; }
 };
+
+VR_PLAN_FN uint32_t lane_weight(uint32_t p, uint32_t s) { return (p > s ? p : s) + ((p + s) >> 3); }
+VR_PLAN_FN uint32_t lane_key(uint32_t weight, uint32_t t, uint32_t shift, bool cut, bool in_frame, bool exists) {
+    const uint32_t top = (1u << (32u - shift)) - 1u;
+    uint32_t c = in_frame ? weight : 0u;
+    if (cut) c = in_frame ? (c < top - 2u ? c : top - 2u) + 2u : (exists ? 1u : 0u);
+    return (c < top ? c : top) << shift | t;
+}
+VR_PLAN_FN uint32_t lane_entry(uint32_t r, uint32_t ex, uint32_t lx) {
+    const uint32_t k = r >> 7, row = k / ex, col = k - row * ex;
+    return ((row << lx) + col) << 7 | (r & 127u);
+}
 
 inline uint32_t next_launch_id(uint32_t& serial) { return ++serial ? serial : ++serial; }
 
diff --git a/voxelraymarcher_amd/csrc/vr_march.hip b/voxelraymarcher_amd/csrc/vr_march.hip
--- a/voxelraymarcher_amd/csrc/vr_march.hip
+++ b/voxelraymarcher_amd/csrc/vr_march.hip
@@ -1,5 +1,6 @@
 #include "vr_device.h"
 #include "vr_crawl.h"
+#include "vr_launch_plan.h"
 
 #include <algorithm>
 #include <type_traits>
@@ -75,25 +76,7 @@
     }
 }
 
-#ifdef VR_LANE_BLOCK
-#define VR_LANE_BLOCK_DEFAULT_X VR_LANE_BLOCK
-#define VR_LANE_BLOCK_DEFAULT_Y VR_LANE_BLOCK
-#else
-#define VR_LANE_BLOCK_DEFAULT_X 16
-#define VR_LANE_BLOCK_DEFAULT_Y 32
-#endif
-#ifndef VR_LANE_BLOCK_X
-#define VR_LANE_BLOCK_X VR_LANE_BLOCK_DEFAULT_X
-#endif
-#ifndef VR_LANE_BLOCK_Y
-#define VR_LANE_BLOCK_Y VR_LANE_BLOCK_DEFAULT_Y
-#endif
-constexpr uint32_t kLaneBlockX = VR_LANE_BLOCK_X, kLaneBlockY = VR_LANE_BLOCK_Y;
-static_assert((kLaneBlockX == 16 || kLaneBlockX == 32) && (kLaneBlockY == 16 || kLaneBlockY == 32),
-              "lane block: 16 or 32 pixels a side");
-constexpr uint32_t kLanePixels = kLaneBlockX * kLaneBlockY;
-constexpr uint32_t kLbX = kLaneBlockX / (8u * kTilesX), kLbY = kLaneBlockY / (8u * kTilesY);
-using PermT = std::conditional<kLanePixels == 256, uint8_t, uint16_t>::type;
+using PermT = uint16_t;
 #ifndef VR_LANE_SEAT
 #define VR_LANE_SEAT 0
 #endif
@@ -104,13 +87,14 @@
     const uint32_t lane = threadIdx.x & 63u, wave = threadIdx.x >> 6;
     uint32_t bx, by;
     tile_group(v, bx, by);
-    const uint32_t BX = bx / kLbX, BY = by / kLbY;
-    if (kLaneOrder && v.perm && (BX + 1u) * kLbX <= gridDim.x && (BY + 1u) * kLbY <= gridDim.y) {
-        const uint32_t q = ((by % kLbY) * kLbX + bx % kLbX) * kTilesX + wave;
-        const uint32_t blk = BY * ((gridDim.x + kLbX - 1u) / kLbX) + BX;
-        const uint32_t p = reinterpret_cast<const PermT*>(v.perm)[(size_t)blk * kLanePixels + q * 64u + lane];
-        x = BX * kLaneBlockX + p % kLaneBlockX;
-        l = BY * kLaneBlockY + p / kLaneBlockX;
+    if (kLaneOrder && v.perm) {
+        const uint32_t lx = v.lane_lx, ly = v.lane_ly;
+        const uint32_t BX = bx >> lx, BY = by >> ly;
+        const uint32_t q = ((((by & ((1u << ly) - 1u)) << lx) + (bx & ((1u << lx) - 1u))) << 1) + wave;
+        const uint32_t blk = BY * ((gridDim.x + (1u << lx) - 1u) >> lx) + BX;
+        const uint32_t p = reinterpret_cast<const PermT*>(v.perm)[((size_t)blk << (7u + lx + ly)) + q * 64u + lane];
+        x = (BX << (4u + lx)) + (p & ((16u << lx) - 1u));
+        l = (BY << (3u + ly)) + (p >> (4u + lx));
     } else {
         x = (bx * kTilesX + wave % kTilesX) * 8u + (lane & 7u);
         l = (by * kTilesY + wave / kTilesX) * 8u + (lane >> 3);
@@ -1274,7 +1258,6 @@
     }
 }
 
-constexpr uint32_t kLaneShift = kLanePixels == 256 ? 8u : kLanePixels == 512 ? 9u : 10u;
 template <bool DESCENDING>
 __device__ __forceinline__ uint32_t wave_sort(uint32_t key, uint32_t lane) {
     for (uint32_t size = 2; size <= 64u; size <<= 1) {
@@ -1293,47 +1276,36 @@
     };
     return spread4(px & 15u) | spread4(py & 15u) << 1 | (px >> 4) << 8 | (py >> 4) << 9;
 }
-__global__ __launch_bounds__(kLanePixels) void perm_kernel(const uint32_t* __restrict__ pcost, uint32_t LW,
-                                                           uint32_t rows, uint32_t gx, uint32_t gy,
-                                                           uint8_t* __restrict__ perm, uint32_t* __restrict__ cost) {
-    constexpr uint32_t kWaves = kLanePixels / 64u, kTiles = (kLaneBlockX / 8u) * (kLaneBlockY / 8u);
-    __shared__ uint32_t sorted[kLanePixels];
-    __shared__ __attribute__((aligned(16))) PermT slots[kLanePixels];
+template <uint32_t LX, uint32_t LY>
+__global__ __launch_bounds__(128u << (LX + LY)) void perm_kernel(const uint32_t* __restrict__ pcost, uint32_t LW,
+                                                                  uint32_t rows, uint32_t gx, uint32_t gy,
+                                                                  uint8_t* __restrict__ perm, uint32_t* __restrict__ cost) {
+    static_assert(kTilesX == 2 && kTilesY == 1, "tile groups of 16x8 pixels, two wave slots each");
+    constexpr uint32_t kBlockX = 16u << LX, kPixels = 128u << (LX + LY), kShift = 7u + LX + LY;
+    constexpr uint32_t kWaves = kPixels / 64u, kGX = 1u << LX, kGY = 1u << LY;
+    __shared__ uint32_t sorted[kPixels];
+    __shared__ __attribute__((aligned(16))) PermT slots[kPixels];
     __shared__ uint32_t wmax[2u * kWaves];
-    __shared__ uint32_t ps[kLanePixels];
-    static_assert(kTiles == kWaves, "one 8x8 tile per wave slot");
+    __shared__ uint32_t ps[kPixels];
     const uint32_t t = threadIdx.x, lane = t & 63u, wave = t >> 6;
-    const uint32_t nbx = (gx + kLbX - 1u) / kLbX, BX = blockIdx.x % nbx, BY = blockIdx.x / nbx;
-    const uint32_t px = t % kLaneBlockX, py = t / kLaneBlockX;
-    const uint32_t x = BX * kLaneBlockX + px, l = BY * kLaneBlockY + py;
+    const uint32_t nbx = (gx + kGX - 1u) >> LX, BX = blockIdx.x % nbx, BY = blockIdx.x / nbx;
+    const uint32_t px = t & (kBlockX - 1u), py = t >> (4u + LX);
+    const uint32_t x = (BX << (4u + LX)) + px, l = (BY << (3u + LY)) + py;
+    const uint32_t ex = min(kGX, gx - (BX << LX)), ey = min(kGY, gy - (BY << LY));
+    const bool in_frame = x < LW && l < rows;
     uint32_t p = 0, s = 0;
-    if (x < LW && l < rows) {
+    if (in_frame) {
         const uint32_t w = pcost[(size_t)l * LW + x];
         p = w >> 16;
         s = w & 0xFFFFu;
     }
-    const uint32_t c = min(max(p, s) + ((p + s) >> 3), (1u << (32u - kLaneShift)) - 1u);
     if (cost) {
         if (t < 2u * kWaves) wmax[t] = 0u;
         ps[t] = p << 16 | s;
     }
-    if ((BX + 1u) * kLbX > gx || (BY + 1u) * kLbY > gy) {
-        if (cost) {
-            __syncthreads();
-            const uint32_t ti = (py >> 3) * (kLaneBlockX / 8u) + (px >> 3);
-            atomicMax(&wmax[ti], p);
-            atomicMax(&wmax[kWaves + ti], s);
-            __syncthreads();
-            if (t < kTiles) {
-                const uint32_t tx = t % (kLaneBlockX / 8u), ty = t / (kLaneBlockX / 8u);
-                const uint32_t col = BX * kLbX + tx / kTilesX, row = BY * kLbY + ty;
-                if (col < gx && row < gy)
-                    cost[(row * gx + col) * kWavesPerTileGroup + tx % kTilesX] = wmax[t] + wmax[kWaves + t];
-            }
-        }
-        return;
-    }
-    const uint32_t key = wave_sort<true>((c << kLaneShift) | t, lane);
+    slots[t] = 0;
+    const uint32_t key = wave_sort<true>(
+        lane_key(lane_weight(p, s), t, kShift, ex < kGX || ey < kGY, in_frame, (px >> 4) < ex && (py >> 3) < ey), lane);
     sorted[t] = key;
     __syncthreads();
     uint32_t rank = lane;
@@ -1346,27 +1318,30 @@
             if (sw[lo + step - 1u] > key) lo += step;
         rank += lo + (sw[63] > key ? 1u : 0u);
     }
-    const uint32_t pix = key & (kLanePixels - 1u);
-    slots[rank] = (PermT)pix;
-    if (cost) {
-        const uint32_t w = ps[pix];
-        atomicMax(&wmax[rank >> 6], w >> 16);
-        atomicMax(&wmax[kWaves + (rank >> 6)], w & 0xFFFFu);
+    const uint32_t pix = key & (kPixels - 1u);
+    if (rank < 128u * ex * ey) {
+        const uint32_t at = lane_entry(rank, ex, LX);
+        slots[at] = (PermT)pix;
+        if (cost) {
+            const uint32_t w = ps[pix];
+            atomicMax(&wmax[at >> 6], w >> 16);
+            atomicMax(&wmax[kWaves + (at >> 6)], w & 0xFFFFu);
+        }
     }
     __syncthreads();
     if (cost && t < kWaves) {
-        const uint32_t g = t / kTilesX;
-        const uint32_t col = BX * kLbX + g % kLbX, row = BY * kLbY + g / kLbX;
-        cost[(row * gx + col) * kWavesPerTileGroup + t % kTilesX] = wmax[t] + wmax[kWaves + t];
+        const uint32_t g = t / kTilesX, col = g & (kGX - 1u), row = g >> LX;
+        if (col < ex && row < ey)
+            cost[(((BY << LY) + row) * gx + (BX << LX) + col) * kWavesPerTileGroup + t % kTilesX] = wmax[t] + wmax[kWaves + t];
     }
     if (kLaneSeat == 1u) {
         const uint32_t q = slots[t];
-        const uint32_t k = wave_sort<false>(lane_morton(q % kLaneBlockX, q / kLaneBlockX) << kLaneShift | q, lane);
-        slots[t] = (PermT)(k & (kLanePixels - 1u));
+        const uint32_t k = wave_sort<false>(lane_morton(q & (kBlockX - 1u), q >> (4u + LX)) << kShift | q, lane);
+        slots[t] = (PermT)(k & (kPixels - 1u));
         __syncthreads();
     }
-    constexpr uint32_t kWords = kLanePixels * sizeof(PermT) / 4u;
-    uint32_t* out = reinterpret_cast<uint32_t*>(perm + (size_t)blockIdx.x * kLanePixels * sizeof(PermT));
+    constexpr uint32_t kWords = kPixels * sizeof(PermT) / 4u;
+    uint32_t* out = reinterpret_cast<uint32_t*>(perm + (size_t)blockIdx.x * kPixels * sizeof(PermT));
     if (t < kWords) out[t] = reinterpret_cast<const uint32_t*>(slots)[t];
 }
 
@@ -1651,19 +1626,28 @@
     rows = (v.local_rows + 8u * kTilesY - 1u) / (8u * kTilesY);
 }
 
-size_t perm_bytes(uint32_t gx, uint32_t gy) {
-    return (size_t)((gx + kLbX - 1u) / kLbX) * ((gy + kLbY - 1u) / kLbY) * kLanePixels * sizeof(PermT);
-}
-
-LaneShape lane_shape() {
-    return {kLaneBlockX, kLaneBlockY, (uint32_t)sizeof(PermT), kLaneSeat};
-}
-
-hipError_t launch_perm(const uint32_t* pcost, uint32_t LW, uint32_t rows, uint32_t gx, uint32_t gy, uint8_t* perm,
-                       uint32_t* cost, hipStream_t stream) {
-    const uint32_t nb = ((gx + kLbX - 1u) / kLbX) * ((gy + kLbY - 1u) / kLbY);
+size_t perm_bytes(uint32_t shape, uint32_t gx, uint32_t gy) {
+    const uint32_t lx = lane_lx(shape), ly = lane_ly(shape);
+    return (size_t)((gx + (1u << lx) - 1u) >> lx) * ((gy + (1u << ly) - 1u) >> ly) * lane_pixels(shape) * sizeof(PermT);
+}
+
+LaneLayout lane_layout() {
+    return {(uint32_t)sizeof(PermT), kLaneSeat};
+}
+
+hipError_t launch_perm(uint32_t shape, const uint32_t* pcost, uint32_t LW, uint32_t rows, uint32_t gx, uint32_t gy,
+                       uint8_t* perm, uint32_t* cost, hipStream_t stream) {
+    if (!lane_shape_ok(shape)) return hipErrorInvalidValue;
+    const uint32_t lx = lane_lx(shape), ly = lane_ly(shape);
+    const uint32_t nb = ((gx + (1u << lx) - 1u) >> lx) * ((gy + (1u << ly) - 1u) >> ly);
     if (nb == 0) return hipSuccess;
-    hipLaunchKernelGGL(perm_kernel, dim3(nb), dim3(kLanePixels), 0, stream, pcost, LW, rows, gx, gy, perm, cost);
+#define VR_PERM(LX, LY) \
+    hipLaunchKernelGGL((perm_kernel<LX, LY>), dim3(nb), dim3(128u << (LX + LY)), 0, stream, pcost, LW, rows, gx, gy, perm, cost)
+    if (shape == kLane16x16) VR_PERM(0, 1);
+    else if (shape == kLane16x32) VR_PERM(0, 2);
+    else if (shape == kLane16x64) VR_PERM(0, 3);
+    else VR_PERM(1, 2);
+#undef VR_PERM
     return hipGetLastError();
 }
 
@@ -1700,13 +1684,20 @@
     const bool hi = in_flight && !count;
     if (store == STORE_VCS) {
         if (algo == ALGO_ORIGINAL) { if (count) VR_LAUNCH(STORE_VCS, ALGO_ORIGINAL, true); else VR_LAUNCH(STORE_VCS, ALGO_ORIGINAL, false); }
-        else if (hi && kLongHiVariant) VR_LAUNCH_HI(STORE_VCS, ALGO_LONGEST, false, true);
-        else { if (count) VR_LAUNCH(STORE_VCS, ALGO_LONGEST, true); else VR_LAUNCH(STORE_VCS, ALGO_LONGEST, false); }
+        else {
+            bool launched = false;
+            if constexpr (kLongHiVariant) {
+                if (hi) { VR_LAUNCH_HI(STORE_VCS, ALGO_LONGEST, false, true); launched = true; }
+            }
+            if (!launched) { if (count) VR_LAUNCH(STORE_VCS, ALGO_LONGEST, true); else VR_LAUNCH(STORE_VCS, ALGO_LONGEST, false); }
+        }
     } else {
         if (algo == ALGO_ORIGINAL) {
-            if (hi && kOrigHiVariant) VR_LAUNCH_HI(STORE_HASH, ALGO_ORIGINAL, false, true);
-            else if (count) VR_LAUNCH(STORE_HASH, ALGO_ORIGINAL, true);
-            else VR_LAUNCH(STORE_HASH, ALGO_ORIGINAL, false);
+            bool launched = false;
+            if constexpr (kOrigHiVariant) {
+                if (hi) { VR_LAUNCH_HI(STORE_HASH, ALGO_ORIGINAL, false, true); launched = true; }
+            }
+            if (!launched) { if (count) VR_LAUNCH(STORE_HASH, ALGO_ORIGINAL, true); else VR_LAUNCH(STORE_HASH, ALGO_ORIGINAL, false); }
         }
         else { if (count) VR_LAUNCH(STORE_HASH, ALGO_LONGEST, true); else VR_LAUNCH(STORE_HASH, ALGO_LONGEST, false); }
     }
diff --git a/voxelraymarcher_amd/renderer.py b/voxelraymarcher_amd/renderer.py
--- a/voxelraymarcher_amd/renderer.py
+++ b/voxelraymarcher_amd/renderer.py
@@ -571,6 +571,12 @@
     return d
 
 
+def debug_lane_shape(device: int = 0, lone=None, in_flight=None) -> None:
+    def code(shape):
+        return 0 if not shape else int(shape[0]) << 16 | int(shape[1])
+    check(lib().vr_debug_lane_shape(int(device), code(lone), code(in_flight)), "vr_debug_lane_shape")
+
+
 def render_tiles(scene: DeviceScene, algorithm: RayMarchAlgorithm, camera: Camera, lighting: _capi.VrLighting,
                  info: VoxelSceneInfo, width: int, height: int, band_rows: int, tile_cols: int, rank: int,
                  nranks: int, out: torch.Tensor, stream=None) -> torch.Tensor:
```

Result: no change. 21960 Mrays/s, median of 2 (+0.1%).
